# ymxlzgy/echoscene

Hardware: AMD Instinct MI355X
Metric: denoising steps/sec (layout+SDF) for 32-node scene-graph, 64^3 SDF (3x16^3 latent), full step = one DDPM layout step + one DDIM shape step over all objects; `value` = the FUSED step (both loops as one hipGraph per step, the layout step on a parallel branch: what the K timed steps ran); `full_steps_p (higher is better)
Workload: dtype f16 MFMA operands / f32 accumulate (shape UNet); f32 (layout, GCN)

## Files before the change

echoscene_amd/csrc/es_conv_route.h:

```cpp
#pragma once
#include <cstddef>
#include <cstdint>
#include "../../include/echoscene_hip.h"
#include "es_error.h"

constexpr int BN = 224;
constexpr int GN_VT = 64;

struct ConvGeom {
    int O, D, H, W;
    int Hi, Wi;
    int Di;
    int lw, lh, ld;
};

enum class ConvKernel {
    none,
    small_n, small_n_tiled, n16, kw_4_1, kw_2_2, ws_256_8_4_3, ws_64_4_4_3, ws_64_4_4_6, ws_128_4_4_3, ws_128_4_8_3, ws_128_4_8_5, ws3,
    ws_256_up_fold,
    linear_ws, linear_deep, lean_256, lean_128, lean_64
};
extern const char* const kConvKernelName[(int)ConvKernel::lean_64 + 1];
enum class ConvReduce { none, plain, gn_part };

enum class SplitRule {
    direct,
    forced_tile,
    few_plain,
    few_kstreams,
    caller,
    rows256,
    deep,
    tiny,
    fill256,
    auto128,
    none
};

struct ConvRoute {
    ConvGeom g;
    int ncdhw;
    long M;
    long omax;
    ConvKernel kernel;
    unsigned gx = 1, gy = 1, gz = 1;
    size_t lds;
    SplitRule rule;
    int S;
    int ncb;
    bool upm, geglu;
    char unbuilt[96];
    bool epi_stats;
    bool stats;
    bool part_ok;
    ConvReduce reduce;
    int vt;
    bool stats_pass;
    int slabs;
    bool fold_bal;
};

struct RouteOptions {
    int conv_tile = 0;
    int conv_force256 = 0;
    int conv_ws = 1;
    int conv_wssplit = 1;
    int conv_wss_target = 256;
    int conv_deep = 1;
    int conv_tinysplit = 1;
    int gn_rg = 1;
    int conv_few = 1;
    int conv_st_bm = 0;
    int conv_st_np = 4;
    int conv_st_ns = 3;
    int conv_kw_ks = 0;
    int env_a3 = 1;
    int env_linws = 1;
    int env_n16 = 1;
};
const RouteOptions& es_route_options();

int conv_route(const es_conv_args& a, const RouteOptions& o, ConvRoute* r);

es_conv_args conv_chunk_args(const es_conv_args& a, const ConvGeom& g, long o0, long n);

inline int gn_voxel_tile(long Oh, int V) {
    int vt = GN_VT;
    while (vt > 8 && Oh * ((V + vt - 1) / vt) < 512) vt >>= 1;
    return vt;
}
```

echoscene_amd/csrc/es_conv_route.hip:

```cpp
#include "es_conv_route.h"
#include <algorithm>
#include <cstdio>
#include <cstdlib>
#include <cstring>
#include <string>

const char* const kConvKernelName[] = {
    "none",
    "small_n", "small_n_tiled", "n16", "kw_4_1", "kw_2_2", "ws_256_8_4_3", "ws_64_4_4_3", "ws_64_4_4_6", "ws_128_4_4_3", "ws_128_4_8_3", "ws_128_4_8_5", "ws3",
    "ws_256_up_fold", "linear_ws", "linear_deep", "lean_256", "lean_128", "lean_64"
};

#ifndef ES_CONV_A3_DEFAULT
#define ES_CONV_A3_DEFAULT true
#endif
namespace {
const struct { const char* name; int RouteOptions::*field; } kOptions[] = {
    {"conv_tile", &RouteOptions::conv_tile}, {"conv_force256", &RouteOptions::conv_force256}, {"conv_ws", &RouteOptions::conv_ws},
    {"conv_wssplit", &RouteOptions::conv_wssplit}, {"conv_wss_target", &RouteOptions::conv_wss_target}, {"conv_deep", &RouteOptions::conv_deep},
    {"conv_tinysplit", &RouteOptions::conv_tinysplit}, {"gn_rg", &RouteOptions::gn_rg}, {"conv_few", &RouteOptions::conv_few},
    {"conv_st_bm", &RouteOptions::conv_st_bm}, {"conv_st_np", &RouteOptions::conv_st_np}, {"conv_st_ns", &RouteOptions::conv_st_ns},
    {"conv_kw_ks", &RouteOptions::conv_kw_ks},
};

RouteOptions& process_options() {
    static RouteOptions o = [] {
        RouteOptions v;
        const char* a3 = getenv("ES_CONV_A3");
        const char* lin = getenv("ES_CONV_LINWS");
        const char* n16 = getenv("ES_CONV_N16");
        v.env_a3 = a3 ? atoi(a3) != 0 : ES_CONV_A3_DEFAULT;
        v.env_linws = !(lin && atoi(lin) == 0);
        v.env_n16 = !(n16 && atoi(n16) == 0);
        return v;
    }();
    return o;
}
}

const RouteOptions& es_route_options() { return process_options(); }

extern "C" int es_vol_set_option(const char* name, int value) {
    ES_REQUIRE(name != nullptr, "es_vol_set_option: null name");
    for (const auto& k : kOptions) if (!strcmp(k.name, name)) { process_options().*k.field = value; return 0; }
    ES_REQUIRE(false, "es_vol_set_option: unknown option '%s'", name);
}
extern "C" int es_vol_options(char* out, int cap) {
    std::string s;
    for (const auto& k : kOptions) { s += k.name; s += '='; s += std::to_string(process_options().*k.field); s += ';'; }
    if (out && cap > 0) { strncpy(out, s.c_str(), (size_t)cap - 1); out[cap - 1] = 0; }
    return (int)s.size() + 1;
}

namespace {

int ilog2_exact(int v) {
    int l = 0;
    while ((1 << l) < v) ++l;
    return (1 << l) == v ? l : -1;
}

int route_geometry(const es_conv_args& a, ConvRoute* r) {
    ES_REQUIRE(a.Cin % 32 == 0 && a.Cin > 0, "es_conv_mfma_f16: Cin=%d must be a positive multiple of 32", a.Cin);
    ES_REQUIRE(a.taps == 27 || a.taps == 1, "es_conv_mfma_f16: taps=%d", a.taps);
    ES_REQUIRE(!a.a2 || (a.Cin2 % 32 == 0 && a.Cin2 > 0), "es_conv_mfma_f16: Cin2=%d", a.Cin2);
    ES_REQUIRE(a.out_f32 || a.out_f16, "es_conv_mfma_f16: no output");
    ES_REQUIRE(a.epilogue == ES_EPI_NONE || (a.epilogue == ES_EPI_GEGLU && a.N % 224 == 0 && a.out_f16 && !a.out_f32 && !a.res &&
                                             !a.rowvec && !a.a2 && a.bias && a.out_ld >= a.N / 2 && a.out_ld % 8 == 0 && a.splitk <= 1),
               "es_conv_mfma_f16: GEGLU epilogue needs N %% 224 == 0 (N=%d), bias, f16 output only, no split-K", a.N);
    ConvGeom& g = r->g;
    g.O = a.O; g.D = a.D; g.H = a.H; g.W = a.W;
    g.Hi = a.H; g.Wi = a.W;
    g.Di = a.D;
    if (a.mode == ES_CONV_DOWN_HW) { g.Hi = 2 * a.H; g.Wi = 2 * a.W; }
    ES_REQUIRE(a.mode >= ES_CONV_SAME && a.mode <= ES_CONV_DOWN_DHW_P01, "es_conv_mfma_f16: unknown mode %d", a.mode);
    if (a.mode == ES_CONV_DOWN_DHW || a.mode == ES_CONV_DOWN_DHW_P01) { g.Hi = 2 * a.H; g.Wi = 2 * a.W; g.Di = 2 * a.D; }
    if (a.mode == ES_CONV_UP_DHW) g.Di = a.D / 2;
    if (a.mode == ES_CONV_UP_HW || a.mode == ES_CONV_UP_DHW) { g.Hi = a.H / 2; g.Wi = a.W / 2; }
    g.lw = ilog2_exact(a.W); g.lh = ilog2_exact(a.H); g.ld = ilog2_exact(a.D);
    ES_REQUIRE(g.lw >= 0 && g.lh >= 0 && g.ld >= 0, "es_conv_mfma_f16: D,H,W must be powers of two (%d,%d,%d)", a.D, a.H, a.W);
    r->ncdhw = a.out_ld < 0 ? 1 : 0;
    ES_REQUIRE(!r->ncdhw || (a.out_f32 && !a.res && !a.out_f16), "es_conv_mfma_f16: NCDHW output is fp32-only, no residual");
    r->M = (long)a.O * a.D * a.H * a.W;
    return 0;
}

long obj_bytes_in(const es_conv_args& a, const ConvGeom& g) { return (long)g.Di * g.Hi * g.Wi * a.Cin * 2; }
long obj_bytes_in2(const es_conv_args& a) { return a.a2 ? (long)a.D * a.H * a.W * a.Cin2 * 2 : 0; }

int route_chunks(const es_conv_args& a, const RouteOptions& o, ConvRoute* r) {
    const ConvGeom& g = r->g;
    const long per_obj_in = obj_bytes_in(a, g), per_obj_in2 = obj_bytes_in2(a);
    const long halo = 4L * ((g.Hi + 1) * g.Wi + 1) * a.Cin;
    const long lim = (1L << 31) - halo - 1;
    long omax = a.O;
    if (per_obj_in > 0) omax = std::min(omax, lim / per_obj_in);
    if (per_obj_in2 > 0) omax = std::min(omax, lim / per_obj_in2);
    ES_REQUIRE(omax >= 1, "es_conv_mfma_f16: one object exceeds 2 GiB of input (%ld bytes)", per_obj_in);
    if (omax >= a.O) return 0;
    ConvRoute rc;
    if (int err = conv_route(conv_chunk_args(a, g, 0, omax), o, &rc)) return err;
    r->omax = omax;
    r->S = rc.S;
    r->slabs = (int)((rc.slabs * omax + a.O - 1) / a.O);
    r->stats_pass = a.gn_stats_out != nullptr;
    return 0;
}

bool route_direct(const es_conv_args& a, const RouteOptions& o, ConvRoute* r) {
    if (a.N <= 4 && a.taps == 27 && a.Cin <= 64) {
        const size_t lds_t = (size_t)1000 * (a.Cin * 2 + 16) + (size_t)a.N * 27 * a.Cin * 2;
        const bool tiled = a.D % 8 == 0 && a.H % 8 == 0 && a.W % 8 == 0 && a.Cin % 8 == 0 && lds_t <= 160 * 1024;
        r->kernel = tiled ? ConvKernel::small_n_tiled : ConvKernel::small_n;
        r->gx = (unsigned)(tiled ? (long)a.O * (a.D / 8) * (a.H / 8) * (a.W / 8) : (r->M + 255) / 256);
        r->lds = tiled ? lds_t : (size_t)a.N * 27 * a.Cin * 2;
        r->S = 1;
        return true;
    }
    if (a.N <= 16 && a.taps == 27 && a.Cin > 64 && r->ncdhw && a.mode == ES_CONV_SAME && !a.a2 && !a.res && !a.rowvec &&
        !a.out_f16 && a.D % 4 == 0 && a.H % 4 == 0 && a.W % 16 == 0 && o.env_n16 &&
        (long)a.O * a.D * a.H * a.W * a.Cin * 2 < (1L << 31)) {
        r->kernel = ConvKernel::n16;
        r->gx = (unsigned)((long)a.O * (a.D / 4) * (a.H / 4) * (a.W / 16));
        r->S = 1;
        return true;
    }
    return false;
}

struct TileCounts {
    long t256, t128, t64;
    long t64h;
};
TileCounts tile_counts(long rows, int N) {
    const long ntn = (N + BN - 1) / BN;
    return {((rows + 255) / 256) * ntn, ((rows + 127) / 128) * ntn, ((rows + 63) / 64) * ntn, ((rows + 63) / 64) * ((N + 111) / 112)};
}
struct LaunchSize {
    long M;
    int ntn, nks;
    TileCounts wg;
    bool can_split;
    bool ws;
    int forced_ks, forced_bm;
};
struct RefSize {
    long Oh;
    TileCounts hg;
    int slab_cap;
    bool small;
};
long ref_objects(const es_conv_args& a) { return a.O_hint < 0 ? -(long)a.O_hint : (long)(a.O_hint > a.O ? a.O_hint : a.O); }

LaunchSize launch_size(const es_conv_args& a, const RouteOptions& o, const ConvRoute& r) {
    LaunchSize L;
    L.M = r.M;
    L.ntn = (a.N + BN - 1) / BN;
    L.nks = a.taps * (a.Cin / 32) + (a.a2 ? a.Cin2 / 32 : 0);
    L.wg = tile_counts(r.M, a.N);
    const bool vec_out = !r.ncdhw && a.N % 4 == 0 && a.out_ld % 4 == 0 && (!a.rowvec || a.rowvec_ld % 4 == 0);
    L.can_split = a.workspace && vec_out;
    L.ws = o.conv_ws != 0 && vec_out && r.M * (long)a.out_ld < (1L << 30) && r.M * (long)a.N < (1L << 30) &&
           (!a.rowvec || (a.D * a.H * a.W) % 64 == 0);
// ... 5 lines not shown
    RefSize R;
    R.Oh = ref_objects(a);
    const long Mh = R.Oh * a.D * a.H * a.W;
    R.hg = tile_counts(Mh, a.N);
    R.slab_cap = Mh * (long)a.N <= (1L << 22) ? 16 : 8;
    R.small = R.hg.t256 < 256 && o.conv_tile != 128 && o.conv_force256 != 1;
    return R;
}

int keep_units(int s, int nks, int units) {
    while (s > 1 && nks / s < units) --s;
    return s;
}
int caller_split(const es_conv_args& a, const LaunchSize& L) { return a.splitk > 1 && L.can_split && a.epilogue != ES_EPI_GEGLU ? a.splitk : 1; }

int split_forced_tile(const es_conv_args& a, const RouteOptions&, const LaunchSize& L, const RefSize&) { return L.forced_bm ? caller_split(a, L) : 0; }

bool few_eligible(const es_conv_args& a, const RouteOptions& o, const LaunchSize& L, const RefSize& R) {
    if (!o.conv_few || !L.ws || !R.small) return false;
    if (a.epilogue == ES_EPI_GEGLU) return a.mode != ES_CONV_UP_HW && a.mode != ES_CONV_UP_DHW && a.taps == 1 && a.splitk <= 0 && L.wg.t128 < 320;
    return a.splitk < 0 && L.can_split;
}
bool few_kstreams_fit(const es_conv_args& a, const LaunchSize& L, const RefSize& R) {
    return a.epilogue != ES_EPI_GEGLU && a.taps == 1 && L.nks < 112 && R.hg.t64h <= 272 && L.nks >= 12;
}
int split_few_plain(const es_conv_args& a, const RouteOptions& o, const LaunchSize& L, const RefSize& R) {
    if (!few_eligible(a, o, L, R)) return 0;
    if (a.epilogue == ES_EPI_GEGLU || (a.taps == 1 && L.nks < 112)) return few_kstreams_fit(a, L, R) ? 0 : 1;
    const long h128 = R.hg.t128;
    int s2 = (int)((256 + h128 / 2) / h128);
    s2 = s2 < 1 ? 1 : (s2 > 8 ? 8 : s2);
    const bool one_round = h128 * s2 <= 272;
    s2 = keep_units(s2, L.nks, 24);
    return !(L.nks >= 800 && h128 * 8 < 256) && one_round && (s2 >= 2 || h128 >= 224) ? s2 : 0;
}
int split_few_kstreams(const es_conv_args& a, const RouteOptions& o, const LaunchSize& L, const RefSize& R) {
    if (!few_eligible(a, o, L, R) || !few_kstreams_fit(a, L, R)) return 0;
    return L.wg.t256 < 256 && L.wg.t64h <= 768 ? 1 : 4;
}

int split_caller(const es_conv_args& a, const RouteOptions&, const LaunchSize& L, const RefSize&) { return a.splitk > 0 ? caller_split(a, L) : 0; }

int split_rows256(const es_conv_args& a, const RouteOptions& o, const LaunchSize& L, const RefSize& R) {
    if (!(L.ws && a.epilogue != ES_EPI_GEGLU && a.splitk < 0 && L.can_split && R.small && o.conv_wssplit != 0)) return 0;
    const long wst = o.conv_wss_target;
    const int s2 = keep_units((int)std::min(wst / R.hg.t256, (long)R.slab_cap), L.nks, 24);
    return s2 >= 2 && R.hg.t256 * s2 >= 160 ? s2 : 0;
}

int split_deep(const es_conv_args& a, const RouteOptions& o, const LaunchSize& L, const RefSize& R) {
    return a.splitk <= 0 && R.small && R.hg.t64 <= 256 && a.taps == 1 && !a.a2 && a.mode == ES_CONV_SAME && L.nks >= 4 && L.nks <= 28 &&
           a.out_ld >= 0 && L.M * (long)a.Cin * 2 < (1L << 31) && o.conv_deep != 0 ? 1 : 0;
}
int split_tiny(const es_conv_args& a, const RouteOptions& o, const LaunchSize& L, const RefSize& R) {
    if (!(a.splitk < 0 && L.can_split && o.conv_force256 != 1 && R.hg.t256 < 256 && R.hg.t128 < 128 && R.hg.t64 < 256 && L.nks >= 10 &&
          o.conv_tinysplit != 0)) return 0;
    const int s3 = (int)std::min(std::min((256 + R.hg.t64 - 1) / R.hg.t64, (long)R.slab_cap), (long)(L.nks / 5));
    return s3 >= 2 ? s3 : 0;
}

int split_fill256(const es_conv_args& a, const RouteOptions&, const LaunchSize& L, const RefSize& R) {
    const long hg256 = R.hg.t256;
    if (!(a.splitk < 0 && L.can_split && hg256 >= 256)) return 0;
    const long r1 = (hg256 + 255) / 256;
    if ((double)hg256 / (double)(r1 * 256) < 0.8)
        for (int s2 = 2; s2 <= 4; ++s2) {
            const long w = hg256 * s2;
            if ((double)w / (double)(((w + 255) / 256) * 256) >= 0.95 && L.nks / s2 >= 48) return s2;
        }
    return 0;
}

int split_auto128(const es_conv_args& a, const RouteOptions& o, const LaunchSize& L, const RefSize& R) {
    if (!(a.splitk < 0 && L.can_split && o.conv_force256 != 1 && R.hg.t256 < 256 && R.hg.t128 < 512)) return 0;
    const long want = (768 + R.hg.t128 / 2) / R.hg.t128;
    const int S = keep_units((int)std::min(std::max(want, 1L), 8L), L.nks, 24);
    return S > 1 ? S : 0;
}
int split_none(const es_conv_args&, const RouteOptions&, const LaunchSize&, const RefSize&) { return 1; }

const struct { SplitRule rule; int (*split)(const es_conv_args&, const RouteOptions&, const LaunchSize&, const RefSize&); } kSplitRules[] = {
    {SplitRule::forced_tile, split_forced_tile}, {SplitRule::few_plain, split_few_plain}, {SplitRule::few_kstreams, split_few_kstreams},
    {SplitRule::caller, split_caller},           {SplitRule::rows256, split_rows256},     {SplitRule::deep, split_deep},
    {SplitRule::tiny, split_tiny},               {SplitRule::fill256, split_fill256},     {SplitRule::auto128, split_auto128},
    {SplitRule::none, split_none},
};
void choose_split(const es_conv_args& a, const RouteOptions& o, const LaunchSize& L, const RefSize& R, ConvRoute* r) {
    for (const auto& k : kSplitRules)
        if (const int S = k.split(a, o, L, R)) {
            r->rule = k.rule;
            r->S = r->slabs = S;
            return;
        }
}

int few_tile_rows(const es_conv_args& a, const LaunchSize& L, const ConvRoute& r) {
    if (L.wg.t256 >= 256) return 256;
    if (r.rule == SplitRule::few_kstreams) return r.S == 1 ? 0 : 128;
    return a.taps == 1 && r.S == 1 ? (L.wg.t128 >= 320 ? 128 : 64) : 128;
}
int tile_rows(const es_conv_args& a, const RouteOptions& o, const LaunchSize& L, const ConvRoute& r) {
    const bool no256 = o.conv_tile == 128, force256 = o.conv_force256 == 1;
    switch (r.rule) {
    case SplitRule::few_plain:
    case SplitRule::few_kstreams: return few_tile_rows(a, L, r);
    case SplitRule::rows256: return 256;
    case SplitRule::tiny: return 64;
    default: break;
    }
    if (!no256 && (L.wg.t256 >= 256 || (force256 && (r.S == 1 || r.rule == SplitRule::fill256)))) return 256;
    return L.wg.t128 >= 512 || r.S > 1 ? 128 : 64;
}

void forced_tile(const RouteOptions& o, const LaunchSize& L, ConvRoute* r) {
    const unsigned uy = (unsigned)L.ntn;
    if (const int ks = L.forced_ks) {
        r->kernel = ks == 4 ? ConvKernel::kw_4_1 : ks == 2 ? ConvKernel::kw_2_2 : ConvKernel::none;
        snprintf(r->unbuilt, sizeof(r->unbuilt), "conv_kw_ks=%d (2 or 4)", ks);
        r->gx = (unsigned)((L.M + 63) / 64); r->gy = ks == 4 ? 2 * uy : uy;
        return;
    }
    const int bm = L.forced_bm, np = o.conv_st_np, ns = o.conv_st_ns;
    if (bm == 64 && np == 4 && ns == 3) r->kernel = ConvKernel::ws_64_4_4_3;
    else if (bm == 64 && np == 4 && ns == 6) r->kernel = ConvKernel::ws_64_4_4_6;
    else if (bm == 128 && np == 4 && ns == 3) r->kernel = ConvKernel::ws_128_4_4_3;
    else if (bm == 128 && np == 8 && ns == 3) r->kernel = ConvKernel::ws_128_4_8_3;
    else if (bm == 128 && np == 8 && ns == 5) r->kernel = ConvKernel::ws_128_4_8_5;
    else snprintf(r->unbuilt, sizeof(r->unbuilt), "conv_st_bm=%d conv_st_np=%d conv_st_ns=%d is not a built tile", bm, np, ns);
    r->gx = (unsigned)((L.M + bm - 1) / bm); r->gy = uy;
}

void tile_256(const es_conv_args& a, const RouteOptions& o, const LaunchSize& L, ConvRoute* r) {
    r->gx = (unsigned)((L.M + 255) / 256);
    if (L.ws && a.taps == 1 && !a.a2 && a.mode == ES_CONV_SAME && r->S == 1 && L.ntn >= 2 && o.env_linws)
        for (const int ncb : {8, 6, 4, 3, 2})
            if (L.ntn % ncb == 0 && (long)r->gx * (L.ntn / ncb) >= 256) {
                r->kernel = ConvKernel::linear_ws;
                r->ncb = ncb; r->gy = (unsigned)(L.ntn / ncb);
                return;
            }
    if (!(L.ws && (!r->geglu || !r->upm))) { r->kernel = ConvKernel::lean_256; return; }
    const bool a3 = o.env_a3 && a.taps == 27 && a.mode == ES_CONV_SAME && !a.a2 && a.W <= 16 && a.W >= 4;
    r->kernel = a3 ? ConvKernel::ws3 : ConvKernel::ws_256_8_4_3;
    if (a3 || !(a.mode == ES_CONV_UP_HW && a.w2 && !a.a2 && r->S == 1 && a.O_hint == 0 && a.H >= 2 && a.W >= 2 &&
                ((long)a.D * r->g.Hi * r->g.Wi) % 256 == 0)) return;
    r->kernel = ConvKernel::ws_256_up_fold;
    const long rounds = (L.wg.t256 + 255) / 256;
    if (L.ntn == 3 && !a.workspace && L.M % 256 == 0 && (double)L.wg.t256 / (double)(rounds * 256) < 0.8) {
        r->fold_bal = true;
        r->gy = 2;
    }
}

bool choose_tile(const es_conv_args& a, const RouteOptions& o, const LaunchSize& L, ConvRoute* r) {
    r->ncb = 1;
    r->gy = (unsigned)L.ntn; r->gz = (unsigned)r->S;
    if (r->rule == SplitRule::forced_tile) { forced_tile(o, L, r); return L.forced_bm == 128; }
    if (r->rule == SplitRule::deep) {
        r->kernel = ConvKernel::linear_deep;
        r->gx = (unsigned)((L.M + 63) / 64);
        return false;
    }
    const bool few = r->rule == SplitRule::few_plain || r->rule == SplitRule::few_kstreams;
    const int rows = tile_rows(a, o, L, *r);
    switch (rows) {
    case 256: tile_256(a, o, L, r); return L.ws && r->ncb == 1;
    case 128: r->kernel = few ? ConvKernel::ws_128_4_8_5 : ConvKernel::lean_128; break;
    case 64: r->kernel = few ? ConvKernel::ws_64_4_4_3 : ConvKernel::lean_64; break;
    default: r->kernel = ConvKernel::kw_4_1; r->gy = 2 * (unsigned)L.ntn; break;
    }
    r->gx = (unsigned)((L.M + (rows ? rows : 64) - 1) / (rows ? rows : 64));
    return few && rows == 128;
}

void route_flags(const es_conv_args& a, bool stats_tile, ConvRoute* r) {
    const int V = a.D * a.H * a.W;
    r->epi_stats = stats_tile && !r->geglu && r->S == 1 && (a.out_f32 || a.out_f16) && a.N % 4 == 0 && a.out_ld % 4 == 0 && V % 64 == 0;
    r->part_ok = r->S > 1 && r->rule != SplitRule::few_kstreams && a.out_f32 && !r->ncdhw && a.N % 4 == 0 && a.N <= 2048 && a.out_ld == a.N &&
                 a.gn_part_groups > 0 && a.gn_part_groups <= 64 && a.N % a.gn_part_groups == 0;
    const bool want_stats = a.gn_stats_out != nullptr;
    r->stats = want_stats && r->epi_stats;
    r->stats_pass = want_stats && !r->epi_stats;
    if (r->S > 1) {
        r->reduce = a.gn_part_out && r->part_ok ? ConvReduce::gn_part : ConvReduce::plain;
        if (r->reduce == ConvReduce::gn_part) r->vt = gn_voxel_tile(ref_objects(a), V);
    }
}

}

es_conv_args conv_chunk_args(const es_conv_args& a, const ConvGeom& g, long o0, long n) {
    const long V = (long)a.D * a.H * a.W;
    es_conv_args c = a;
    c.O = (int32_t)n;
    c.O_hint = a.O_hint < 0 ? a.O_hint : (a.O_hint > a.O ? a.O_hint : a.O);
    c.a = (const char*)a.a + o0 * obj_bytes_in(a, g);
    if (a.a2) c.a2 = (const char*)a.a2 + o0 * obj_bytes_in2(a);
    if (a.rowvec) c.rowvec = a.rowvec + o0 * a.rowvec_ld;
    if (a.out_ld < 0) {
        c.out_f32 = a.out_f32 + o0 * a.N * V;
    } else {
        if (a.res) c.res = a.res + o0 * V * a.out_ld;
        if (a.out_f32) c.out_f32 = a.out_f32 + o0 * V * a.out_ld;
        if (a.out_f16) c.out_f16 = (char*)a.out_f16 + o0 * V * a.out_ld * 2;
    }
    c.gn_stats_out = c.gn_part_out = nullptr;
    return c;
}

int conv_route(const es_conv_args& a, const RouteOptions& o, ConvRoute* r) {
    *r = ConvRoute{};
    if (int err = route_geometry(a, r)) return err;
    if (int err = route_chunks(a, o, r)) return err;
    if (r->omax || route_direct(a, o, r)) return 0;
    ES_REQUIRE(!a.gn_stats_out || ((a.out_f32 || a.out_f16) && !r->ncdhw && a.N % 4 == 0 && a.out_ld % 4 == 0 && (a.D * a.H * a.W) % 64 == 0 &&
                                   a.epilogue == ES_EPI_NONE),
               "es_conv_mfma_f16: gn_stats_out needs a channels-last output, N %% 4 == 0 and voxels per object %% 64 == 0");
    r->upm = a.mode == ES_CONV_UP_HW || a.mode == ES_CONV_UP_DHW;
    r->geglu = a.epilogue == ES_EPI_GEGLU;
    ES_REQUIRE(!r->upm || (!a.a2 && a.taps == 27), "es_conv_mfma_f16: nearest-up modes take 3x3x3 convs without a fused skip");
    const LaunchSize L = launch_size(a, o, *r);
    choose_split(a, o, L, ref_size(a, o), r);
    route_flags(a, choose_tile(a, o, L, r), r);
    return 0;
}

extern "C" int es_conv_route_of(const es_conv_args* a, es_conv_route_info* out) {
    ConvRoute r;
    if (conv_route(*a, es_route_options(), &r) != 0) return -1;
    *out = es_conv_route_info{(int32_t)r.kernel, r.gx, r.gy, r.gz, (int32_t)r.lds, r.S, r.slabs, r.ncb, (int32_t)r.omax,
                              (int32_t)r.epi_stats, (int32_t)r.stats, (int32_t)r.stats_pass, (int32_t)r.part_ok, (int32_t)r.reduce, r.vt,
                              (int32_t)r.fold_bal};
    return 0;
}
extern "C" int es_conv_emits_gn_stats(const es_conv_args* a) {
    es_conv_route_info i;
    return es_conv_route_of(a, &i) == 0 ? i.epi_stats : -1;
}
extern "C" int es_conv_emits_gn_part(const es_conv_args* a) {
    es_conv_route_info i;
    return es_conv_route_of(a, &i) == 0 ? i.part_ok : -1;
}
extern "C" int es_conv_split_of(const es_conv_args* a) {
    es_conv_route_info i;
    return es_conv_route_of(a, &i) == 0 ? i.slabs : -1;
}
extern "C" int es_conv_kernel_of(const es_conv_args* a, char* name_out, int cap) {
    es_conv_route_info i;
    if (es_conv_route_of(a, &i) != 0) return -1;
    if (name_out && cap > 0) snprintf(name_out, (size_t)cap, "%s", i.omax ? "chunked" : kConvKernelName[i.kernel]);
    return i.S > 1 ? i.S : 1;
}
extern "C" int es_conv_fold_balanced(const es_conv_args* a) {
    es_conv_route_info i;
    return es_conv_route_of(a, &i) == 0 ? i.fold_bal : -1;
}
```

echoscene_amd/csrc/es_vol.hip:

```cpp
#include "es_common.h"
#include "es_conv_route.h"
#include <string>
#include <algorithm>
#include <cstdlib>
#include <initializer_list>
#include <utility>
#include <type_traits>

namespace {

__device__ __forceinline__ int f_swz(int row) { return (0x1320 >> (((row >> 2) & 3) * 4)) & 3; }


__global__ __launch_bounds__(256) void k_gn_partial(const es_gn_args a, float* part, int vt) {
    __shared__ float ssum4[4][2048], ssq4[4][2048];
    float* ssum = ssum4[0];
    float* ssq = ssq4[0];
    const int o = blockIdx.y, tile = blockIdx.x, C = a.C1 + a.C2;
    const int v0 = tile * vt;
    const int nv = min(vt, a.V - v0);
    const int c4n = C >> 2;
    const int CX = 64;
    const int cx = threadIdx.x & (CX - 1), vy = threadIdx.x >> 6;
    for (int c4 = cx; c4 < c4n; c4 += CX) {
// ... 828 lines not shown
        stage_advance();
    };

    f4 acc[MI][7];
#pragma unroll
    for (int i = 0; i < MI; ++i)
#pragma unroll
        for (int j = 0; j < 7; ++j) acc[i][j] = f4{0.f, 0.f, 0.f, 0.f};

    const int i16 = lane & 15, q = lane >> 4;
    const int fragA = (wm * WROWS + i16) * 64 + ((q ^ f_swz(i16)) << 4);
    const int fragB = A_BYTES + (wn * 112 + i16) * 64 + ((q ^ f_swz(i16)) << 4);

    stage_all(0);
    if (nloc > 1) stage_all(1);
    int ks = 0;
    auto body = [&](auto slot_c) __attribute__((always_inline)) {
        constexpr int RS = decltype(slot_c)::value;
        constexpr int WS = (RS + 2) % NS;
        if (ks + 1 < nloc) wait_vmcnt<NLOAD>(); else wait_vmcnt<0>();
        __builtin_amdgcn_s_barrier();
        const bool pf = ks + 2 < nloc;
        if (pf) stage_prep();
        h8 af[MI], bfr[7];
        const char* As = smem + RS * STAGE_BYTES;
#pragma unroll
        for (int j = 0; j < 7; ++j) bfr[j] = *(const h8*)(As + fragB + j * 1024);
#pragma unroll
        for (int i = 0; i < MI; ++i) af[i] = *(const h8*)(As + fragA + i * 1024);
        constexpr int PPR = (NLOAD + MI - 1) / MI;
#pragma unroll
        for (int i = 0; i < MI; ++i) {
#pragma unroll
            for (int j = 0; j < 7; ++j)
                acc[i][j] = __builtin_amdgcn_mfma_f32_16x16x32_f16(af[i], bfr[j], acc[i][j], 0, 0, 0);
            __builtin_amdgcn_sched_barrier(0);
            if (pf) {
#pragma unroll
                for (int pp = 0; pp < PPR; ++pp)
                    if (i * PPR + pp < NLOAD) stage_piece(WS, i * PPR + pp);
            }
            __builtin_amdgcn_sched_barrier(0);
        }
        if (pf) stage_advance();
    };
    while (true) {
        body(std::integral_constant<int, 0>{}); if (++ks >= nloc) break;
        body(std::integral_constant<int, 1>{}); if (++ks >= nloc) break;
        body(std::integral_constant<int, 2>{}); if (++ks >= nloc) break;
    }
    conv_epilogue<BM_, NW_>(a, g, acc, smem, M, m0, n0, wave, lane, S, bz, ncdhw);
}

__global__ __launch_bounds__(256) void k_linear_deep(const es_conv_args a, const ConvGeom g) {
    constexpr int BM_ = 64, NW_ = 4, NS = 7, NT = 256;
    constexpr int WROWS = BM_ / (NW_ / 2), MI = WROWS / 16;
    constexpr int A_BYTES = BM_ * BK * 2, B_BYTES = BNP * BK * 2, STAGE_BYTES = A_BYTES + B_BYTES;
    constexpr int NA = BM_ * 4 / NT, NB = BNP * 4 / NT, NLOAD = NA + NB;
    constexpr unsigned OOB = 0x80000000u;
    typedef __attribute__((address_space(3))) void* lds_ptr;
    extern __shared__ __attribute__((aligned(16))) char smem[];
    const int tid = threadIdx.x, lane = tid & 63;
    const int wave = __builtin_amdgcn_readfirstlane(tid >> 6);
    const int wm = wave >> 1, wn = wave & 1;
    const long M = (long)g.O * g.D * g.H * g.W;
    int bx, by, bz;
    conv_tile_of(a, bx, by, bz);
    const long m0 = (long)bx * BM_;
    const int n0 = by * BN;
    const int nloc = a.Cin >> 5;
    unsigned voffA;
    {
        const int row = tid >> 2;
        const long m = m0 + row;
        voffA = m < M ? (unsigned)(m * a.Cin * 2 + (((tid & 3) ^ f_swz(row)) * 16)) : OOB;
    }
    const __amdgpu_buffer_rsrc_t rA = __builtin_amdgcn_make_buffer_rsrc(uniform_ptr(a.a), (short)0, (int)OOB, 0x00020000);
    const __amdgpu_buffer_rsrc_t rB = __builtin_amdgcn_make_buffer_rsrc(uniform_ptr((const _Float16*)a.w + ((long)by * nloc) * (BNP * BK)), (short)0, (int)OOB, 0x00020000);
    auto stage = [&](int ks, int slot) __attribute__((always_inline)) {
        char* dst = smem + slot * STAGE_BYTES + wave * 1024;
        __builtin_amdgcn_raw_ptr_buffer_load_lds(rA, (lds_ptr)dst, 16, (int)voffA, (int)((unsigned)ks * 64u), 0, 0);
#pragma unroll
        for (int j = 0; j < NB; ++j) {
            const unsigned vB = (unsigned)tid * 16u + (unsigned)j * (NT * 16) >= (unsigned)(BN * BK * 2) ? OOB : (unsigned)tid * 16u;
            __builtin_amdgcn_raw_ptr_buffer_load_lds(rB, (lds_ptr)(dst + A_BYTES + j * (NT * 16)), 16, (int)vB,
                                                     (int)((unsigned)ks * (unsigned)B_BYTES + (unsigned)j * (NT * 16)), 0, 0);
        }
    };
    f4 acc[MI][7];
#pragma unroll
    for (int i = 0; i < MI; ++i)
#pragma unroll
        for (int j = 0; j < 7; ++j) acc[i][j] = f4{0.f, 0.f, 0.f, 0.f};
    const int i16 = lane & 15, q = lane >> 4;
    const int fragA = (wm * WROWS + i16) * 64 + ((q ^ f_swz(i16)) << 4);
    const int fragB = A_BYTES + (wn * 112 + i16) * 64 + ((q ^ f_swz(i16)) << 4);
    int issued = 0;
    for (; issued < NS - 1 && issued < nloc; ++issued) stage(issued, issued);
    int slot = 0;
    for (int ks = 0; ks < nloc; ++ks) {
        const int after = issued - 1 - ks;
        if (after >= 5) wait_vmcnt<5 * NLOAD>(); else if (after == 4) wait_vmcnt<4 * NLOAD>(); else if (after == 3) wait_vmcnt<3 * NLOAD>();
        else if (after == 2) wait_vmcnt<2 * NLOAD>(); else if (after == 1) wait_vmcnt<NLOAD>(); else wait_vmcnt<0>();
        __builtin_amdgcn_s_barrier();
        if (issued < nloc) { const int ws_ = slot == 0 ? NS - 1 : slot - 1; stage(issued, ws_); ++issued; }
        const char* As = smem + slot * STAGE_BYTES;
        h8 af[MI], bfr[7];
#pragma unroll
        for (int j = 0; j < 7; ++j) bfr[j] = *(const h8*)(As + fragB + j * 1024);
#pragma unroll
        for (int i = 0; i < MI; ++i) af[i] = *(const h8*)(As + fragA + i * 1024);
#pragma unroll
        for (int i = 0; i < MI; ++i)
#pragma unroll
            for (int j = 0; j < 7; ++j) acc[i][j] = __builtin_amdgcn_mfma_f32_16x16x32_f16(af[i], bfr[j], acc[i][j], 0, 0, 0);
        slot = slot == NS - 1 ? 0 : slot + 1;
    }
    conv_epilogue<BM_, NW_>(a, g, acc, smem, M, m0, n0, wave, lane, 1, 0, 0);
}

template <int MI>
__device__ __forceinline__ void ws_read_frags(const char* As, int fragA, int fragB, h8 (&af)[MI], h8 (&bfr)[7]) {
#pragma unroll
    for (int j = 0; j < 7; ++j) bfr[j] = *(const h8*)(As + fragB + j * 1024);
#pragma unroll
    for (int i = 0; i < MI; ++i) af[i] = *(const h8*)(As + fragA + i * 1024);
}

template <int MI>
__device__ __forceinline__ void ws_mma(f4 (&acc)[MI][7], const h8 (&af)[MI], const h8 (&bfr)[7]) {
#pragma unroll
    for (int i = 0; i < MI; ++i)
#pragma unroll
        for (int j = 0; j < 7; ++j) acc[i][j] = __builtin_amdgcn_mfma_f32_16x16x32_f16(af[i], bfr[j], acc[i][j], 0, 0, 0);
}

#ifdef ES_STAMP
__device__ unsigned long long* g_stamp_buf = nullptr;
#define ES_STAMP_AT(k) do { if (stamp && lane == 0) stamp[k] = __builtin_amdgcn_s_memrealtime(); } while (0)
#else
#define ES_STAMP_AT(k) do { } while (0)
#endif

template <int NL, int MAXA>
__device__ __forceinline__ void wait_ahead(int ahead) {
    if constexpr (MAXA > 0) {
        if (ahead >= MAXA) { wait_vmcnt<MAXA * NL>(); return; }
        wait_ahead<NL, MAXA - 1>(ahead);
    } else {
        wait_vmcnt<0>();
    }
}

template <int BM_, int NC_, int NP_, bool UP_, int EPI_, bool STATS_, int NS_ = 3, bool FOLD_ = false>
__device__ __forceinline__ void conv_ws_tile(const es_conv_args& a, const ConvGeom& g, int ncdhw, char* smem, const int wave, const int lane,
                                             const long M, const int bx, const int by, const int ks_begin, const int ks_end,
                                             const int S, const int bz, unsigned long long* stamp) {
    constexpr int NS = NS_, UPS_ = 1;
    constexpr int WROWS = BM_ / (NC_ / 2);
    constexpr int MI = WROWS / 16;
    constexpr int A_BYTES = BM_ * BK * 2, B_BYTES = BNP * BK * 2, UNIT_BYTES = A_BYTES + B_BYTES;
    constexpr int STAGE_BYTES = UPS_ * UNIT_BYTES;
    constexpr int APIECES = BM_ / 16, BPIECES = BNP / 16;
    constexpr int NA = APIECES / NP_, NB = BPIECES / NP_, NLOAD = NA + NB;
    static_assert(APIECES % NP_ == 0 && BPIECES % NP_ == 0, "pieces must divide over the producer waves");
    constexpr unsigned OOB = 0x80000000u;
    typedef __attribute__((address_space(3))) void* lds_ptr;
    (void)stamp;
    const long m0 = (long)bx * BM_;
    const int n0 = by * BN;
    const int kch0 = a.Cin >> 5;
    const int ntap0 = FOLD_ ? 12 : a.taps;
    const int nks0 = ntap0 * kch0;
    const int nloc = ks_end - ks_begin;
    const int nstage = (nloc + UPS_ - 1) / UPS_;
    static_assert(!FOLD_ || UP_, "the folded taps are those of a nearest-up conv");
    const int fold_cls = FOLD_ ? (int)((m0 >> (g.lw + g.lh + g.ld - 2)) & 3) : 0;
    const int fold_ph = fold_cls >> 1, fold_pw = fold_cls & 1;
    if (wave >= NC_) {
        const int pw = wave - NC_;
        int a_lc[NA], a_o[NA], a_d[NA], a_h[NA], a_w[NA];
        bool a_ok[NA];
#pragma unroll
        for (int j = 0; j < NA; ++j) {
            const int p = (pw + NP_ * j) * 64 + lane;
            const int row = p >> 2;
            a_lc[j] = (p & 3) ^ f_swz(row);
            const long m = m0 + row;
            a_ok[j] = m < M;
            const long mm = a_ok[j] ? m : 0;
            a_w[j] = (int)(mm & (g.W - 1));
            a_h[j] = (int)((mm >> g.lw) & (g.H - 1));
            a_d[j] = (int)((mm >> (g.lw + g.lh)) & (g.D - 1));
            a_o[j] = (int)(mm >> (g.lw + g.lh + g.ld));
            if constexpr (FOLD_) {
                a_w[j] = 2 * (int)(mm & (g.Wi - 1)) + fold_pw;
                a_h[j] = 2 * (int)((mm >> (g.lw - 1)) & (g.Hi - 1)) + fold_ph;
                a_d[j] = (int)((mm >> (g.lw + g.lh - 2)) & (g.D - 1));
            }
        }
        int st_phase = ks_begin >= nks0 ? 1 : 0;
        int st_tap = st_phase ? 0 : ks_begin % ntap0;
        int st_c = st_phase ? (ks_begin - nks0) : (ks_begin / ntap0);
        int st_ntap = st_phase ? 1 : ntap0, st_kch = st_phase ? (a.Cin2 >> 5) : kch0;
        unsigned st_boff = (unsigned)(st_phase ? (ks_begin - nks0) : ks_begin) * (unsigned)B_BYTES;
        unsigned voff[NA], msk[NA];
        int upm[NA][3], upp[NA][3];
        int dtab = 0;
        __amdgpu_buffer_rsrc_t rA, rB;
        auto set_phase = [&]() __attribute__((always_inline)) {
            const _Float16* Wg = (const _Float16*)(st_phase ? a.w2 : a.w);
            const long nks_ph = st_phase ? (long)(a.Cin2 >> 5) : (long)nks0;
            if constexpr (FOLD_) Wg = (const _Float16*)a.w2 + ((long)fold_cls * ((a.N + BN - 1) / BN) * nks0) * (BNP * BK);
            rB = __builtin_amdgcn_make_buffer_rsrc((void*)(Wg + ((long)by * nks_ph) * (BNP * BK)), (short)0, (int)OOB, 0x00020000);
            const _Float16* Ag = (const _Float16*)(st_phase ? a.a2 : a.a);
            const int Cin = st_phase ? a.Cin2 : a.Cin;
            const int p01 = (!st_phase && a.mode == ES_CONV_DOWN_DHW_P01) ? 1 : 0;
            const bool down = !st_phase && (a.mode == ES_CONV_DOWN_HW || a.mode == ES_CONV_DOWN_DHW || p01);
            const bool downd = !st_phase && (a.mode == ES_CONV_DOWN_DHW || p01);
            const int Dsrc = downd ? 2 * g.D : g.D;
            const int Hi = st_phase ? g.H : g.Hi, Wi = st_phase ? g.W : g.Wi;
            const int ntap = st_phase ? 1 : a.taps;
            const bool updhw = UP_ && a.mode == ES_CONV_UP_DHW;
            const int Di = updhw ? g.D / 2 : g.D;
            const int bias = ntap == 27 ? ((Hi + 1) * Wi + 1) * Cin * 2 : 0;
            rA = __builtin_amdgcn_make_buffer_rsrc((void*)((const char*)Ag - bias), (short)0, (int)OOB, 0x00020000);
            {
                const int t = lane < 27 ? lane : 13;
                const int kd = t / 9 - 1, kh = (t / 3) % 3 - 1, kw = t % 3 - 1;
                dtab = ntap == 27 ? ((kd * Hi + kh) * Wi + kw) * Cin * 2 + bias : 0;
                if (UP_) dtab = ntap == 27 ? (updhw ? 0 : kd * Hi * Wi * Cin * 2) + bias : 0;
            }
#pragma unroll
            for (int j = 0; j < NA; ++j) {
                const int ch = down ? 2 * a_h[j] + p01 : a_h[j];
                const int cw = down ? 2 * a_w[j] + p01 : a_w[j];
                const int cd = downd ? 2 * a_d[j] + p01 : a_d[j];
                voff[j] = (unsigned)(((((long)a_o[j] * Dsrc + cd) * Hi + ch) * Wi + cw) * Cin * 2 + a_lc[j] * 16);
                if (UP_) {
                    const int sd = updhw ? a_d[j] >> 1 : a_d[j];
                    voff[j] = (unsigned)(((((long)a_o[j] * Di + sd) * Hi + (a_h[j] >> 1)) * Wi + (a_w[j] >> 1)) * Cin * 2 + a_lc[j] * 16);
                    const int SD = Hi * Wi * Cin * 2, SH = Wi * Cin * 2, SW = Cin * 2;
                    upm[j][0] = (updhw && !(a_d[j] & 1)) ? -SD : 0; upp[j][0] = (updhw && (a_d[j] & 1)) ? SD : 0;
                    upm[j][1] = !(a_h[j] & 1) ? -SH : 0;            upp[j][1] = (a_h[j] & 1) ? SH : 0;
                    upm[j][2] = !(a_w[j] & 1) ? -SW : 0;            upp[j][2] = (a_w[j] & 1) ? SW : 0;
                }
                unsigned m = 0;
                if (ntap == 1) {
                    m = a_ok[j] ? 1u : 0u;
                } else {
                    m = a_ok[j] ? tap_mask27(cd, Dsrc, ch, UP_ ? g.H : Hi, cw, UP_ ? g.W : Wi) : 0u;
                }
                msk[j] = m;
            }
        };
        set_phase();
        ES_STAMP_AT(1);
        const unsigned voffB = (unsigned)lane * 16u;
        auto issue_unit = [&](char* dst) __attribute__((always_inline)) {
            int tap27 = st_tap;
            if constexpr (FOLD_) tap27 = (st_tap >> 2) * 9 + (((st_tap >> 1) & 1) + fold_ph) * 3 + (st_tap & 1) + fold_pw;
            const unsigned sA = (unsigned)__builtin_amdgcn_readlane(dtab, tap27) + (unsigned)st_c * 64u;
            const unsigned sbit = 1u << tap27;
            int ukd = 0, ukh = 0, ukw = 0;
            if (UP_) { ukd = tap27 / 9 - 1; ukh = (tap27 / 3) % 3 - 1; ukw = tap27 % 3 - 1; }
#pragma unroll
            for (int j = 0; j < NA; ++j) {
                unsigned vs = voff[j];
                if (UP_) {
                    vs += (unsigned)(ukd < 0 ? upm[j][0] : ukd > 0 ? upp[j][0] : 0);
                    vs += (unsigned)(ukh < 0 ? upm[j][1] : ukh > 0 ? upp[j][1] : 0);
                    vs += (unsigned)(ukw < 0 ? upm[j][2] : ukw > 0 ? upp[j][2] : 0);
                }
                const unsigned vo = (msk[j] & sbit) ? vs : OOB;
                __builtin_amdgcn_raw_ptr_buffer_load_lds(rA, (lds_ptr)(dst + (pw + NP_ * j) * 1024), 16, (int)vo, (int)sA, 0, 0);
            }
#pragma unroll
            for (int j = 0; j < NB; ++j) {
                const int q = pw + NP_ * j;
                const unsigned vB = q * 16 >= BN ? OOB : voffB;
                __builtin_amdgcn_raw_ptr_buffer_load_lds(rB, (lds_ptr)(dst + A_BYTES + q * 1024), 16, (int)vB,
                                                         (int)(st_boff + (unsigned)q * 1024u), 0, 0);
            }
            st_boff += (unsigned)B_BYTES;
            if (++st_tap == st_ntap) {
                st_tap = 0;
                if (++st_c == st_kch && !st_phase && a.a2) {
                    st_phase = 1; st_c = 0; st_ntap = 1; st_kch = a.Cin2 >> 5; st_boff = 0;
                    set_phase();
                }
            }
        };
        int issued = 0;
        auto issue_stage = [&](int st) __attribute__((always_inline)) {
            char* base = smem + (st % NS) * STAGE_BYTES;
#pragma unroll
            for (int u = 0; u < UPS_; ++u)
                if (issued < nloc) { issue_unit(base + u * UNIT_BYTES); ++issued; }
        };
        {
            static_assert(NLOAD * (NS - 2) <= 63, "vmcnt is a 6-bit counter");
#pragma unroll
            for (int st = 0; st < NS - 1; ++st)
                if (st < nstage) issue_stage(st);
            for (int st = 0; st < nstage; ++st) {
                wait_ahead<NLOAD, NS - 2>(nstage - 1 - st);
                __builtin_amdgcn_s_barrier();
                if (st == 0) ES_STAMP_AT(2);
                if (st + NS - 1 < nstage) issue_stage(st + NS - 1);
            }
        }
        ES_STAMP_AT(3);
        f4 dummy[MI][7];
        conv_epilogue<BM_, NC_, false, true, EPI_, false, STATS_, FOLD_>(a, g, dummy, smem, M, m0, n0, wave, lane, S, bz, ncdhw);
        ES_STAMP_AT(4);
        return;
    }
    const int wm = wave >> 1, wn = wave & 1;
    f4 acc[MI][7];
#pragma unroll
    for (int i = 0; i < MI; ++i)
#pragma unroll
        for (int j = 0; j < 7; ++j) acc[i][j] = f4{0.f, 0.f, 0.f, 0.f};
    const int i16 = lane & 15, q = lane >> 4;
    const int fragA = (wm * WROWS + i16) * 64 + ((q ^ f_swz(i16)) << 4);
    const int fragB = A_BYTES + (wn * 112 + i16) * 64 + ((q ^ f_swz(i16)) << 4);
    h8 af[MI], bfr[7];
    {
        int slot = 0;
        ES_STAMP_AT(1);
        __builtin_amdgcn_s_barrier();
        ES_STAMP_AT(2);
        ws_read_frags<MI>(smem, fragA, fragB, af, bfr);
        for (int ks = 0; ks + 1 < nloc; ++ks) {
            slot = slot == NS - 1 ? 0 : slot + 1;
            const char* const An = smem + slot * STAGE_BYTES;
#pragma unroll
            for (int j = 0; j < 7; ++j) acc[0][j] = __builtin_amdgcn_mfma_f32_16x16x32_f16(af[0], bfr[j], acc[0][j], 0, 0, 0);
            __builtin_amdgcn_sched_barrier(0);
            asm volatile("s_waitcnt lgkmcnt(0)" ::: "memory");
            __builtin_amdgcn_s_barrier();
            __builtin_amdgcn_sched_barrier(0);
#pragma unroll
            for (int i = 1; i < MI; ++i) {
                af[i - 1] = *(const h8*)(An + fragA + (i - 1) * 1024);
                __builtin_amdgcn_sched_barrier(0);
                if (i < MI - 1) {
#pragma unroll
                    for (int j = 0; j < 7; ++j) acc[i][j] = __builtin_amdgcn_mfma_f32_16x16x32_f16(af[i], bfr[j], acc[i][j], 0, 0, 0);
                    __builtin_amdgcn_sched_barrier(0);
                } else {
#pragma unroll
                    for (int j = 0; j < 7; ++j) {
                        acc[i][j] = __builtin_amdgcn_mfma_f32_16x16x32_f16(af[i], bfr[j], acc[i][j], 0, 0, 0);
                        __builtin_amdgcn_sched_barrier(0);
                        bfr[j] = *(const h8*)(An + fragB + j * 1024);
                        __builtin_amdgcn_sched_barrier(0);
                    }
                }
            }
            af[MI - 1] = *(const h8*)(An + fragA + (MI - 1) * 1024);
            __builtin_amdgcn_sched_barrier(0);
        }
        ws_mma<MI>(acc, af, bfr);
    }
    ES_STAMP_AT(3);
    conv_epilogue<BM_, NC_, true, true, EPI_, false, STATS_, FOLD_>(a, g, acc, smem, M, m0, n0, wave, lane, S, bz, ncdhw);
    ES_STAMP_AT(4);
}

template <int BM_, int NC_, int NP_, bool UP_ = false, int EPI_ = ES_EPI_NONE, bool STATS_ = false, int NS_ = 3>
__global__ __launch_bounds__(64 * (NC_ + NP_), 3) void k_conv_ws(const es_conv_args a, const ConvGeom g, int ncdhw) {
    extern __shared__ __attribute__((aligned(16))) char smem[];
    const int tid = threadIdx.x, lane = tid & 63;
    const int wave = __builtin_amdgcn_readfirstlane(tid >> 6);
    unsigned long long* stamp = nullptr;
#ifdef ES_STAMP
    stamp = g_stamp_buf ? g_stamp_buf + ((size_t)(blockIdx.x + gridDim.x * (blockIdx.y + gridDim.y * blockIdx.z)) * (NC_ + NP_) + wave) * 8 : nullptr;
#endif
    ES_STAMP_AT(0);
    const long M = (long)g.O * g.D * g.H * g.W;
    int bx, by, bz;
    conv_tile_of(a, bx, by, bz);
    const int S = gridDim.z;
    int ks_begin, ks_end;
    split_range(a.taps * (a.Cin >> 5), a.a2 ? (a.Cin2 >> 5) : 0, a.taps, bz, S, ks_begin, ks_end);
    conv_ws_tile<BM_, NC_, NP_, UP_, EPI_, STATS_, NS_>(a, g, ncdhw, smem, wave, lane, M, bx, by, ks_begin, ks_end, S, bz, stamp);
}

template <bool STATS_>
__global__ __launch_bounds__(768, 3) void k_conv_ws_fold(const es_conv_args a, const ConvGeom g) {
    extern __shared__ __attribute__((aligned(16))) char smem[];
    const int tid = threadIdx.x, lane = tid & 63;
    const int wave = __builtin_amdgcn_readfirstlane(tid >> 6);
    unsigned long long* stamp = nullptr;
#ifdef ES_STAMP
    stamp = g_stamp_buf ? g_stamp_buf + ((size_t)(blockIdx.x + gridDim.x * (blockIdx.y + gridDim.y * blockIdx.z)) * 12 + wave) * 8 : nullptr;
#endif
    ES_STAMP_AT(0);
    const long M = (long)g.O * g.D * g.H * g.W;
    int bx, by, bz;
    conv_tile_of(a, bx, by, bz);
    conv_ws_tile<256, 8, 4, true, ES_EPI_NONE, STATS_, 3, true>(a, g, 0, smem, wave, lane, M, bx, by, 0, 12 * (a.Cin >> 5), 1, 0, stamp);
}

template <bool STATS_>
__global__ __launch_bounds__(768, 3) void k_conv_ws_fold_bal(const es_conv_args a, const ConvGeom g) {
    extern __shared__ __attribute__((aligned(16))) char smem[];
    const int tid = threadIdx.x, lane = tid & 63;
    const int wave = __builtin_amdgcn_readfirstlane(tid >> 6);
    const long M = (long)g.O * g.D * g.H * g.W;
    int bx, by, bz;
    conv_tile_of(a, bx, by, bz);
    const int nks = 12 * (a.Cin >> 5);
    conv_ws_tile<256, 8, 4, true, ES_EPI_NONE, STATS_, 3, true>(a, g, 0, smem, wave, lane, M, bx, by, 0, nks, 1, 0, nullptr);
    __syncthreads();
    conv_ws_tile<128, 8, 4, true, ES_EPI_NONE, STATS_, 3, true>(a, g, 0, smem, wave, lane, M, 2 * bx + by, 2, 0, nks, 1, 0, nullptr);
}

typedef int i4v __attribute__((ext_vector_type(4)));
template <int DIR>
__device__ __forceinline__ h8 a3_shift(const h8 v, const bool zero_lane) {
    i4v x = __builtin_bit_cast(i4v, v);
#pragma unroll
    for (int e = 0; e < 4; ++e) {
        const int s = DIR < 0 ? __builtin_amdgcn_update_dpp(0, x[e], 0x111, 0xf, 0xf, true) : __builtin_amdgcn_update_dpp(0, x[e], 0x101, 0xf, 0xf, true);
        x[e] = zero_lane ? 0 : s;
    }
    return __builtin_bit_cast(h8, x);
}

template <bool STATS_>
__global__ __launch_bounds__(768, 3) void k_conv_ws3(const es_conv_args a, const ConvGeom g) {
    constexpr int BM_ = 256, NC_ = 8, NP_ = 4, NSB = 7, MI = 4;
    constexpr int A_BYTES = BM_ * BK * 2, B_BYTES = BNP * BK * 2, A_RING = NSB * B_BYTES;
    constexpr int NA = (BM_ / 16) / NP_, NB = (BNP / 16) / NP_;
    constexpr unsigned OOB = 0x80000000u;
    typedef __attribute__((address_space(3))) void* lds_ptr;
    extern __shared__ __attribute__((aligned(16))) char smem[];
    const int tid = threadIdx.x, lane = tid & 63;
    const int wave = __builtin_amdgcn_readfirstlane(tid >> 6);
    const long M = (long)g.O * g.D * g.H * g.W;
    int bx, by, bz;
    conv_tile_of(a, bx, by, bz);
    const int S = gridDim.z;
    const int kch0 = a.Cin >> 5, nks0 = 27 * kch0;
    int ks_begin, ks_end;
    split_range(nks0, 0, 27, bz, S, ks_begin, ks_end);
    const int nloc = ks_end - ks_begin, ngrp = nloc / 3;
    const long m0 = (long)bx * BM_;
    const int n0 = by * BN;
    if (wave >= NC_) {
        const int pw = wave - NC_;
        unsigned voff[NA], msk[NA];
#pragma unroll
        for (int j = 0; j < NA; ++j) {
            const int p = (pw + NP_ * j) * 64 + lane;
            const int row = p >> 2;
            const int lc = (p & 3) ^ f_swz(row);
            const long m = m0 + row;
            const bool ok = m < M;
            const long mm = ok ? m : 0;
            const int w = (int)(mm & (g.W - 1)), h = (int)((mm >> g.lw) & (g.H - 1)), d = (int)((mm >> (g.lw + g.lh)) & (g.D - 1));
            const int o = (int)(mm >> (g.lw + g.lh + g.ld));
            voff[j] = (unsigned)(((((long)o * g.D + d) * g.H + h) * g.W + w) * a.Cin * 2 + lc * 16);
            msk[j] = ok ? tap_mask27(d, g.D, h, g.H, w, g.W) : 0u;
        }
        const int bias = ((g.H + 1) * g.W + 1) * a.Cin * 2;
        const __amdgpu_buffer_rsrc_t rA = __builtin_amdgcn_make_buffer_rsrc((void*)((const char*)a.a - bias), (short)0, (int)OOB, 0x00020000);
        const __amdgpu_buffer_rsrc_t rB = __builtin_amdgcn_make_buffer_rsrc((void*)((const _Float16*)a.w + ((long)by * nks0) * (BNP * BK)), (short)0, (int)OOB, 0x00020000);
        int dtab;
        {
            const int t = lane < 27 ? lane : 13;
            const int kd = t / 9 - 1, kh = (t / 3) % 3 - 1, kw = t % 3 - 1;
            dtab = ((kd * g.H + kh) * g.W + kw) * a.Cin * 2 + bias;
        }
        int a_tap = ks_begin % 27, a_c = ks_begin / 27;
        unsigned b_off = (unsigned)ks_begin * (unsigned)B_BYTES;
        const unsigned voffB = (unsigned)lane * 16u;
        auto issue_A = [&](int slot) __attribute__((always_inline)) {
            char* dst = smem + A_RING + slot * A_BYTES;
            const unsigned sA = (unsigned)__builtin_amdgcn_readlane(dtab, a_tap + 1) + (unsigned)a_c * 64u;
            const unsigned sbit = 1u << (a_tap + 1);
#pragma unroll
            for (int j = 0; j < NA; ++j)
                __builtin_amdgcn_raw_ptr_buffer_load_lds(rA, (lds_ptr)(dst + (pw + NP_ * j) * 1024), 16, (int)((msk[j] & sbit) ? voff[j] : OOB), (int)sA, 0, 0);
            a_tap += 3;
            if (a_tap == 27) { a_tap = 0; ++a_c; }
        };
        auto issue_B = [&](int slot) __attribute__((always_inline)) {
            char* dst = smem + slot * B_BYTES;
#pragma unroll
            for (int j = 0; j < NB; ++j) {
                const int q = pw + NP_ * j;
                __builtin_amdgcn_raw_ptr_buffer_load_lds(rB, (lds_ptr)(dst + q * 1024), 16, (int)(q * 16 >= BN ? OOB : voffB), (int)(b_off + (unsigned)q * 1024u), 0, 0);
            }
            b_off += (unsigned)B_BYTES;
        };
        int sb = 0;
        auto issue_group = [&](int gi) __attribute__((always_inline)) {
            issue_A(gi & 1);
#pragma unroll
            for (int t = 0; t < 3; ++t) { issue_B(sb); sb = sb == NSB - 1 ? 0 : sb + 1; }
        };
        issue_group(0);
        for (int gi = 0; gi < ngrp; ++gi) {
            wait_vmcnt<0>();
            __builtin_amdgcn_s_barrier();
            if (gi + 1 < ngrp) issue_group(gi + 1);
        }
        __builtin_amdgcn_s_barrier();
        f4 dummy[MI][7];
        conv_epilogue<BM_, NC_, false, true, ES_EPI_NONE, false, STATS_>(a, g, dummy, smem, M, m0, n0, wave, lane, S, bz, 0);
        return;
    }
    const int wm = wave >> 1, wn = wave & 1;
    f4 acc[MI][7];
#pragma unroll
    for (int i = 0; i < MI; ++i)
#pragma unroll
        for (int j = 0; j < 7; ++j) acc[i][j] = f4{0.f, 0.f, 0.f, 0.f};
    const int i16 = lane & 15, q = lane >> 4;
    const int fragA = A_RING + (wm * 64 + i16) * 64 + ((q ^ f_swz(i16)) << 4);
    const int fragB = (wn * 112 + i16) * 64 + ((q ^ f_swz(i16)) << 4);
    const bool zl = (i16 & (g.W - 1)) == 0, zr = (i16 & (g.W - 1)) == ((g.W - 1) & 15);
    h8 afc[MI], bq[3];
    __builtin_amdgcn_s_barrier();
    bq[0] = *(const h8*)(smem + fragB);
    bq[1] = *(const h8*)(smem + fragB + 1024);
#pragma unroll
    for (int i = 0; i < MI; ++i) afc[i] = *(const h8*)(smem + fragA + i * 1024);
    int slotB = 0;
    for (int grp = 0; grp < ngrp; ++grp) {
        const char* const An = smem + ((grp + 1) & 1) * A_BYTES;
        auto unit = [&](auto kwc) __attribute__((always_inline)) {
            constexpr int KW = decltype(kwc)::value;
            const char* const Bc = smem + slotB * B_BYTES;
            slotB = slotB == NSB - 1 ? 0 : slotB + 1;
            const char* const Bn = smem + slotB * B_BYTES;
            h8 ash[MI];
// ... 1041 lines not shown
    const int h0 = jh == 0 ? 0 : (ph == 0 ? 1 : 2), h1 = jh == 0 ? (ph == 0 ? 0 : 1) : 2;
    const int w0 = jw == 0 ? 0 : (pw == 0 ? 1 : 2), w1 = jw == 0 ? (pw == 0 ? 0 : 1) : 2;
    double s = 0.0;
    for (int kh = h0; kh <= h1; ++kh)
        for (int kw = w0; kw <= w1; ++kw) s += (double)w27[kd * 9 + kh * 3 + kw];
    float f = (float)s;
    if ((double)f != s) {
        uint32_t u = __builtin_bit_cast(uint32_t, f);
        const double af = f < 0.f ? -(double)f : (double)f, as = s < 0.0 ? -s : s;
        if (af > as) --u;
        u |= 1u;
        f = __builtin_bit_cast(float, u);
    }
    return f;
}

extern "C" size_t es_pack_conv_up_fold_f16_size(int N, int Cin) { return 4 * es_pack_conv_f16_size(N, Cin, 12); }

extern "C" int es_pack_conv_up_fold_f16(const float* h_w, int N, int CinW, uint16_t* h_out) {
    ES_REQUIRE(h_w && h_out && N > 0 && CinW > 0, "es_pack_conv_up_fold_f16: N=%d Cin=%d", N, CinW);
    const int Cin = (CinW + 31) / 32 * 32;
    const int nt = (N + BN - 1) / BN, kch = Cin / 32;
    es_parallel_for(4L * nt * kch * 12, [=](long bi) {
        const int tap = (int)(bi % 12), kc = (int)((bi / 12) % kch), t = (int)((bi / (12L * kch)) % nt), cls = (int)(bi / (12L * kch * nt));
        uint16_t* blk = h_out + (size_t)bi * (BNP * BK);
        for (int p = 0; p < BNP * 4; ++p) {
            const int row = p >> 2, lc = (p & 3) ^ h_swz(row);
            const int n = t * BN + row;
            for (int e = 0; e < 8; ++e) {
                const int c = kc * 32 + lc * 8 + e;
                blk[p * 8 + e] = (row < BN && n < N && c < CinW) ? f32_to_f16_bits(up_fold_weight(h_w + ((size_t)n * CinW + c) * 27, cls, tap)) : 0;
            }
        }
    });
    return 0;
}

__global__ __launch_bounds__(256) void k_pack_conv_up_fold_f16(const float* __restrict__ w, int N, int CinW, int kch, int nt, h8* __restrict__ out, long nslots) {
    const long s = (long)blockIdx.x * 256 + threadIdx.x;
    if (s >= nslots) return;
    const int p = (int)(s & (BNP * 4 - 1));
    const long bi = s / (BNP * 4);
    const int tap = (int)(bi % 12), kc = (int)((bi / 12) % kch), t = (int)((bi / (12L * kch)) % nt), cls = (int)(bi / (12L * kch * nt));
    const int row = p >> 2, lc = (p & 3) ^ ((0x1320 >> (((row >> 2) & 3) * 4)) & 3);
    const int n = t * BN + row;
    h8 v;
#pragma unroll
    for (int e = 0; e < 8; ++e) {
        const int c = kc * 32 + lc * 8 + e;
        v[e] = (row < BN && n < N && c < CinW) ? (_Float16)up_fold_weight(w + ((size_t)n * CinW + c) * 27, cls, tap) : (_Float16)0.f;
    }
    out[s] = v;
}

extern "C" int es_pack_conv_up_fold_f16_dev(const float* d_w, int N, int CinW, uint16_t* d_out, es_stream stream) {
    ES_REQUIRE(d_w && d_out && N > 0 && CinW > 0, "es_pack_conv_up_fold_f16_dev: N=%d Cin=%d", N, CinW);
    const int Cin = (CinW + 31) / 32 * 32;
    const long nslots = (long)es_pack_conv_up_fold_f16_size(N, Cin) / 8;
    hipLaunchKernelGGL(k_pack_conv_up_fold_f16, dim3((unsigned)((nslots + 255) / 256)), dim3(256), 0, (hipStream_t)stream, d_w, N, CinW, Cin / 32,
                       (N + BN - 1) / BN, (h8*)d_out, nslots);
    ES_CHECK_HIP(hipGetLastError());
    return 0;
}

extern "C" int es_pack_conv_rows_f16(const float* h_w, int N, int CinW, int taps, uint16_t* h_out) {
    const int Cin = (CinW + 31) / 32 * 32;
    for (int n = 0; n < N; ++n)
        for (int t = 0; t < taps; ++t)
            for (int c = 0; c < Cin; ++c)
                h_out[((size_t)n * taps + t) * Cin + c] = c < CinW ? f32_to_f16_bits(h_w[((size_t)n * CinW + c) * taps + t]) : 0;
    return 0;
}

namespace {
struct LdsLimits {
    hipError_t err = hipSuccess;
    LdsLimits(std::initializer_list<std::pair<const void*, int>> kernels) {
        for (const auto& k : kernels)
            if (const hipError_t e = hipFuncSetAttribute(k.first, hipFuncAttributeMaxDynamicSharedMemorySize, k.second); err == hipSuccess) err = e;
    }
};

dim3 grid_of(const ConvRoute& r) { return dim3(r.gx, r.gy, r.gz); }
}

constexpr int LDS256 = 3 * (256 * BK * 2 + BNP * BK * 2), LDS128 = 3 * (128 * BK * 2 + BNP * BK * 2), LDS64 = 3 * (64 * BK * 2 + BNP * BK * 2);
constexpr int LDSLIN = LDS256 + 8 * 16 * 116 * 4;
constexpr int LDSDEEP = 7 * (64 * BK * 2 + BNP * BK * 2);
constexpr int LDSWS3 = 9 * 16384;

template <int BM_, int NC_, int NP_, int NS_>
static int launch_ws(const es_conv_args* a, const ConvRoute& r, hipStream_t st) {
    constexpr int LDS = NS_ * (BM_ * BK * 2 + BNP * BK * 2);
    constexpr bool CAN_STATS = BM_ / (NC_ / 2) == 64;
    static_assert(LDS <= 160 * 1024, "ring exceeds the CU's LDS");
    static const LdsLimits lim{{(const void*)k_conv_ws<BM_, NC_, NP_, false, ES_EPI_NONE, false, NS_>, LDS},
                               {(const void*)k_conv_ws<BM_, NC_, NP_, true, ES_EPI_NONE, false, NS_>, LDS},
                               {(const void*)k_conv_ws<BM_, NC_, NP_, false, ES_EPI_GEGLU, false, NS_>, LDS}};
    ES_REQUIRE(lim.err == hipSuccess, "es_conv_mfma_f16: hipFuncSetAttribute failed: %s", hipGetErrorString(lim.err));
    const dim3 blk(64 * (NC_ + NP_));
    if (r.geglu) hipLaunchKernelGGL((k_conv_ws<BM_, NC_, NP_, false, ES_EPI_GEGLU, false, NS_>), grid_of(r), blk, LDS, st, *a, r.g, r.ncdhw);
    else if (r.stats) {
        if constexpr (CAN_STATS) {
            static const LdsLimits lim_stats{{(const void*)k_conv_ws<BM_, NC_, NP_, false, ES_EPI_NONE, true, NS_>, LDS},
                                             {(const void*)k_conv_ws<BM_, NC_, NP_, true, ES_EPI_NONE, true, NS_>, LDS}};
            ES_REQUIRE(lim_stats.err == hipSuccess, "es_conv_mfma_f16: hipFuncSetAttribute failed: %s", hipGetErrorString(lim_stats.err));
            if (r.upm) hipLaunchKernelGGL((k_conv_ws<BM_, NC_, NP_, true, ES_EPI_NONE, true, NS_>), grid_of(r), blk, LDS, st, *a, r.g, r.ncdhw);
            else hipLaunchKernelGGL((k_conv_ws<BM_, NC_, NP_, false, ES_EPI_NONE, true, NS_>), grid_of(r), blk, LDS, st, *a, r.g, r.ncdhw);
        } else ES_REQUIRE(false, "launch_ws: row-group sums need 64-row waves");
    }
    else if (r.upm) hipLaunchKernelGGL((k_conv_ws<BM_, NC_, NP_, true, ES_EPI_NONE, false, NS_>), grid_of(r), blk, LDS, st, *a, r.g, r.ncdhw);
    else hipLaunchKernelGGL((k_conv_ws<BM_, NC_, NP_, false, ES_EPI_NONE, false, NS_>), grid_of(r), blk, LDS, st, *a, r.g, r.ncdhw);
    return 0;
}

template <int KS_, int NCH_>
static int launch_kw(const es_conv_args* a, const ConvRoute& r, hipStream_t st) {
    constexpr int RING = 3 * KS_ * (64 * BK * 2 + NCH_ * 112 * BK * 2), PART = 4 * 112 * 64 * 4;
    constexpr int LDS = RING > PART ? RING : PART;
    static const LdsLimits lim{{(const void*)k_conv_kw<KS_, NCH_, false, ES_EPI_NONE>, LDS},
                               {(const void*)k_conv_kw<KS_, NCH_, true, ES_EPI_NONE>, LDS},
                               {(const void*)k_conv_kw<KS_, NCH_, false, ES_EPI_GEGLU>, LDS}};
    ES_REQUIRE(lim.err == hipSuccess, "es_conv_mfma_f16: hipFuncSetAttribute failed: %s", hipGetErrorString(lim.err));
    const dim3 blk(768);
    if (r.geglu) hipLaunchKernelGGL((k_conv_kw<KS_, NCH_, false, ES_EPI_GEGLU>), grid_of(r), blk, LDS, st, *a, r.g, r.ncdhw);
    else if (r.upm) hipLaunchKernelGGL((k_conv_kw<KS_, NCH_, true, ES_EPI_NONE>), grid_of(r), blk, LDS, st, *a, r.g, r.ncdhw);
    else hipLaunchKernelGGL((k_conv_kw<KS_, NCH_, false, ES_EPI_NONE>), grid_of(r), blk, LDS, st, *a, r.g, r.ncdhw);
    return 0;
}

template <int BM_, int NW_>
static void launch_lean(const es_conv_args* a, const ConvRoute& r, hipStream_t st) {
    constexpr int LDS = 3 * (BM_ * BK * 2 + BNP * BK * 2);
    if (r.upm) hipLaunchKernelGGL((k_conv_lean<BM_, NW_, true>), grid_of(r), dim3(64 * NW_), LDS, st, *a, r.g, r.ncdhw);
    else hipLaunchKernelGGL((k_conv_lean<BM_, NW_>), grid_of(r), dim3(64 * NW_), LDS, st, *a, r.g, r.ncdhw);
}

static void launch_rowgroup_stats(const es_conv_args* a, long rows, hipStream_t st) {
    const long n4 = ((rows + 63) / 64) * (a->N / 4);
    const int blocks = (int)((n4 + 255) / 256 < 8192 ? (n4 + 255) / 256 : 8192);
    hipLaunchKernelGGL(k_rowgroup_stats, dim3(blocks), dim3(256), 0, st, (const float*)a->out_f32, rows, a->N, a->out_ld, a->gn_stats_out);
}

static int conv_launch(const es_conv_args* a, const ConvRoute& r, hipStream_t st) {
    static const LdsLimits lim{{(const void*)k_conv_small_n_tiled, 160 * 1024},
                               {(const void*)k_conv_n16, N16_A_BYTES + N16_B_BYTES},
                               {(const void*)k_conv_lean<256, 8>, LDS256}, {(const void*)k_conv_lean<256, 8, true>, LDS256},
                               {(const void*)k_conv_lean<128, 4>, LDS128}, {(const void*)k_conv_lean<128, 4, true>, LDS128},
                               {(const void*)k_conv_lean<64, 4>, LDS64}, {(const void*)k_conv_lean<64, 4, true>, LDS64},
                               {(const void*)k_linear_deep, LDSDEEP},
                               {(const void*)k_linear_ws<ES_EPI_NONE>, LDSLIN}, {(const void*)k_linear_ws<ES_EPI_GEGLU>, LDSLIN},
                               {(const void*)k_conv_ws3<false>, LDSWS3}, {(const void*)k_conv_ws3<true>, LDSWS3},
                               {(const void*)k_conv_ws_fold<false>, LDS256}, {(const void*)k_conv_ws_fold<true>, LDS256},
                               {(const void*)k_conv_ws_fold_bal<false>, LDS256}, {(const void*)k_conv_ws_fold_bal<true>, LDS256}};
    ES_REQUIRE(lim.err == hipSuccess, "es_conv_mfma_f16: hipFuncSetAttribute failed: %s", hipGetErrorString(lim.err));
    ES_REQUIRE(r.kernel != ConvKernel::none, "es_conv_mfma_f16: %s", r.omax ? "a chunked route is launched chunk by chunk" : r.unbuilt);
    int rc = 0;
    switch (r.kernel) {
    case ConvKernel::none: break;
    case ConvKernel::small_n:
    case ConvKernel::small_n_tiled:
        ES_REQUIRE(a->mode == ES_CONV_SAME && !a->a2 && !a->res && !a->rowvec && !a->out_f16 && !a->gn_stats_out,
                   "es_conv_mfma_f16: the N<=4, Cin<=64 direct kernel takes SAME mode, fp32 output, no fusions");
        if (r.kernel == ConvKernel::small_n_tiled) hipLaunchKernelGGL(k_conv_small_n_tiled, grid_of(r), dim3(256), r.lds, st, *a, r.g, r.ncdhw);
        else hipLaunchKernelGGL(k_conv_small_n, grid_of(r), dim3(256), r.lds, st, *a, r.g, r.ncdhw);
        break;
    case ConvKernel::n16: hipLaunchKernelGGL(k_conv_n16, grid_of(r), dim3(256), N16_A_BYTES + N16_B_BYTES, st, *a, r.g); break;
    case ConvKernel::kw_4_1: rc = launch_kw<4, 1>(a, r, st); break;
    case ConvKernel::kw_2_2: rc = launch_kw<2, 2>(a, r, st); break;
    case ConvKernel::ws_256_8_4_3: rc = launch_ws<256, 8, 4, 3>(a, r, st); break;
    case ConvKernel::ws_64_4_4_3: rc = launch_ws<64, 4, 4, 3>(a, r, st); break;
    case ConvKernel::ws_64_4_4_6: rc = launch_ws<64, 4, 4, 6>(a, r, st); break;
    case ConvKernel::ws_128_4_4_3: rc = launch_ws<128, 4, 4, 3>(a, r, st); break;
    case ConvKernel::ws_128_4_8_3: rc = launch_ws<128, 4, 8, 3>(a, r, st); break;
    case ConvKernel::ws_128_4_8_5: rc = launch_ws<128, 4, 8, 5>(a, r, st); break;
    case ConvKernel::ws3:
        if (r.stats) hipLaunchKernelGGL((k_conv_ws3<true>), grid_of(r), dim3(768), LDSWS3, st, *a, r.g);
        else hipLaunchKernelGGL((k_conv_ws3<false>), grid_of(r), dim3(768), LDSWS3, st, *a, r.g);
        break;
    case ConvKernel::ws_256_up_fold:
        if (r.fold_bal) {
            if (r.stats) hipLaunchKernelGGL((k_conv_ws_fold_bal<true>), grid_of(r), dim3(768), LDS256, st, *a, r.g);
            else hipLaunchKernelGGL((k_conv_ws_fold_bal<false>), grid_of(r), dim3(768), LDS256, st, *a, r.g);
        } else if (r.stats) hipLaunchKernelGGL((k_conv_ws_fold<true>), grid_of(r), dim3(768), LDS256, st, *a, r.g);
        else hipLaunchKernelGGL((k_conv_ws_fold<false>), grid_of(r), dim3(768), LDS256, st, *a, r.g);
        break;
    case ConvKernel::linear_ws:
        if (r.geglu) hipLaunchKernelGGL((k_linear_ws<ES_EPI_GEGLU>), grid_of(r), dim3(768), LDSLIN, st, *a, r.g, r.ncb);
        else hipLaunchKernelGGL((k_linear_ws<ES_EPI_NONE>), grid_of(r), dim3(768), LDSLIN, st, *a, r.g, r.ncb);
        break;
    case ConvKernel::linear_deep: hipLaunchKernelGGL(k_linear_deep, grid_of(r), dim3(256), LDSDEEP, st, *a, r.g); break;
    case ConvKernel::lean_256: launch_lean<256, 8>(a, r, st); break;
    case ConvKernel::lean_128: launch_lean<128, 4>(a, r, st); break;
    case ConvKernel::lean_64: launch_lean<64, 4>(a, r, st); break;
    }
    if (rc) return rc;
    const int V = a->D * a->H * a->W;
    if (r.reduce == ConvReduce::gn_part)
        hipLaunchKernelGGL(k_conv_splitk_reduce_gn, dim3((V + r.vt - 1) / r.vt, a->O), dim3(256), 0, st, *a, r.M, V, r.S, r.vt);
    else if (r.reduce == ConvReduce::plain) {
        const long n4 = r.M * (a->N / 4);
        const int blocks = (int)((n4 + 255) / 256 < 4096 ? (n4 + 255) / 256 : 4096);
        hipLaunchKernelGGL(k_conv_splitk_reduce, dim3(blocks), dim3(256), 0, st, *a, r.M, V, r.S);
    }
    if (r.stats_pass) {
        ES_REQUIRE(a->out_f32, "es_conv_mfma_f16: this launch's route forms gn_stats_out by a pass over the fp32 output: out_f32 must be given "
                               "(es_conv_emits_gn_stats() == 0)");
        launch_rowgroup_stats(a, r.M, st);
    }
    ES_CHECK_HIP(hipGetLastError());
    return 0;
}

extern "C" int es_conv_mfma_f16(const es_conv_args* a, es_stream stream) {
    ConvRoute r;
    if (int rc = conv_route(*a, es_route_options(), &r)) return rc;
    const hipStream_t st = (hipStream_t)stream;
    if (!r.omax) return conv_launch(a, r, st);
    for (long o0 = 0; o0 < a->O; o0 += r.omax) {
        const es_conv_args c = conv_chunk_args(*a, r.g, o0, std::min(r.omax, (long)a->O - o0));
        ConvRoute rc;
        if (int err = conv_route(c, es_route_options(), &rc)) return err;
        if (int err = conv_launch(&c, rc, st)) return err;
    }
    if (r.stats_pass) {
        ES_REQUIRE(a->out_f32 && !r.ncdhw && a->N % 4 == 0 && a->out_ld % 4 == 0 && ((long)a->D * a->H * a->W) % 64 == 0,
                   "es_conv_mfma_f16: gn_stats_out needs a channels-last fp32 output");
        launch_rowgroup_stats(a, r.M, st);
        ES_CHECK_HIP(hipGetLastError());
    }
    return 0;
}

extern "C" int es_groupnorm_vol(const es_gn_args* a, es_stream stream) {
    const int C = a->C1 + a->C2;
    ES_REQUIRE(C % a->groups == 0 && C <= 2048 && a->groups <= 64, "es_groupnorm_vol: C=%d groups=%d", C, a->groups);
    ES_REQUIRE(a->C1 % 8 == 0 && a->C2 % 8 == 0, "es_groupnorm_vol: channel counts must be multiples of 8 (%d,%d)", a->C1, a->C2);
    ES_REQUIRE(a->stats != nullptr, "es_groupnorm_vol: stats scratch missing");
    const long Oh = a->O_hint < 0 ? -(long)a->O_hint : (long)(a->O_hint > a->O ? a->O_hint : a->O);
    const int vt = gn_voxel_tile(Oh, a->V);
    const int ntiles = (a->V + vt - 1) / vt;
    float* part = a->stats;
    const bool from_rg = a->stats1 && (!a->x2 || a->stats2) && a->V % 64 == 0 && (a->x1_is_f16 || es_route_options().gn_rg != 0);
    ES_REQUIRE(!a->x1_is_f16 || (from_rg && !a->x2 && !a->raw_f16),
               "es_groupnorm_vol: an f16 source needs the producer's row-group sums (stats1), one source, no raw copy");
    ES_REQUIRE(!a->part_in || (!from_rg && !a->x2), "es_groupnorm_vol: part_in needs one source and no row-group sums");
    if (a->part_in) part = (float*)a->part_in;
    else if (!from_rg) hipLaunchKernelGGL(k_gn_partial, dim3(ntiles, a->O), dim3(256), 0, (hipStream_t)stream, *a, part, vt);
    int vpb = 32;
    while (vpb > 8 && (long)a->O * ((a->V + vpb - 1) / vpb) < 512) vpb >>= 1;
    while (vpb < 1024 && (long)a->O * ((a->V + vpb - 1) / vpb) > 16384) vpb <<= 1;
    const float* fin = nullptr;
    if (from_rg) {
        hipLaunchKernelGGL(k_gn_finalize_rg, dim3(a->groups, a->O), dim3(256), 0, (hipStream_t)stream, *a, part);
        fin = part;
    } else if (ntiles > 128) {
        float* f = a->part_in ? a->stats : part + (size_t)a->O * ntiles * a->groups * 2;
        hipLaunchKernelGGL(k_gn_finalize, dim3(a->groups, a->O), dim3(256), 0, (hipStream_t)stream, *a, part, ntiles, f);
        fin = f;
    }
    hipLaunchKernelGGL(k_gn_apply, dim3((a->V + vpb - 1) / vpb, a->O), dim3(256), 0, (hipStream_t)stream, *a, part, ntiles, vpb, fin);
    ES_CHECK_HIP(hipGetLastError());
    return 0;
}

extern "C" int es_layernorm_tokens(const es_ln_args* a, es_stream stream) {
    ES_REQUIRE(a->C <= 1024 && a->C > 0 && a->C % 4 == 0, "es_layernorm_tokens: C=%d (a multiple of 4, max 1024)", a->C);
    long wgs = ((long)a->M + 3) / 4;
    if (wgs > 2048) wgs = 2048;
    hipLaunchKernelGGL(k_layernorm, dim3((unsigned)wgs), dim3(256), 0, (hipStream_t)stream, *a);
    ES_CHECK_HIP(hipGetLastError());
    return 0;
}

extern "C" int es_attention_f16(const es_attn_args* a, es_stream stream) {
    ES_REQUIRE(a->dhead % 4 == 0 && a->dhead <= 256 && a->dhead > 0, "es_attention_f16: dhead=%d (multiple of 4, <= 256)", a->dhead);
    ES_REQUIRE(a->scale > 0.f, "es_attention_f16: scale=%g must be positive (the row maximum is taken over the raw scores)", (double)a->scale);
    const bool big = a->Ntok >= 512 && a->dhead <= 96;
    const int rows = big ? 128 : 64;
    dim3 grid((a->Ntok + rows - 1) / rows, a->B * a->heads);
    hipStream_t st = (hipStream_t)stream;
    if (a->dhead <= 32) { if (big) hipLaunchKernelGGL((k_attention<32, 4, 2>), grid, dim3(256), 0, st, *a); else hipLaunchKernelGGL((k_attention<32, 4, 1>), grid, dim3(256), 0, st, *a); }
    else if (a->dhead <= 64) { if (big) hipLaunchKernelGGL((k_attention<64, 4, 2>), grid, dim3(256), 0, st, *a); else hipLaunchKernelGGL((k_attention<64, 4, 1>), grid, dim3(256), 0, st, *a); }
    else if (a->dhead <= 96) { if (big) hipLaunchKernelGGL((k_attention<96, 4, 2>), grid, dim3(256), 0, st, *a); else hipLaunchKernelGGL((k_attention<96, 4, 1>), grid, dim3(256), 0, st, *a); }
    else hipLaunchKernelGGL((k_attention<256, 4, 1>), grid, dim3(256), 0, st, *a);
    ES_CHECK_HIP(hipGetLastError());
    return 0;
}

extern "C" int es_geglu_f16(const es_geglu_args* a, es_stream stream) {
    ES_REQUIRE(a->C4 % 4 == 0, "es_geglu_f16: C4=%d", a->C4);
    const long n4 = (long)a->M * (a->C4 / 4);
    const int blocks = (int)((n4 + 255) / 256 < 8192 ? (n4 + 255) / 256 : 8192);
    hipLaunchKernelGGL(k_geglu, dim3(blocks), dim3(256), 0, (hipStream_t)stream, *a);
    ES_CHECK_HIP(hipGetLastError());
    return 0;
}

static int latent_to_cl(const float* x, int O, int C, int V, int Cpad, void* out, int is_f32, es_stream stream) {
    const long n = (long)O * V * Cpad;
    const int blocks = (int)((n + 255) / 256 < 4096 ? (n + 255) / 256 : 4096);
    hipLaunchKernelGGL(k_to_cl, dim3(blocks), dim3(256), 0, (hipStream_t)stream, x, O, C, V, Cpad, (_Float16*)out, is_f32);
    ES_CHECK_HIP(hipGetLastError());
    return 0;
}
extern "C" int es_latent_to_cl_f16(const float* x, int O, int C, int V, int Cpad, void* out, es_stream stream) { return latent_to_cl(x, O, C, V, Cpad, out, 0, stream); }
extern "C" int es_latent_to_cl_f32(const float* x, int O, int C, int V, int Cpad, void* out, es_stream stream) { return latent_to_cl(x, O, C, V, Cpad, out, 1, stream); }

extern "C" int es_split_f16x3(const float* x, long M, int C, void* out, es_stream stream) {
    ES_REQUIRE(x && out && M > 0 && C > 0 && C % 4 == 0, "es_split_f16x3: M=%ld C=%d (C a multiple of 4)", M, C);
    const long n = M * (C / 4);
    const int blocks = (int)((n + 255) / 256 < 8192 ? (n + 255) / 256 : 8192);
    hipLaunchKernelGGL(k_split_f16x3, dim3(blocks), dim3(256), 0, (hipStream_t)stream, x, M, C, (_Float16*)out);
    ES_CHECK_HIP(hipGetLastError());
    return 0;
}

extern "C" int es_shape_stem(const es_stem_args* a, es_stream stream) {
    const long n1 = (long)a->O * 32 * 512, n2 = (long)a->O * 512;
    const int Cx = a->Cin ? a->Cin : 3;
    ES_REQUIRE(Cx >= 1 && Cx <= 4, "es_shape_stem: Cin=%d (3 or 4)", Cx);
    (void)n1;
    hipLaunchKernelGGL(k_stem1, dim3(64, a->O), dim3(256), (size_t)(Cx * 288 + 32 * Cx * 27) * 4, (hipStream_t)stream, *a);
    static const LdsLimits lim{{(const void*)k_stem2, 32 * 513 * 4}};
    ES_REQUIRE(lim.err == hipSuccess, "es_shape_stem: hipFuncSetAttribute failed: %s", hipGetErrorString(lim.err));
    hipLaunchKernelGGL(k_stem2, dim3((unsigned)((n2 * 8 + 255) / 256)), dim3(256), 32 * 513 * 4, (hipStream_t)stream, *a);
    ES_CHECK_HIP(hipGetLastError());
    return 0;
}

extern "C" int es_vq_lookup(const es_vq_args* a, es_stream stream) {
    ES_REQUIRE(a->n_embed > 0 && a->n_embed * 16 <= 160 * 1024 - 1024, "es_vq_lookup: n_embed=%d too large for LDS", a->n_embed);
    ES_REQUIRE(a->Cpad >= 3, "es_vq_lookup: Cpad=%d", a->Cpad);
    static const LdsLimits lim{{(const void*)k_vq_lookup, 160 * 1024 - 1024}};
    ES_REQUIRE(lim.err == hipSuccess, "es_vq_lookup: hipFuncSetAttribute failed: %s", hipGetErrorString(lim.err));
    const long M = (long)a->O * a->V;
    hipLaunchKernelGGL(k_vq_lookup, dim3((unsigned)((M + 255) / 256)), dim3(256), (size_t)a->n_embed * 16, (hipStream_t)stream, *a);
    ES_CHECK_HIP(hipGetLastError());
    return 0;
}
```

echoscene_amd/hip.py:

```python
import ctypes as C
import os

HERE = os.path.dirname(os.path.abspath(__file__))
LIB_PATH = os.path.join(HERE, 'libechoscene_hip%s.so' % os.environ.get('ES_LIB_TAG', ''))

c_f32p = C.c_void_p
c_i32p = C.c_void_p

SEG_DIRECT, SEG_GATHER, SEG_CSRMEAN, SEG_CSRSUM, SEG_CSRWAVG = 0, 1, 2, 3, 4
PRO_NONE, PRO_SILU, PRO_GN, PRO_GN_SILU, PRO_LN, PRO_GEGLU, PRO_LN_ATTN = 0, 1, 2, 3, 4, 5, 6
ACT_NONE, ACT_RELU, ACT_SILU, ACT_GEGLU, ACT_SIGMOID = 0, 1, 2, 3, 4
CONV_SAME, CONV_DOWN_HW, CONV_UP_HW, CONV_UP_DHW, CONV_DOWN_DHW = 0, 1, 2, 3, 4
CONV_DOWN_DHW_P01 = 5
EPI_NONE, EPI_GEGLU = 0, 1
(OP_LINEAR, OP_DDPM, OP_DDIM, OP_COPY, OP_CONV, OP_GN, OP_LN, OP_ATTN, OP_GEGLU, OP_TO_CL, OP_STEM) = range(1, 12)
OP_VQ = 12
OP_FORK, OP_JOIN, OP_ROWSEL = 13, 14, 15
OP_CONV_F32, OP_ATTN_F32 = 16, 17
OP_DDIM_BLEND, OP_CONV_C1 = 18, 19
OP_DDPM_KEEP = 21


class Seg(C.Structure):
    _fields_ = [('ptr', C.c_void_p), ('idx', C.c_void_p), ('ent_row', C.c_void_p), ('ent_off', C.c_void_p),
                ('step', C.c_void_p), ('step_stride', C.c_int32), ('ld', C.c_int32), ('width', C.c_int32),
                ('mode', C.c_int32), ('nslab', C.c_int32), ('slab_stride', C.c_int32), ('pre_act', C.c_int32),
                ('pro', C.c_int32), ('gamma', C.c_void_p), ('beta', C.c_void_p), ('eps', C.c_float), ('gs', C.c_int32),
                ('ent_wt', C.c_void_p)]


class LinearArgs(C.Structure):
    _fields_ = [('seg', Seg * 3), ('nseg', C.c_int32), ('M', C.c_int32), ('K', C.c_int32), ('N', C.c_int32),
                ('wpack', C.c_void_p), ('bias', C.c_void_p), ('prologue', C.c_int32), ('gamma', C.c_void_p),
                ('beta', C.c_void_p), ('eps', C.c_float), ('act', C.c_int32), ('res', C.c_void_p),
                ('res_ld', C.c_int32), ('res_nslab', C.c_int32), ('res_slab_stride', C.c_int32),
                ('res2', C.c_void_p), ('res2_ld', C.c_int32), ('res2_nslab', C.c_int32), ('res2_slab_stride', C.c_int32),
                ('out', C.c_void_p),
                ('out_ld', C.c_int32), ('nbatch', C.c_int32), ('a_bstride', C.c_int32), ('out_bstride', C.c_int32),
                ('kb_per_slice', C.c_int32), ('out_slab_stride', C.c_int32), ('fuse_next', C.c_int32),
                ('res_step', C.c_void_p), ('res_step_stride', C.c_int32), ('seg_slices', C.c_int32)]


class UpdateArgs(C.Structure):
    _fields_ = [('x', C.c_void_p), ('eps', C.c_void_p), ('eps_nslab', C.c_int32), ('eps_slab_stride', C.c_int32),
                ('noise', C.c_void_p), ('noise_stride', C.c_int32),
                ('coef', C.c_void_p), ('coef_stride', C.c_int32), ('step', C.c_void_p), ('n', C.c_int32),
                ('inc_step', C.c_int32), ('clip_x0', C.c_int32)]


class ConvArgs(C.Structure):
    _fields_ = [('a', C.c_void_p), ('w', C.c_void_p), ('O', C.c_int32), ('D', C.c_int32), ('H', C.c_int32),
                ('W', C.c_int32), ('Cin', C.c_int32), ('N', C.c_int32), ('taps', C.c_int32), ('mode', C.c_int32),
                ('a2', C.c_void_p), ('w2', C.c_void_p), ('Cin2', C.c_int32), ('bias', C.c_void_p),
                ('rowvec', C.c_void_p), ('rowvec_ld', C.c_int32), ('res', C.c_void_p), ('out_f32', C.c_void_p), ('out_f16', C.c_void_p),
                ('workspace', C.c_void_p), ('splitk', C.c_int32), ('out_ld', C.c_int32), ('O_hint', C.c_int32),
                ('epilogue', C.c_int32), ('gn_stats_out', C.c_void_p), ('gn_part_out', C.c_void_p), ('gn_part_groups', C.c_int32)]


class ConvRouteInfo(C.Structure):
    _fields_ = [('kernel', C.c_int32), ('grid_x', C.c_uint32), ('grid_y', C.c_uint32), ('grid_z', C.c_uint32)] + \
               [(f, C.c_int32) for f in ('lds', 'S', 'slabs', 'ncb', 'omax', 'epi_stats', 'stats', 'stats_pass', 'part_ok', 'reduce', 'vt',
                                         'fold_bal')]


CONV_KERNELS = ('none', 'small_n', 'small_n_tiled', 'n16', 'kw_4_1', 'kw_2_2', 'ws_256_8_4_3', 'ws_64_4_4_3', 'ws_64_4_4_6', 'ws_128_4_4_3',
                'ws_128_4_8_3', 'ws_128_4_8_5', 'ws3', 'ws_256_up_fold', 'linear_ws', 'linear_deep', 'lean_256', 'lean_128', 'lean_64')


class GNArgs(C.Structure):
    _fields_ = [('x1', C.c_void_p), ('C1', C.c_int32), ('x2', C.c_void_p), ('C2', C.c_int32), ('O', C.c_int32),
                ('V', C.c_int32), ('groups', C.c_int32), ('eps', C.c_float), ('gamma', C.c_void_p),
                ('beta', C.c_void_p), ('silu', C.c_int32), ('stats', C.c_void_p), ('y_f16', C.c_void_p),
                ('raw_f16', C.c_void_p), ('O_hint', C.c_int32), ('stats1', C.c_void_p), ('stats2', C.c_void_p), ('x1_is_f16', C.c_int32), ('y_is_f32', C.c_int32), ('part_in', C.c_void_p)]


class LNArgs(C.Structure):
    _fields_ = [('x', C.c_void_p), ('M', C.c_int32), ('C', C.c_int32), ('eps', C.c_float), ('gamma', C.c_void_p),
                ('beta', C.c_void_p), ('y_f16', C.c_void_p), ('y_is_f32', C.c_int32)]


class AttnArgs(C.Structure):
    _fields_ = [('qkv', C.c_void_p), ('B', C.c_int32), ('Ntok', C.c_int32), ('heads', C.c_int32),
                ('dhead', C.c_int32), ('scale', C.c_float), ('out_f16', C.c_void_p)]


class GegluArgs(C.Structure):
    _fields_ = [('h_f32', C.c_void_p), ('M', C.c_int32), ('C4', C.c_int32), ('out_f16', C.c_void_p), ('out_is_f32', C.c_int32)]


class RowSelArgs(C.Structure):
    _fields_ = [('table', C.c_void_p), ('stride', C.c_int32), ('step', C.c_void_p), ('out', C.c_void_p),
                ('out_ld', C.c_int32), ('rows', C.c_int32), ('n', C.c_int32)]


class CopyArgs(C.Structure):
    _fields_ = [('dst', C.c_void_p), ('src', C.c_void_p), ('bytes', C.c_size_t), ('rows', C.c_int32),
                ('dst_pitch', C.c_size_t), ('src_pitch', C.c_size_t)]


class ToClArgs(C.Structure):
    _fields_ = [('x', C.c_void_p), ('O', C.c_int32), ('C', C.c_int32), ('V', C.c_int32), ('Cpad', C.c_int32),
                ('out', C.c_void_p), ('out_is_f32', C.c_int32)]


class StemArgs(C.Structure):
    _fields_ = [('x', C.c_void_p), ('w0', C.c_void_p), ('b0', C.c_void_p), ('w1', C.c_void_p), ('b1', C.c_void_p),
                ('scratch', C.c_void_p), ('out', C.c_void_p), ('O', C.c_int32), ('Cin', C.c_int32), ('x_ostride', C.c_int32)]


class VQArgs(C.Structure):
    _fields_ = [('z', C.c_void_p), ('codebook', C.c_void_p), ('lut', C.c_void_p), ('O', C.c_int32), ('V', C.c_int32),
                ('n_embed', C.c_int32), ('Cpad', C.c_int32), ('idx_out', C.c_void_p), ('out_f16', C.c_void_p)]


class BlendArgs(C.Structure):
    _fields_ = [('x', C.c_void_p), ('x0', C.c_void_p), ('mask', C.c_void_p), ('noise', C.c_void_p), ('noise_stride', C.c_int32),
                ('tab', C.c_void_p), ('step', C.c_void_p), ('O', C.c_int32), ('n', C.c_int32)]

OP_PLMS, OP_PLMS_FIRST_A, OP_PLMS_FIRST_B = 23, 24, 25
OP_DDIM_ROWS = 27


OP_DDIM_BLEND_VOX = 28


class BlendVoxArgs(C.Structure):
    _fields_ = [('x', C.c_void_p), ('x0', C.c_void_p), ('mask', C.c_void_p), ('noise', C.c_void_p), ('noise_stride', C.c_int32),
                ('tab', C.c_void_p), ('step', C.c_void_p), ('O', C.c_int32), ('C', C.c_int32), ('V', C.c_int32)]


class PlmsArgs(C.Structure):
    _fields_ = [('x', C.c_void_p), ('eps', C.c_void_p), ('eps_nslab', C.c_int32), ('eps_slab_stride', C.c_int32),
                ('coef', C.c_void_p), ('coef_stride', C.c_int32), ('n', C.c_int32), ('step', C.c_void_p),
                ('inc_step', C.c_int32), ('ring_stride', C.c_int32), ('ring', C.c_void_p), ('xsave', C.c_void_p)]


class DdpmKeepArgs(C.Structure):
    _fields_ = [('x', C.c_void_p), ('eps', C.c_void_p), ('eps_nslab', C.c_int32), ('eps_slab_stride', C.c_int32),
                ('noise', C.c_void_p), ('noise_stride', C.c_int32),
                ('coef', C.c_void_p), ('coef_stride', C.c_int32), ('step', C.c_void_p), ('n', C.c_int32),
                ('inc_step', C.c_int32), ('clip_x0', C.c_int32),
                ('x0', C.c_void_p), ('mask', C.c_void_p), ('keep_noise', C.c_void_p), ('keep_noise_stride', C.c_int32),
                ('tab', C.c_void_p), ('n_tab', C.c_int32), ('row', C.c_int32)]


class ConvC1Args(C.Structure):
    _fields_ = [('x', C.c_void_p), ('w', C.c_void_p), ('bias', C.c_void_p), ('out_f32', C.c_void_p), ('out_f16', C.c_void_p),
                ('O', C.c_int32), ('D', C.c_int32), ('H', C.c_int32), ('W', C.c_int32), ('N', C.c_int32)]


class _OpU(C.Union):
    _fields_ = [('linear', LinearArgs), ('update', UpdateArgs), ('copy', CopyArgs), ('conv', ConvArgs),
                ('gn', GNArgs), ('ln', LNArgs), ('attn', AttnArgs), ('geglu', GegluArgs), ('tocl', ToClArgs),
                ('stem', StemArgs), ('vq', VQArgs), ('rowsel', RowSelArgs), ('blend', BlendArgs), ('conv_c1', ConvC1Args),
                ('keep', DdpmKeepArgs), ('plms', PlmsArgs), ('blend_vox', BlendVoxArgs)]


class Op(C.Structure):
    _fields_ = [('kind', C.c_int32), ('lane', C.c_int32), ('u', _OpU)]


class BufferDesc(C.Structure):
    _fields_ = [('ptr', C.c_void_p), ('bytes', C.c_size_t)]


class RegionDesc(C.Structure):
    _fields_ = [('name', C.c_char * 32), ('ptr', C.c_void_p), ('bytes', C.c_size_t)]


EXPORTS = {
    'es_abi_version': (C.c_int, []),
    'es_last_error': (C.c_char_p, []),
    'es_device_info': (C.c_int, [C.c_char_p, C.c_int, C.POINTER(C.c_int)]),
    'es_pack_linear_f32_size': (C.c_size_t, [C.c_int, C.c_int]),
    'es_pack_linear_f32': (C.c_int, [C.c_void_p, C.c_int, C.c_int, C.c_void_p]),
    'es_pack_linear_f32_dev': (C.c_int, [C.c_void_p, C.c_int, C.c_int, C.c_void_p, C.c_void_p]),
    'es_matmul_f64': (C.c_int, [C.c_void_p, C.c_void_p, C.c_void_p, C.c_int, C.c_int, C.c_int, C.c_void_p]),
    'es_pack_linear_geglu_f32': (C.c_int, [C.c_void_p, C.c_void_p, C.c_int, C.c_int, C.c_void_p, C.c_void_p]),
    'es_linear_rows_f32': (C.c_int, [C.POINTER(LinearArgs), C.c_void_p]),
    'es_linear_rows_multi_f32': (C.c_int, [C.POINTER(C.POINTER(LinearArgs)), C.c_int, C.c_void_p]),
    'es_rows_set_kernel_family': (C.c_int, [C.c_int]),
    'es_rows_get_kernel_family': (C.c_int, []),
    'es_vol_set_option': (C.c_int, [C.c_char_p, C.c_int]),
    'es_vol_options': (C.c_int, [C.c_char_p, C.c_int]),
    'es_options_string': (C.c_int, [C.c_char_p, C.c_int]),
    'es_model_file_options': (C.c_int, [C.c_char_p, C.c_char_p, C.c_int]),
    'es_linear_rows_slices': (C.c_int, [C.POINTER(LinearArgs), C.POINTER(C.c_int)]),
    'es_linear_rows_takes_ln_attn': (C.c_int, [C.POINTER(LinearArgs)]),
    'es_linear_rows_auto_slices': (C.c_int, [C.c_int, C.c_int, C.c_int]),
    'es_row_select': (C.c_int, [C.POINTER(RowSelArgs), C.c_void_p]),
    'es_ddpm_update': (C.c_int, [C.POINTER(UpdateArgs), C.c_void_p]),
    'es_ddim_update': (C.c_int, [C.POINTER(UpdateArgs), C.c_void_p]),
    'es_ddim_blend': (C.c_int, [C.POINTER(BlendArgs), C.c_void_p]),
    'es_ddim_blend_vox': (C.c_int, [C.POINTER(BlendVoxArgs), C.c_void_p]),
    'es_range_mask': (C.c_int, [C.c_void_p, C.c_int, C.c_int, C.c_int, C.c_int, C.c_void_p, C.c_void_p]),
    'es_partial_shape': (C.c_int, [C.c_void_p, C.c_void_p, C.c_int, C.c_int, C.c_float, C.c_void_p, C.c_void_p, C.c_void_p, C.c_void_p]),
    'es_conv_c1_f32': (C.c_int, [C.POINTER(ConvC1Args), C.c_void_p]),
    'es_ddpm_update_keep': (C.c_int, [C.POINTER(DdpmKeepArgs), C.c_void_p]),
    'es_ddim_rows_update': (C.c_int, [C.POINTER(DdpmKeepArgs), C.c_void_p]),
    'es_plms_update': (C.c_int, [C.POINTER(PlmsArgs), C.c_void_p]),
    'es_plms_first_a': (C.c_int, [C.POINTER(PlmsArgs), C.c_void_p]),
    'es_plms_first_b': (C.c_int, [C.POINTER(PlmsArgs), C.c_void_p]),
    'es_box_prescale': (C.c_int, [C.c_void_p, C.c_int, C.c_int, C.c_void_p, C.c_void_p, C.c_void_p, C.c_int, C.c_void_p, C.c_int,
                                  C.c_void_p]),
    'es_box_postprocess': (C.c_int, [C.c_void_p, C.c_int, C.c_void_p, C.c_void_p, C.c_void_p, C.c_int, C.c_float,
                                     C.c_void_p]),
    'es_box_descale': (C.c_int, [C.c_void_p, C.c_int, C.c_int, C.c_void_p, C.c_int, C.c_void_p]),
    'es_conv_mfma_f16': (C.c_int, [C.POINTER(ConvArgs), C.c_void_p]),
    'es_conv_emits_gn_stats': (C.c_int, [C.POINTER(ConvArgs)]),
    'es_conv_emits_gn_part': (C.c_int, [C.POINTER(ConvArgs)]),
    'es_conv_split_of': (C.c_int, [C.POINTER(ConvArgs)]),
    'es_conv_kernel_of': (C.c_int, [C.POINTER(ConvArgs), C.c_char_p, C.c_int]),
    'es_conv_fold_balanced': (C.c_int, [C.POINTER(ConvArgs)]),
    'es_conv_route_of': (C.c_int, [C.POINTER(ConvArgs), C.POINTER(ConvRouteInfo)]),
    'es_split_f16x3': (C.c_int, [C.c_void_p, C.c_long, C.c_int, C.c_void_p, C.c_void_p]),
    'es_pack_conv_f16_size': (C.c_size_t, [C.c_int, C.c_int, C.c_int]),
    'es_pack_conv_f16': (C.c_int, [C.c_void_p, C.c_int, C.c_int, C.c_int, C.c_void_p]),
    'es_pack_conv_f16_dev': (C.c_int, [C.c_void_p, C.c_int, C.c_int, C.c_int, C.c_void_p, C.c_void_p]),
    'es_pack_conv_rows_f16': (C.c_int, [C.c_void_p, C.c_int, C.c_int, C.c_int, C.c_void_p]),
    'es_pack_conv_up_fold_f16_size': (C.c_size_t, [C.c_int, C.c_int]),
    'es_pack_conv_up_fold_f16': (C.c_int, [C.c_void_p, C.c_int, C.c_int, C.c_void_p]),
    'es_pack_conv_up_fold_f16_dev': (C.c_int, [C.c_void_p, C.c_int, C.c_int, C.c_void_p, C.c_void_p]),
    'es_groupnorm_vol': (C.c_int, [C.POINTER(GNArgs), C.c_void_p]),
    'es_layernorm_tokens': (C.c_int, [C.POINTER(LNArgs), C.c_void_p]),
    'es_attention_f16': (C.c_int, [C.POINTER(AttnArgs), C.c_void_p]),
    'es_geglu_f16': (C.c_int, [C.POINTER(GegluArgs), C.c_void_p]),
    'es_latent_to_cl_f16': (C.c_int, [C.c_void_p, C.c_int, C.c_int, C.c_int, C.c_int, C.c_void_p, C.c_void_p]),
    'es_latent_to_cl_f32': (C.c_int, [C.c_void_p, C.c_int, C.c_int, C.c_int, C.c_int, C.c_void_p, C.c_void_p]),
    'es_pack_conv_f32_size': (C.c_size_t, [C.c_int, C.c_int, C.c_int]),
    'es_pack_conv_f32': (C.c_int, [C.c_void_p, C.c_int, C.c_int, C.c_int, C.c_void_p]),
    'es_conv_f32': (C.c_int, [C.POINTER(ConvArgs), C.c_void_p]),
    'es_attention_f32': (C.c_int, [C.POINTER(AttnArgs), C.c_void_p]),
    'es_shape_stem': (C.c_int, [C.POINTER(StemArgs), C.c_void_p]),
    'es_vq_lookup': (C.c_int, [C.POINTER(VQArgs), C.c_void_p]),
    'es_init': (C.c_int, []),
    'es_chamfer_forward': (C.c_int, [C.c_void_p, C.c_void_p, C.c_int, C.c_int, C.c_int, C.c_void_p, C.c_void_p, C.c_void_p,
                                     C.c_void_p, C.c_void_p]),
    'es_chamfer_backward': (C.c_int, [C.c_void_p, C.c_void_p, C.c_int, C.c_int, C.c_int, C.c_void_p, C.c_void_p, C.c_void_p,
                                      C.c_void_p, C.c_void_p, C.c_void_p, C.c_void_p]),
    'es_marching_cubes_workspace': (C.c_size_t, [C.c_int, C.c_int]),
    'es_marching_cubes_count': (C.c_int, [C.c_void_p, C.c_int, C.c_int, C.c_float, C.c_void_p, C.c_void_p, C.c_void_p,
                                          C.c_void_p]),
    'es_marching_cubes_emit': (C.c_int, [C.c_void_p, C.c_int, C.c_int, C.c_float, C.c_void_p, C.c_void_p, C.c_void_p,
                                         C.c_void_p, C.c_void_p, C.c_void_p, C.c_void_p]),
    'es_mesh_sdf_workspace': (C.c_size_t, [C.c_int, C.c_long]),
    'es_mesh_sdf': (C.c_int, [C.c_void_p, C.c_void_p, C.c_void_p, C.c_void_p, C.c_int, C.c_long, C.c_long, C.c_int, C.c_float, C.c_float,
                              C.c_void_p, C.c_void_p, C.c_void_p, C.c_void_p, C.c_void_p]),
    'es_chamfer_matrix': (C.c_int, [C.c_void_p, C.c_int, C.c_int, C.c_void_p, C.c_int, C.c_int, C.c_int, C.c_void_p, C.c_void_p]),
    'es_cloud_normalize': (C.c_int, [C.c_void_p, C.c_void_p, C.c_void_p, C.c_int, C.c_int, C.c_long, C.c_void_p, C.c_void_p, C.c_void_p]),
    'es_emd_matrix': (C.c_int, [C.c_void_p, C.c_int, C.c_void_p, C.c_int, C.c_int, C.c_int, C.c_void_p, C.c_void_p, C.c_void_p]),
    'es_emd_matrix_rounds': (C.c_int, [C.c_void_p, C.c_int, C.c_void_p, C.c_int, C.c_int, C.c_int, C.c_void_p, C.c_void_p, C.c_void_p,
                                       C.c_void_p]),
    'es_emd_max_points': (C.c_int, []),
    'es_relation_check': (C.c_int, [C.c_void_p, C.c_int, C.c_int, C.c_void_p, C.c_int, C.c_void_p, C.c_int, C.c_void_p, C.c_int, C.c_int,
                                    C.c_int, C.c_double, C.c_void_p, C.c_void_p, C.c_void_p, C.c_void_p, C.c_void_p]),
    'es_box3d_iou': (C.c_int, [C.c_void_p, C.c_int, C.c_void_p, C.c_int, C.c_int, C.c_int, C.c_void_p, C.c_void_p, C.c_void_p]),
    'es_plan_create': (C.c_void_p, [C.POINTER(Op), C.c_int]),
    'es_plan_destroy': (None, [C.c_void_p]),
    'es_plan_num_ops': (C.c_int, [C.c_void_p]),
    'es_plan_run': (C.c_int, [C.c_void_p, C.c_void_p]),
    'es_plan_capture': (C.c_int, [C.c_void_p, C.c_void_p]),
    'es_sampler_run': (C.c_int, [C.c_void_p, C.c_void_p, C.c_int, C.c_int, C.c_int, C.c_void_p]),
    'es_op_pointer_offsets': (C.c_int, [C.c_int, C.POINTER(C.c_size_t), C.c_int]),
    'es_model_save': (C.c_int, [C.c_char_p, C.c_void_p, C.POINTER(BufferDesc), C.c_int, C.POINTER(RegionDesc), C.c_int]),
    'es_model_load': (C.c_void_p, [C.c_char_p]),
    'es_model_free': (None, [C.c_void_p]),
    'es_model_region': (C.c_int, [C.c_void_p, C.c_char_p, C.POINTER(C.c_void_p), C.POINTER(C.c_size_t)]),
    'es_model_num_ops': (C.c_int, [C.c_void_p]),
    'es_model_run': (C.c_int, [C.c_void_p, C.c_int, C.c_int, C.c_void_p]),
    'es_layout_sample': (C.c_int, [C.c_void_p, C.c_void_p, C.c_int, C.c_int, C.c_void_p, C.c_void_p]),
    'es_layout_sample_keep': (C.c_int, [C.c_void_p, C.c_void_p, C.c_int, C.c_int, C.c_void_p, C.c_void_p, C.c_void_p, C.c_void_p,
                                        C.c_void_p]),
    'es_shape_sample': (C.c_int, [C.c_void_p, C.c_void_p, C.c_int, C.c_void_p, C.c_void_p]),
    'es_vq_decode': (C.c_int, [C.c_void_p, C.c_void_p, C.c_void_p, C.c_void_p]),
}

_lib = None


def lib():
    global _lib
    if _lib is None:
        import torch
        if not os.path.exists(LIB_PATH):
            raise RuntimeError(
                'libechoscene_hip.so is missing (%s). Build it with `python -m echoscene_amd.build` '
                '(hipcc --offload-arch=gfx950); there is no CPU/PyTorch fallback.' % LIB_PATH)
        L = C.CDLL(LIB_PATH)
        for name, (res, args) in EXPORTS.items():
            fn = getattr(L, name)
            fn.restype, fn.argtypes = res, args
        if L.es_abi_version() != 10:
            raise RuntimeError('libechoscene_hip.so ABI version mismatch')
        _lib = L
    return _lib


def check(rc, what=''):
    if rc != 0:
        raise RuntimeError('%s failed (status %d): %s' % (what or 'echoscene_hip call', rc,
                                                          lib().es_last_error().decode()))


def current_stream():
    import torch
    return C.c_void_p(torch.cuda.current_stream().cuda_stream)


def ptr(t):
    return None if t is None else C.c_void_p(t.data_ptr())
```

echoscene_amd/plan_vol.py:

```python
import ctypes as C
import os
import torch

from . import hip
from .hip import ConvArgs, GNArgs, LNArgs, AttnArgs, GegluArgs, ToClArgs, StemArgs, BlendArgs, BlendVoxArgs, ConvC1Args, Op
from .plan import (Builder, PackedLinear, GCNWeights, View, seg, emit_gcn, own, mm64)


VOL_FOLD_FFO = True
VOL_GN_F16 = True
VOL_GN_PART_FUSED = True
VOL_GN_RG_ANY = False


def _gn_rg():
    buf = C.create_string_buffer(512)
    hip.lib().es_vol_options(buf, 512)
    opts = dict(kv.split('=') for kv in buf.value.decode().strip(';').split(';'))
    return int(opts.get('gn_rg', '1')) != 0


def up_fold_weights(W):
    W = W.detach().double().cpu()
    assert W.dim() == 5 and tuple(W.shape[2:]) == (3, 3, 3)
# ... 82 lines not shown
            pad = torch.zeros((W.shape[0], cp - cin) + tuple(W.shape[2:]), dtype=W.dtype, device=W.device)
            W = torch.cat([W, pad], 1)
        hi = W.half().float()
        lo = (W - hi).half().float()
        super().__init__(torch.cat([hi, hi, lo], 1), b, device, geglu=False)
        self.cin_part, self.cin_true = cp, cin
        self.weight_bytes = self.N * cin * self.taps * 6


class UNet3DWeights:
    def __init__(self, sd, net, device, precision='fp16'):
        self.precision = precision
        PackedConv = globals()[{'fp32': 'PackedConv32', 'fp32x': 'PackedConvX3'}.get(precision, 'PackedConv')]
        self.device, self.mc, self.topo = device, net.model_channels, net.topo
        self.enable_t_emb, self.mp = net.enable_t_emb, net.messsage_passing
        self.heads = net.num_heads
        self.concat = bool(getattr(net, 'concat', False))
        dv = lambda k: own(sd[k], device)
        PL = lambda w, b: PackedLinear(sd[w], sd[b] if b else None, device)
        PC = lambda w, b: PackedConv(sd[w], sd[b] if b else None, device)
        self.te0 = PL('time_embed.0.weight', 'time_embed.0.bias')
        self.te2 = PL('time_embed.2.weight', 'time_embed.2.bias')
        self.shape_t = None
        if self.mp:
            self.stem = [dv('shape_embeddings.0.weight'), dv('shape_embeddings.0.bias'),
                         dv('shape_embeddings.2.weight'), dv('shape_embeddings.2.bias')]
            self.stem_lin = PL('shape_embeddings.5.weight', 'shape_embeddings.5.bias')
            self.shape_t = PL('shape_time_emb.weight', 'shape_time_emb.bias') if net.enable_t_emb else None
            self.pred_table = sd['pred_embeddings.weight'].detach().float().cpu()
            self.gcn = GCNWeights(sd, 'shape_code_graph_cov', device)
        inp, mid, out = net.topo
        names = [(f'input_blocks.{i}.{j}', it) for i, blk in enumerate(inp) for j, it in enumerate(blk)]
        names += [(f'middle_block.{j}', it) for j, it in enumerate(mid)]
        names += [(f'output_blocks.{i}.{j}', it) for i, blk in enumerate(out) for j, it in enumerate(blk)]
        self.items, self.emb_slices, self.ca = {}, {}, {}
        emb_w, emb_b, ca_v, ca_b, off = [], [], [], [], 0
        for name, it in names:
            kind, d = it[0], {}
            if kind == 'conv_in':
                d['conv'] = PC(name + '.weight', name + '.bias')
            elif kind == 'res':
                d['gn1'] = (dv(name + '.in_layers.0.weight'), dv(name + '.in_layers.0.bias'))
                d['conv1'] = PC(name + '.in_layers.2.weight', name + '.in_layers.2.bias')
                d['gn2'] = (dv(name + '.out_layers.0.weight'), dv(name + '.out_layers.0.bias'))
                d['conv2'] = PC(name + '.out_layers.3.weight', name + '.out_layers.3.bias')
                if (name + '.skip_connection.weight') in sd:
                    d['skip'] = PackedConv(sd[name + '.skip_connection.weight'].flatten(1), None, device)
                    d['bias2'] = (sd[name + '.out_layers.3.bias'].float() +
                                  sd[name + '.skip_connection.bias'].float()).contiguous().to(device)
                emb_w.append(sd[name + '.emb_layers.1.weight'])
                emb_b.append(sd[name + '.emb_layers.1.bias'])
                self.emb_slices[name] = (off, it[2])
                off += it[2]
            elif kind == 'attn' and self.concat:
                Cc = it[1]
                ch = Cc // self.heads
                perm = torch.cat([torch.cat([torch.arange(h * 3 * ch + part * ch, h * 3 * ch + (part + 1) * ch)
                                             for h in range(self.heads)]) for part in range(3)])
                d['gn'] = (dv(name + '.norm.weight'), dv(name + '.norm.bias'))
                d['qkv'] = PackedConv(sd[name + '.qkv.weight'].flatten(1)[perm], sd[name + '.qkv.bias'][perm], device)
                d['proj_out'] = PackedConv(sd[name + '.proj_out.weight'].flatten(1), sd[name + '.proj_out.bias'], device)
            elif kind == 'attn':
                tb = name + '.transformer_blocks.0'
                d['gn'] = (dv(name + '.norm.weight'), dv(name + '.norm.bias'))
                d['proj_in'] = PackedConv(sd[name + '.proj_in.weight'].flatten(1), sd[name + '.proj_in.bias'], device)
                d['ln1'] = (dv(tb + '.norm1.weight'), dv(tb + '.norm1.bias'))
                d['ln3'] = (dv(tb + '.norm3.weight'), dv(tb + '.norm3.bias'))
                d['qkv'] = PackedConv(torch.cat([sd[tb + '.attn1.to_q.weight'], sd[tb + '.attn1.to_k.weight'],
                                                 sd[tb + '.attn1.to_v.weight']], 0), None, device)
                d['o1'] = PC(tb + '.attn1.to_out.0.weight', tb + '.attn1.to_out.0.bias')
                d['o2'] = PL(tb + '.attn2.to_out.0.weight', tb + '.attn2.to_out.0.bias')
                d['ff1'] = PackedConv(sd[tb + '.ff.net.0.proj.weight'], sd[tb + '.ff.net.0.proj.bias'], device, geglu=True)
                d['ff2'] = PC(tb + '.ff.net.2.weight', tb + '.ff.net.2.bias')
                d['proj_out'] = PackedConv(sd[name + '.proj_out.weight'].flatten(1), sd[name + '.proj_out.bias'], device)
                if VOL_FOLD_FFO:
                    W2, b2 = sd[tb + '.ff.net.2.weight'].double(), sd[tb + '.ff.net.2.bias'].double()
                    Wp, bp = sd[name + '.proj_out.weight'].flatten(1).double(), sd[name + '.proj_out.bias'].double()
                    d['ffo'] = PackedConv(mm64(Wp, W2).float(), None, device)
                    d['po'] = PackedConv(Wp.float(), None, device)
                    d['ffo_bias'] = (mm64(Wp, b2) + bp).float().contiguous().to(device)
                self.ca[name] = (len(ca_v), it[1])
                ca_v.append(mm64(sd[tb + '.attn2.to_out.0.weight'], sd[tb + '.attn2.to_v.weight']).float())
                ca_b.append(sd[tb + '.attn2.to_out.0.bias'])
            elif kind == 'down':
                d['conv'] = PC(name + '.op.weight', name + '.op.bias')
            elif kind == 'up':
                if precision == 'fp16' and not self.concat:
                    d['conv'] = PackedConv(sd[name + '.conv.weight'], sd[name + '.conv.bias'], device, up_fold=True)
                else:
                    d['conv'] = PC(name + '.conv.weight', name + '.conv.bias')
            self.items[name] = d
        self.emb_all = PackedLinear(torch.cat(emb_w, 0), torch.cat(emb_b, 0), device)
        self.cav_all = None if self.concat else PackedLinear(torch.cat(ca_v, 0), torch.cat(ca_b, 0), device)
        self.out_gn = (dv('out.0.weight'), dv('out.0.bias'))
        self.out_conv = PC('out.2.weight', 'out.2.bias')
        self.in_ch, self.out_ch = net.in_channels, net.out_channels


class VolBuilderMixin:

    def _push(self, kind, field, a):
        op = Op()
        op.kind, op.lane = kind, 0
        setattr(op.u, field, a)
        self.ops.append(op)
        return len(self.ops) - 1

    def conv(self, a_f16, pc, O, dims, mode=hip.CONV_SAME, bias=None, rowvec=None, res=None, out_f32=None,
             out_f16=None, skip=None, ncdhw=False, splitk=None, epilogue=0, out_ld=None, w_fold=None):
        D, H, W = dims
        assert w_fold is None or (skip is None and mode == hip.CONV_UP_HW)
        if getattr(self, 'fp32x', False) and a_f16.dtype == torch.float32:
            assert isinstance(pc, PackedConvX3) and not epilogue
            a3 = self.split3(a_f16, pc.cin_part)
            if skip is not None:
                skip = (self.split3(skip[0], skip[1].cin_part), skip[1])
            out = out_f32 if out_f32 is not None else out_f16
            assert out is not None and out.dtype == torch.float32 and (out_f32 is None or out_f16 is None)
            return self.conv(a3, pc, O, dims, mode=mode, bias=bias, rowvec=rowvec, res=res, out_f32=out, skip=skip, ncdhw=ncdhw,
                             splitk=splitk, out_ld=out_ld)
        if getattr(self, 'fp32', False) and not getattr(self, 'fp32x', False):
            return self._conv32(a_f16, pc, O, dims, mode, bias, rowvec, res, out_f32, out_f16, skip, ncdhw, out_ld)
        a = ConvArgs()
        a.a, a.w = a_f16.data_ptr(), pc.w.data_ptr()
        a.O, a.D, a.H, a.W = O, D, H, W
        a.Cin, a.N, a.taps, a.mode = pc.Cin, pc.N, pc.taps, mode
        if skip is not None:
            a.a2, a.w2, a.Cin2 = skip[0].data_ptr(), skip[1].w.data_ptr(), skip[1].Cin
            self.weight_bytes += skip[1].weight_bytes
            self.flops += 2 * O * D * H * W * skip[1].Cin * pc.N
        bt = pc.b if bias is None else bias
        a.bias = bt.data_ptr() if bt is not None else None
        if rowvec is not None:
            a.rowvec, a.rowvec_ld = rowvec.ptr, rowvec.ld
        a.res = res.data_ptr() if res is not None else None
        a.out_f32 = out_f32.data_ptr() if out_f32 is not None else None
        a.out_f16 = out_f16.data_ptr() if out_f16 is not None else None
        a.out_ld = -1 if ncdhw else (pc.N if out_ld is None else out_ld)
        a.epilogue = epilogue
        a.O_hint = int(getattr(self, 'o_hint', 0) or 0)
        M = O * D * H * W
        Mh = (-a.O_hint if a.O_hint < 0 else max(a.O_hint, O)) * D * H * W
        folded = False
        if w_fold is not None:
            a.w2 = w_fold.data_ptr()
            self.keep.append(w_fold)
            name = C.create_string_buffer(32)
            if hip.lib().es_conv_kernel_of(C.byref(a), name, 32) < 0:
                raise RuntimeError('es_conv_kernel_of: ' + hip.lib().es_last_error().decode())
            folded = name.value == b'ws_256_up_fold'
        if not folded and not ncdhw and Mh * pc.N <= 8192 * 5376 and pc.N % 4 == 0 and not epilogue:
            a.splitk = -1 if splitk is None else splitk
            a.workspace = 1
            S = hip.lib().es_conv_split_of(C.byref(a))
            if S < 0:
                raise RuntimeError('es_conv_split_of: ' + hip.lib().es_last_error().decode())
            need = max(S, splitk or 0, 1) * M * pc.N
            if getattr(self, '_ws', None) is None or self._ws.numel() < need:
                self._ws = self.buf(need, scratch=True)
                for op in self.ops:
                    if op.kind == hip.OP_CONV and op.u.conv.workspace:
                        op.u.conv.workspace = self._ws.data_ptr()
            a.workspace = self._ws.data_ptr()
        self.keep += [pc, bt, skip]
        self.weight_bytes += pc.weight_bytes
        self.flops += 2 * O * D * H * W * pc.cin_true * pc.taps * pc.N
        idx = self._push(hip.OP_CONV, 'conv', a)
        if out_f32 is not None and not ncdhw and not epilogue and (out_ld is None or out_ld == pc.N):
            if not hasattr(self, '_conv_of'):
                self._conv_of = {}
            self._conv_of[out_f32.data_ptr()] = (idx, M, pc.N)
        return idx

    def split3(self, x32, C):
        rows = x32.numel() // C
        out = self.buf(rows, 3 * C, dtype=torch.float16, scratch=True)
        a = ToClArgs()
        a.x, a.O, a.C, a.V, a.Cpad, a.out, a.out_is_f32 = x32.data_ptr(), rows, C, 1, C, out.data_ptr(), 2
        self._push(hip.OP_TO_CL, 'tocl', a)
        return out

    def _conv32(self, a32, pc, O, dims, mode, bias, rowvec, res, out_f32, out_f16, skip, ncdhw, out_ld):
        D, H, W = dims
        assert isinstance(pc, PackedConv32) and a32.dtype == torch.float32
        a = ConvArgs()
        a.a, a.w = a32.data_ptr(), pc.w.data_ptr()
        a.O, a.D, a.H, a.W = O, D, H, W
        a.Cin, a.N, a.taps, a.mode = pc.Cin, pc.N, pc.taps, mode
        if skip is not None:
            a.a2, a.w2, a.Cin2 = skip[0].data_ptr(), skip[1].w.data_ptr(), skip[1].Cin
            self.flops += 2 * O * D * H * W * skip[1].Cin * pc.N
        bt = pc.b if bias is None else bias
        a.bias = bt.data_ptr() if bt is not None else None
        if rowvec is not None:
            a.rowvec, a.rowvec_ld = rowvec.ptr, rowvec.ld
        a.res = res.data_ptr() if res is not None else None
        out = out_f32 if out_f32 is not None else out_f16
        assert out is not None and out.dtype == torch.float32 and (out_f32 is None or out_f16 is None)
        a.out_f32 = out.data_ptr()
        a.out_ld = -1 if ncdhw else (pc.N if out_ld is None else out_ld)
        self.keep += [pc, bt, skip]
        self.weight_bytes += pc.weight_bytes
        self.flops += 2 * O * D * H * W * pc.cin_true * pc.taps * pc.N
        return self._push(hip.OP_CONV_F32, 'conv', a)

    def _rowgroup_producer(self, x, Cx, M, V):
        if not _gn_rg() or V % 64 or x is None:
            return None
        ent = getattr(self, '_conv_of', {}).get(x.data_ptr())
        if ent is None or ent[1] != M or ent[2] != Cx:
            return None
        op = self.ops[ent[0]]
        if op.kind != hip.OP_CONV or op.u.conv.out_f32 != x.data_ptr():
            return None
        if not VOL_GN_RG_ANY:
            q = ConvArgs.from_buffer_copy(op.u.conv)
            if q.O_hint > q.O or q.O_hint < 0:
                q.O, q.O_hint = abs(q.O_hint), 0
            if hip.lib().es_conv_emits_gn_stats(C.byref(q)) != 1:
                return None
        return op

    def _rowgroup_stats(self, op, x, Cx, M):
        st = getattr(self, '_rg_stats', None)
        if st is None:
            st = self._rg_stats = {}
        ent = st.get(x.data_ptr())
        if ent is None or ent[0] is not op:
            buf = self.buf(2 * (M // 64) * Cx, scratch=True)
            op.u.conv.gn_stats_out = buf.data_ptr()
            st[x.data_ptr()] = ent = (op, buf)
        assert op.u.conv.gn_stats_out == ent[1].data_ptr() and op.u.conv.out_f32 == x.data_ptr()
        return ent[1]

    def conv_gn_intermediate(self, a_f16, pc, O, dims, rowvec=None):
        D, H, W = dims
        M, V = O * D * H * W, D * H * W
        if getattr(self, 'fp32', False):
            h32 = self.buf(M, pc.N, scratch=True)
            self.conv(a_f16, pc, O, dims, rowvec=rowvec, out_f32=h32)
            return h32
        h16 = self.buf(M, pc.N, dtype=torch.float16, scratch=True)
        idx = self.conv(a_f16, pc, O, dims, rowvec=rowvec, out_f16=h16)
        op = self.ops[idx]
        L = hip.lib()
        if V % 64 == 0 and _gn_rg() and VOL_GN_F16:
            whole = ConvArgs.from_buffer_copy(op.u.conv)
            if whole.O_hint > whole.O or whole.O_hint < 0:
                whole.O, whole.O_hint = abs(whole.O_hint), 0
            if L.es_conv_emits_gn_stats(C.byref(whole)) == 1:
                st = self.buf(2 * (M // 64) * pc.N, scratch=True)
                op.u.conv.gn_stats_out = st.data_ptr()
                if L.es_conv_emits_gn_stats(C.byref(op.u.conv)) != 1:
                    h32 = self.buf(M, pc.N, scratch=True)
                    op.u.conv.out_f32 = h32.data_ptr()
                    self.keep.append(h32)
                if not hasattr(self, '_f16_stats'):
                    self._f16_stats = {}
                self._f16_stats[h16.data_ptr()] = st
                return h16
        h32 = self.buf(M, pc.N, scratch=True)
        op.u.conv.out_f32, op.u.conv.out_f16 = h32.data_ptr(), None
        self.scratch.discard(h16.data_ptr())
        self.keep[:] = [t for t in self.keep if t is not h16]
        del h16
        if not hasattr(self, '_conv_of'):
            self._conv_of = {}
        self._conv_of[h32.data_ptr()] = (idx, M, pc.N)
        return h32

    def groupnorm(self, x1, C1, x2, C2, O, V, gamma, beta, eps, silu, y_f16, raw_f16=None, groups=32):
        a = GNArgs()
        a.x1, a.C1 = x1.data_ptr(), C1
        a.x2, a.C2 = (x2.data_ptr(), C2) if x2 is not None else (None, 0)
        a.O, a.V, a.groups, a.eps = O, V, groups, eps
        a.gamma, a.beta, a.silu = gamma.data_ptr(), beta.data_ptr(), int(silu)
        need = O * ((V + 7) // 8) * groups * 2 + O * groups * 2
        st = getattr(self, '_gn_stats', None)
        if st is None or st.numel() < need:
            st = self._gn_stats = self.buf(need, scratch=True)
        a.stats = st.data_ptr()
        a.y_f16 = y_f16.data_ptr()
        a.raw_f16 = raw_f16.data_ptr() if raw_f16 is not None else None
        a.O_hint = int(getattr(self, 'o_hint', 0) or 0)
        if getattr(self, 'fp32', False):
            assert y_f16.dtype == torch.float32 and (raw_f16 is None or raw_f16.dtype == torch.float32)
            a.y_is_f32 = 1
            self.keep += [gamma, beta]
            return self._push(hip.OP_GN, 'gn', a)
        if x1.dtype == torch.float16:
            assert x2 is None and raw_f16 is None
            a.x1_is_f16 = 1
            a.stats1 = self._f16_stats[x1.data_ptr()].data_ptr()
            self.keep += [gamma, beta]
            return self._push(hip.OP_GN, 'gn', a)
        p1 = self._rowgroup_producer(x1, C1, O * V, V)
        p2 = self._rowgroup_producer(x2, C2, O * V, V) if x2 is not None else None
        if p1 is not None and (x2 is None or p2 is not None):
            a.stats1 = self._rowgroup_stats(p1, x1, C1, O * V).data_ptr()
            a.stats2 = self._rowgroup_stats(p2, x2, C2, O * V).data_ptr() if x2 is not None else None
        elif x2 is None and VOL_GN_PART_FUSED:
            ent = getattr(self, '_conv_of', {}).get(x1.data_ptr())
            if ent is not None and ent[1] == O * V and ent[2] == C1:
                op = self.ops[ent[0]]
                cv = op.u.conv
                if op.kind == hip.OP_CONV and cv.out_f32 == x1.data_ptr() and not cv.gn_part_out and not cv.gn_stats_out:
# ... 577 lines not shown
```

echoscene_amd/samplers.py:

```python
import math
import os

import torch

from . import hip
from .plan import (Builder, GraphIndex, View, GCNWeights, UNet1DWeights, emit_gcn, emit_unet1d_step, time_tables, sub_plan)
from .plan_vol import UNet3DWeights, emit_unet3d_step, VQWeights, emit_vq_decode, VQEncWeights, emit_vq_encode
from .schedules import LayoutSchedule, LayoutDdimSchedule, ShapeSchedule, timestep_embedding_table, SHAPE_SAMPLERS, LAYOUT_SAMPLERS


def _cap(n_triples):
    return max(32, (int(n_triples) + 31) // 32 * 32)


def state_dict_for(module, device=None):
    dev = None if device is None else torch.device(device)
    on_dev = lambda v: dev is not None and dev.type == 'cuda' and v.is_cuda and (dev.index is None or v.device.index == dev.index)
    return {k: (v.detach() if on_dev(v) else v.detach().cpu()) for k, v in module.state_dict().items()}


def _cpu_sd(module):
    return state_dict_for(module, None)


# ... 106 lines not shown


def _check_mask(x0, mask, shape, loop, form, unit, per=1):
    mask = torch.as_tensor(mask, dtype=torch.float32)
    mask = mask.reshape(-1) if per == 1 else mask
    x0 = torch.as_tensor(x0)
    if mask.numel() != shape[0] * per or tuple(x0.shape) != tuple(shape):
        raise ValueError('%s: x0 must be %s = %s and mask [O]; got %s and %d entries' % (loop, form, tuple(shape), tuple(x0.shape), mask.numel()))
    if not bool(((mask == 0) | (mask == 1)).all()):
        raise ValueError('%s: the mask is per %s, 0 (generate) or 1 (keep)' % (loop, unit))
    return x0, mask


def _check_shape_mask(x0, mask, O, z_shape):
    z_shape = tuple(int(d) for d in z_shape)
    zd = z_shape[1:]
    m = torch.as_tensor(mask, dtype=torch.float32)
    if tuple(m.shape) in ((O, 1) + zd, (O,) + zd, (O, math.prod(zd))):
        return _check_mask(x0, m.reshape(O, -1), (O,) + z_shape, 'masked DDIM', '[O, C, D, H, W]', 'voxel', per=math.prod(zd)) + (True,)
    if m.numel() != O:
        raise ValueError('masked DDIM: the mask is per object, [O] = [%d], or per latent voxel, [O, 1, D, H, W] / [O, D, H, W] with '
                         '(D, H, W) = %s -- one value for all channels; got %s (a mask per channel is not supported)'
                         % (O, zd, tuple(m.shape)))
    return _check_mask(x0, m, (O,) + z_shape, 'masked DDIM', '[O, C, D, H, W]', 'object') + (False,)


class LayoutDenoiser:

    def __init__(self, net, diffusion_kwargs, device=None, sampler='ddpm', steps=None, eta=0.0, weights=None):
        if sampler not in LAYOUT_SAMPLERS:
            raise ValueError('layout_sampler must be one of %s, got %r' % (LAYOUT_SAMPLERS, sampler))
        if sampler == 'ddpm' and (steps is not None or float(eta or 0.0) != 0.0):
            raise ValueError("layout_steps / layout_eta need layout_sampler='ddim' (the ancestral loop runs every trained timestep)")
        if sampler == 'ddim' and steps is None:
            raise ValueError("layout_sampler='ddim' needs layout_steps")
        self.sampler, self.eta = sampler, float(eta or 0.0)
        self.device = device or torch.device('cuda')
        self.net = net
        dk = dict(diffusion_kwargs)
        if sampler == 'ddim' and dk.get('model_mean_type', 'eps') != 'eps':
            raise ValueError("layout DDIM: model_mean_type=%r has no reference arithmetic under DDIM" % (dk.get('model_mean_type'),))
        self.w = weights if weights is not None else UNet1DWeights(state_dict_for(net, self.device), net, self.device)
        self.sched = LayoutSchedule(dk.get('time_num', 1000), dk.get('beta_start', 1e-4), dk.get('beta_end', 0.02),
                                    dk.get('schedule_type', 'linear'), dk.get('model_mean_type', 'eps'),
                                    dk.get('model_var_type', 'fixedsmall'))
        self.T = self.sched.time_num
        if sampler == 'ddim':
            self.sched = LayoutDdimSchedule(self.sched, steps, self.eta)
        self.n_iter = len(self.sched.timesteps)
        self.temb = timestep_embedding_table(self.sched.timesteps, net.model_channels).to(self.device)
        self.coef = self.sched.coef.to(self.device)
        self.keep_tab = self.sched.keep_tab.to(self.device)
        self.tables = time_tables(self.w, self.temb, self.w.box_t, self.device)
        self._plans, self._last, self.max_plans = {}, None, 4

    def _plan_for(self, obj_embed, triples, clip=False, keep=False):
        O = obj_embed.shape[0]
        cap = _cap(triples.shape[0])
        key = (O, cap) + (('clip',) if clip else ()) + (('keep',) if keep else ())
        sig = hash(triples.detach().cpu().numpy().tobytes())
        st = self._plans.get(key)
        if st is None:
            g = GraphIndex(triples, O, self.device, capacity=cap)
            b = Builder(self.device)
            bufs = emit_layout_step(b, self.w, g, obj_embed, self.temb, self.tables, self.n_iter, self.coef, self.keep_tab, clip, keep,
                                    sampler=self.sampler, step_noise=self.sampler == 'ddpm' or self.eta != 0.0)
            n_eps_ops = bufs.pop('n_eps_ops')
            st = new_state(plan=b.finish(), eps_plan=sub_plan(b, b.ops[:n_eps_ops]), g=g, sig=sig, **bufs)
            if len(self._plans) >= self.max_plans:
                self._plans.pop(next(iter(self._plans)))
            self._plans[key] = st
        elif st['sig'] != sig:
            st['g'].update(triples)
            st['pred'].copy_(self.w.pred_table[torch.from_numpy(st['g'].p_host)])
            st['sig'] = sig
        st['objbuf'][:, :st['oe_w']].copy_(obj_embed.to(self.device))
        self._last = st
        return st

    @property
    def weight_bytes_per_step(self):
        return self._last['plan'].weight_bytes

    def save_model(self, path, obj_embed, triples, keep=False):
        from .plan import save_model
        st = self._plan_for(obj_embed, triples, keep=keep)
        regions = dict(x=st['x'], noise=st['noise'], step=st['step'], coef=self.coef)
        if keep:
            regions.update(x0=st['x0'], mask=st['mask'], knoise=st['knoise'], ktab=self.keep_tab)
        return save_model(st['plan'], path, regions)

    def eps(self, x, obj_embed, triples, iteration):
        st = self._plan_for(obj_embed, triples)
        st['x'].copy_(x.to(self.device))
        st['eps_plan'].sample(st['step'], int(iteration), 1, use_graph=False)
        torch.cuda.synchronize()
        return st['eps'].value()

    def _fill_keep(self, st, x0, mask, keep_noise):
        O, D = st['x'].shape
        x0, mask = _check_mask(x0, mask, (O, D), 'masked layout loop', '[O, %d]' % D, 'node')
        n = self.n_iter
        if keep_noise is not None and (keep_noise.dim() < 2 or keep_noise.shape[0] < n or keep_noise[0].numel() != O * D):
            raise ValueError('masked layout loop: keep_noise must be [T, O, %d] with T = %d' % (D, n))
        st['x0'].copy_(x0.to(self.device).float())
        st['mask'].copy_(mask.to(self.device))
        if keep_noise is None:
            st['knoise'].normal_()
        else:
            st['knoise'].copy_(keep_noise.to(self.device).float()[:n].reshape(n, O * D))

    def _prime_keep(self, st):
        O, D = st['x'].shape
        a = hip.BlendArgs()
        a.x, a.x0, a.mask, a.noise = st['x'].data_ptr(), st['x0'].data_ptr(), st['mask'].data_ptr(), st['knoise'].data_ptr()
        a.noise_stride, a.tab, a.step, a.O, a.n = O * D, self.keep_tab.data_ptr(), st['step'].data_ptr(), O, D
        st['step'].zero_()
        import ctypes
        hip.check(hip.lib().es_ddim_blend(ctypes.byref(a), hip.current_stream()), 'es_ddim_blend')

    def stage(self, obj_embed, triples, noise=None, x0=None, mask=None, keep_noise=None, clip=False, prime=True):
        _check_keep_pair(x0, mask, keep_noise, 'the masked layout loop')
        st = self._plan_for(obj_embed, triples, clip=clip, keep=mask is not None)
        if mask is not None:
            self._fill_keep(st, x0, mask, keep_noise)
        if noise is None:
            st['noise'].normal_()
        else:
            st['noise'][:noise.shape[0]].copy_(noise.to(self.device))
        st['x'].copy_(st['noise'][0])
        if mask is not None and prime:
            self._prime_keep(st)
        return st

    def sample(self, obj_embed, triples, noise=None, n_steps=None, use_graph=True, clip_denoised=False, x0=None, mask=None,
               keep_noise=None):
        if self.sampler == 'ddim' and clip_denoised:
            raise ValueError('layout DDIM: clip_denoised=True has no reference arithmetic under DDIM (p_sample_ddim never clips)')
        n_steps = self.n_iter if n_steps is None else n_steps
        if not 0 <= n_steps <= self.n_iter:
            raise ValueError('n_steps must be in [0, %d] (the iterations of the schedule), got %r' % (self.n_iter, n_steps))
        st = self.stage(obj_embed, triples, noise, x0, mask, keep_noise, clip=bool(clip_denoised), prime=n_steps > 0)
        st['plan'].sample(st['step'], 0, n_steps, use_graph=use_graph)
        return st['x'].clone()


CANON_OBJECTS = 4


class ShapeDenoiser:

    def __init__(self, df, model_params=None, ddim_steps=100, device=None, z_shape=(3, 16, 16, 16), rank=0, world=1,
                 group=None, deterministic=False, force_exchange=False, precision='fp16', ddim_eta=0.0, sampler='ddim', weights=None,
                 up_fold=True):
        if precision not in ('fp16', 'fp32', 'fp32x'):
            raise ValueError("precision must be 'fp16', 'fp32' or 'fp32x'")
        if sampler not in SHAPE_SAMPLERS:
            raise ValueError('sampler must be one of %s, got %r' % (SHAPE_SAMPLERS, sampler))
        self.sampler = sampler
        self.precision = precision
        self.force_exchange = bool(force_exchange)
        self.device = device or torch.device('cuda')
        self.df = df
        net = df.diffusion_net
        self.net = net
        if weights is not None:
            if getattr(weights, 'precision', None) != precision:
                raise ValueError('weights were packed for precision %r, this denoiser asks for %r' % (getattr(weights, 'precision', None), precision))
            self.w = weights
        else:
            sd = {k[len('diffusion_net.'):]: v for k, v in state_dict_for(df, self.device).items()}
            self.w = UNet3DWeights(sd, net, self.device, precision)
        mp = dict(model_params or {})
        self.ddim_eta = float(ddim_eta)
        self.sched = ShapeSchedule(ddim_steps, mp.get('timesteps', 1000), mp.get('linear_start', 0.00085),
                                   mp.get('linear_end', 0.012), eta=self.ddim_eta)
        self.S = len(self.sched.timesteps)
        if sampler == 'plms':
            self._check_plms()
        self.z_shape = tuple(z_shape)
        self.per = math.prod(int(d) for d in self.z_shape)
        self.temb = timestep_embedding_table(self.sched.timesteps, net.model_channels).to(self.device)
        self.coef = self.sched.coef.to(self.device)
        self.keep_tab = self.sched.keep_tab.to(self.device)
        self.rank, self.world, self.group = rank, world, group
        self.deterministic = deterministic
        self.up_fold = bool(up_fold)
        self.tables = time_tables(self.w, self.temb, self.w.shape_t, self.device)
        self._plans, self.max_plans = {}, 2
        self._cur, self._use_graph = None, True
        self._fused, self._fused_key = None, None

    def _check_plms(self):
        if self.ddim_eta != 0.0:
            raise ValueError('ddim_eta must be 0 for PLMS')
        if self.S < 2:
            raise ValueError('PLMS needs at least 2 timesteps (ddim_steps=%d yields %d)' % (self.S, self.S))

    def _sampler_of(self, sampler):
        sampler = self.sampler if sampler is None else sampler
        if sampler not in SHAPE_SAMPLERS:
            raise ValueError('sampler must be one of %s, got %r' % (SHAPE_SAMPLERS, sampler))
        if sampler == 'plms':
            self._check_plms()
        return sampler

    def _insert_plan(self, key, st):
        while len(self._plans) >= self.max_plans:
            old = self._plans.pop(next(iter(self._plans)))
            if self._fused_key is not None and old['plan'] is not None and self._fused_key[1] == id(old['plan']):
                self._fused, self._fused_key = None, None
        self._plans[key] = st

    def fused_plan(self, layout_plan, ss, r):
        from .plan import combine_plans
        key = (id(layout_plan), id(ss['plan']), r)
        if self._fused_key != key:
            self._fused, self._fused_key = combine_plans(self.device, ss['plan'], layout_plan, side_repeat=r), key
        return self._fused

    def _build_state(self, uc, triples, c, O, cap, keep, sampler, sig):
        from .parallel import partition
        lo, hi, block = partition(O, self.world, self.rank)
        if hi == lo:
            z = lambda *sh: torch.zeros(*sh, device=self.device)
            return new_state(empty=True, x=z(0, *self.z_shape), eps=z(0, *self.z_shape), lo=lo, hi=hi, O=O, codes_local=z(block, 64),
                             codes_all=z(block * self.world, 64), sig=sig, sampler=sampler)
        g = GraphIndex(triples, O, self.device, capacity=cap)
        b = Builder(self.device)
        b.shard_block = block
        b.force_exchange = self.force_exchange
        b.up_fold = self.up_fold and not self.deterministic
        if self.deterministic:
            b.o_hint = -CANON_OBJECTS
        plms = sampler == 'plms'
        bufs = emit_shape_step(b, self.w, g, uc, self.temb, self.tables, self.coef, self.keep_tab, self.S, self.z_shape, lo, hi,
                               c_local=None if c is None else c[lo:hi], gather_rows=block * self.world, keep=bool(keep), plms=plms,
                               step_noise=self.ddim_eta != 0.0, keep_vox=keep == 'vox')
        ops = compose_step_plans(b.ops, bufs.pop('n_blend'), bufs.pop('split'), bufs.pop('n_eps_ops'), *bufs.pop('first_ops'), plms=plms,
                                 sharded=(self.world > 1 or self.force_exchange) and self.w.mp)
        st = new_state(lo=lo, hi=hi, O=O, g=g, sig=sig, sampler=sampler, **bufs)
        made = {id(ops['plan']): b.finish()}
        for name in SUB_PLANS:
            if ops[name] is not None:
                if id(ops[name]) not in made:
                    made[id(ops[name])] = sub_plan(b, ops[name])
                st[name] = made[id(ops[name])]
        return st

    def _plan_for(self, uc, triples, c=None, keep=False, sampler=None):
        uc = uc.reshape(uc.shape[0], -1)
        O = uc.shape[0]
        concat = self.w.concat
        if concat or not self.w.mp:
            if c is None:
                raise ValueError("this shape denoiser needs the conditioning c_s (concat: [O, 4096], echo2shape.py:234-235; "
                                 "no message passing: the cross-attention key [O, 1, context_dim])")
            c = c.reshape(O, -1).to(self.device).float()
        else:
            c = None
        cap = _cap(triples.shape[0])
        sampler = self._sampler_of(sampler)
        key = ((O, cap, 'keepvox' if keep == 'vox' else 'keep') if keep else (O, cap)) + (('plms',) if sampler == 'plms' else ())
        sig = hash(triples.detach().cpu().numpy().tobytes())
        st = self._plans.get(key)
        if st is None:
            st = self._build_state(uc, triples, c, O, cap, keep, sampler, sig)
            self._insert_plan(key, st)
        elif st['sig'] != sig and not st['empty']:
            st['g'].update(triples)
            if st['pred'] is not None:
                st['pred'].copy_(self.w.pred_table[torch.from_numpy(st['g'].p_host)])
            st['sig'] = sig
        if st['empty']:
            return st
        if st['objbuf'] is not None:
            st['objbuf'][:, :st['ucw']].copy_(uc.to(self.device))
        if concat:
            st['xc'][:, 3].copy_(c[st['lo']:st['hi']])
        elif st['cdev'] is not None:
            st['cdev'].copy_(c[st['lo']:st['hi']])
        return st

    def passes(self, i):
        return 2 if (self._cur['sampler'] == 'plms' and int(i) == 0) else 1

    def codes_local(self, i, p=0):
        st = self._cur
        if not st['empty']:
            plan, first = (st['stem2_plan'], 1) if p else (st['stem_plan'], int(i))
            plan.sample(st['step'], first, 1, use_graph=self._use_graph)
        return st['codes_local']

    def gather_buffers(self):
        st = self._cur
        return st['codes_local'], st['codes_all']

    def step(self, i, codes_all, p=0):
        st = self._cur
        if st['empty']:
            return
        if codes_all.data_ptr() != st['codes_all'].data_ptr():
            st['codes_all'][:codes_all.shape[0]].copy_(codes_all)
        plan, first = st['main_plan'], int(i)
        if st['sampler'] == 'plms' and int(i) == 0:
            plan, first = (st['main_b_plan'], 1) if p else (st['main_a_plan'], 0)
        plan.sample(st['step'], first, 1, use_graph=self._use_graph)

    def latents_local(self):
        return self._cur['x']

    def save_model(self, path, uc, triples, c=None, keep=False):
        from .plan import save_model
        if self.sampler == 'plms':
            raise NotImplementedError("model files hold the DDIM loop only (es_shape_sample); sampler='plms' has no C host yet")
        assert self.world == 1 and not self.force_exchange
        st = self._plan_for(uc, triples, c, keep=keep)
        regions = dict(x=st['x'], step=st['step'], coef=self.coef)
        if keep:
            regions.update(x0=st['x0'], mask=st['mask'], keep_noise=st['knoise'])
        if st['snoise'] is not None:
            regions['step_noise'] = st['snoise']
        return save_model(st['plan'], path, regions)

    def step_graph(self, group=None):
        st = self._cur
        if st['sampler'] == 'plms':
            return None
        if not self._use_graph or (st['stem_plan'] is None and not st['empty']) or os.environ.get('ES_STEP_GRAPH', '0') != '1':
            return None
        if 'step_graph' in st:
            return st['step_graph']
        st['step_graph'] = None
        import torch.distributed as dist
        if not dist.is_initialized() or dist.get_backend(group) != 'nccl':
            return None
        send, recv = st['codes_local'], st['codes_all']
        g, ok = None, 1
        dist.all_gather_into_tensor(recv, send, group=group)
        torch.cuda.synchronize(self.device)
        if not st['empty']:
            try:
                s = torch.cuda.Stream(device=self.device)
                s.wait_stream(torch.cuda.current_stream(self.device))
                with torch.cuda.stream(s):
                    g = torch.cuda.CUDAGraph()
                    with torch.cuda.graph(g, stream=s):
                        st['stem_plan'].run()
                        dist.all_gather_into_tensor(recv, send, group=group)
                        st['main_plan'].run()
                torch.cuda.current_stream(self.device).wait_stream(s)
            except Exception as e:
                import warnings
                warnings.warn('sharded DDIM step: the RCCL exchange could not be captured on rank %d (%s)' % (self.rank, e))
                g, ok = None, 0
        flag = torch.tensor([ok], dtype=torch.int32, device=self.device)
        dist.all_reduce(flag, op=dist.ReduceOp.MIN, group=group)
        if int(flag.item()) != 1:
            g = None
        st['step_graph'] = g
        return g

    def begin(self, first_step):
        self._cur['step'].fill_(int(first_step))

    def eps(self, x, uc, triples, iteration, c=None):
        assert self.world == 1
        st = self._plan_for(uc, triples, c)
        st['x'].copy_(x.to(self.device))
        st['eps_plan'].sample(st['step'], int(iteration), 1, use_graph=False)
        return st['eps'].clone()

    @staticmethod
    def _run_loop(st, n_steps, use_graph):
        if st['sampler'] == 'plms':
            if n_steps > 0:
                st['first_plan'].sample(st['step'], 0, 1, use_graph=use_graph)
                st['plan'].sample(st['step'], 1, n_steps - 1, use_graph=use_graph)
        else:
            st['plan'].sample(st['step'], 0, n_steps, use_graph=use_graph)

    def _fill_table(self, st, name, given):
        O, lo, hi = st['O'], st['lo'], st['hi']
        if given is None and self.world > 1:
            given = torch.randn(self.S, O, self.per, device=self.device)
# ... 182 lines not shown
```

include/echoscene_hip.h:

```cpp
#ifndef ECHOSCENE_HIP_H
#define ECHOSCENE_HIP_H

#include <stddef.h>
#include <stdint.h>

#ifdef __cplusplus
extern "C" {
#endif

typedef void* es_stream;
typedef struct es_plan es_plan;

#define ES_ABI_VERSION 10
int es_abi_version(void);
const char* es_last_error(void);
int es_device_info(char* name_out, int name_cap, int* cu_count);

enum { ES_SEG_DIRECT = 0, ES_SEG_GATHER = 1, ES_SEG_CSRMEAN = 2, ES_SEG_CSRSUM = 3, ES_SEG_CSRWAVG = 4 };
enum { ES_PRO_NONE = 0, ES_PRO_SILU = 1, ES_PRO_GN = 2, ES_PRO_GN_SILU = 3, ES_PRO_LN = 4, ES_PRO_GEGLU = 5, ES_PRO_LN_ATTN = 6 };
enum { ES_ACT_NONE = 0, ES_ACT_RELU = 1, ES_ACT_SILU = 2, ES_ACT_GEGLU = 3, ES_ACT_SIGMOID = 4 };

typedef struct es_seg {
    const float* ptr;
    const int32_t* idx;
// ... 44 lines not shown
size_t es_pack_linear_f32_size(int N, int K);
int es_pack_linear_f32(const float* h_w, int N, int K, float* h_out);
int es_pack_linear_f32_dev(const float* d_w, int N, int K, float* d_out, es_stream stream);
int es_matmul_f64(const double* d_a, const double* d_b, double* d_c, int N, int K, int M, es_stream stream);
int es_pack_linear_geglu_f32(const float* h_w, const float* h_bias, int Nh, int K, float* h_out, float* h_bias_out);

int es_linear_rows_f32(const es_linear_args* args, es_stream stream);
int es_linear_rows_multi_f32(const es_linear_args* const* args, int n, es_stream stream);
int es_rows_set_kernel_family(int family);
int es_rows_get_kernel_family(void);

int es_vol_set_option(const char* name, int value);
int es_vol_options(char* out, int cap);
int es_options_string(char* out, int cap);
int es_model_file_options(const char* path, char* out, int cap);
int es_linear_rows_slices(const es_linear_args* args, int* kb_per_slice);
int es_linear_rows_takes_ln_attn(const es_linear_args* args);
int es_linear_rows_auto_slices(int K, int N, int kalign_cols);

typedef struct es_update_args {
    float* x;
    const float* eps;
    int32_t eps_nslab, eps_slab_stride;
    const float* noise;
    int32_t noise_stride;
    const float* coef;
    int32_t coef_stride;
    int32_t* step;
    int32_t n;
    int32_t inc_step;
    int32_t clip_x0;
} es_update_args;
int es_ddpm_update(const es_update_args* args, es_stream stream);
int es_box_postprocess(float* boxes, int ld, const float* sincos, float* angle_out, const float* stats,
                       int O, float angle_scale, es_stream stream);
int es_box_descale(float* boxes, int ld, int ncol, const float* stats, int O, es_stream stream);
int es_ddim_update(const es_update_args* args, es_stream stream);
typedef struct es_blend_args {
    float* x;
    const float* x0;
    const float* mask;
    const float* noise;
    int32_t noise_stride;
    const float* tab;
    const int32_t* step;
    int32_t O, n;
} es_blend_args;
int es_ddim_blend(const es_blend_args* args, es_stream stream);
typedef struct es_blend_vox_args {
    float* x;
    const float* x0;
    const float* mask;
    const float* noise;
    int32_t noise_stride;
    const float* tab;
    const int32_t* step;
    int32_t O, C, V;
} es_blend_vox_args;
int es_ddim_blend_vox(const es_blend_vox_args* args, es_stream stream);
int es_range_mask(const int32_t* bounds, int K, int D, int H, int W, float* mask, es_stream stream);
int es_partial_shape(const float* sdf, const int32_t* bounds, int K, int n, float fill, float* shape_part, float* shape_missing,
                     uint8_t* shape_mask, es_stream stream);
typedef struct es_plms_args {
    float* x;
    const float* eps;
    int32_t eps_nslab, eps_slab_stride;
    const float* coef;
    int32_t coef_stride;
    int32_t n;
    int32_t* step;
    int32_t inc_step;
    int32_t ring_stride;
    float* ring;
    float* xsave;
} es_plms_args;
int es_plms_update(const es_plms_args* args, es_stream stream);
int es_plms_first_a(const es_plms_args* args, es_stream stream);
int es_plms_first_b(const es_plms_args* args, es_stream stream);
typedef struct es_ddpm_keep_args {
    float* x;
    const float* eps;
    int32_t eps_nslab, eps_slab_stride;
    const float* noise;
    int32_t noise_stride;
    const float* coef;
    int32_t coef_stride;
    int32_t* step;
    int32_t n;
    int32_t inc_step;
    int32_t clip_x0;
    const float* x0;
    const float* mask;
    const float* keep_noise;
    int32_t keep_noise_stride;
    const float* tab;
    int32_t n_tab;
    int32_t row;
} es_ddpm_keep_args;
int es_ddpm_update_keep(const es_ddpm_keep_args* args, es_stream stream);
int es_ddim_rows_update(const es_ddpm_keep_args* args, es_stream stream);
int es_box_prescale(const float* boxes, int ld, int ncol, const float* angles, const double* stats, float* out, int out_ld,
                    float* sincos_out, int O, es_stream stream);

enum { ES_CONV_SAME = 0, ES_CONV_DOWN_HW = 1, ES_CONV_UP_HW = 2, ES_CONV_UP_DHW = 3, ES_CONV_DOWN_DHW = 4,
       ES_CONV_DOWN_DHW_P01 = 5 };

typedef struct es_conv_args {
    const void* a;
    const void* w;
    int32_t O, D, H, W;
    int32_t Cin, N;
    int32_t taps;
    int32_t mode;
    const void* a2; const void* w2; int32_t Cin2;
    const float* bias;
    const float* rowvec;
    int32_t rowvec_ld;
    const float* res;
    float* out_f32;
    void* out_f16;
    void* workspace;
    int32_t splitk;
    int32_t out_ld;
    int32_t O_hint;
    int32_t epilogue;
    float* gn_stats_out;
    float* gn_part_out;
    int32_t gn_part_groups;
} es_conv_args;
enum { ES_EPI_NONE = 0, ES_EPI_GEGLU = 1 };
int es_conv_mfma_f16(const es_conv_args* args, es_stream stream);
int es_conv_emits_gn_stats(const es_conv_args* args);
int es_conv_emits_gn_part(const es_conv_args* args);
int es_conv_split_of(const es_conv_args* args);
int es_conv_kernel_of(const es_conv_args* args, char* name_out, int cap);
int es_conv_fold_balanced(const es_conv_args* args);
typedef struct es_conv_route_info {
    int32_t kernel;
    uint32_t grid_x, grid_y, grid_z;
    int32_t lds;
    int32_t S;
    int32_t slabs;
    int32_t ncb;
    int32_t omax;
    int32_t epi_stats;
    int32_t stats;
    int32_t stats_pass;
    int32_t part_ok;
    int32_t reduce;
    int32_t vt;
    int32_t fold_bal;
} es_conv_route_info;
int es_conv_route_of(const es_conv_args* args, es_conv_route_info* out);
int es_split_f16x3(const float* x, long M, int C, void* out, es_stream stream);
size_t es_pack_conv_f16_size(int N, int Cin, int taps);
int es_pack_conv_f16(const float* h_w, int N, int Cin, int taps, uint16_t* h_out);
int es_pack_conv_f16_dev(const float* d_w, int N, int Cin, int taps, uint16_t* d_out, es_stream stream);
int es_pack_conv_rows_f16(const float* h_w, int N, int Cin, int taps, uint16_t* h_out);
size_t es_pack_conv_up_fold_f16_size(int N, int Cin);
int es_pack_conv_up_fold_f16(const float* h_w, int N, int Cin, uint16_t* h_out);
int es_pack_conv_up_fold_f16_dev(const float* d_w, int N, int Cin, uint16_t* d_out, es_stream stream);

typedef struct es_gn_args {
    const float* x1; int32_t C1;
    const float* x2; int32_t C2;
    int32_t O, V;
    int32_t groups; float eps;
    const float* gamma; const float* beta;
    int32_t silu;
    float* stats;
    void* y_f16;
    void* raw_f16;
    int32_t O_hint;
    const float* stats1;
    const float* stats2;
    int32_t x1_is_f16;
    int32_t y_is_f32;
    const float* part_in;
} es_gn_args;
int es_groupnorm_vol(const es_gn_args* args, es_stream stream);

typedef struct es_ln_args {
    const float* x; int32_t M, C; float eps; const float* gamma; const float* beta; void* y_f16;
    int32_t y_is_f32;
} es_ln_args;
int es_layernorm_tokens(const es_ln_args* args, es_stream stream);

typedef struct es_attn_args {
    const void* qkv;
    int32_t B, Ntok, heads, dhead;
    float scale;
    void* out_f16;
} es_attn_args;
int es_attention_f16(const es_attn_args* args, es_stream stream);

typedef struct es_geglu_args { const float* h_f32; int32_t M, C4; void* out_f16; int32_t out_is_f32; } es_geglu_args;
int es_geglu_f16(const es_geglu_args* args, es_stream stream);

size_t es_pack_conv_f32_size(int N, int Cin, int taps);
int es_pack_conv_f32(const float* h_w, int N, int Cin, int taps, float* h_out);
int es_conv_f32(const es_conv_args* args, es_stream stream);
int es_attention_f32(const es_attn_args* args, es_stream stream);

typedef struct es_vq_args {
    const float* z;
    const float* codebook;
    const float* lut;
    int32_t O, V, n_embed, Cpad;
    int32_t* idx_out;
    void* out_f16;
} es_vq_args;
int es_vq_lookup(const es_vq_args* args, es_stream stream);

typedef struct es_conv_c1_args {
    const float* x;
    const float* w;
    const float* bias;
    float* out_f32;
    void* out_f16;
    int32_t O, D, H, W, N;
} es_conv_c1_args;
int es_conv_c1_f32(const es_conv_c1_args* args, es_stream stream);

int es_latent_to_cl_f16(const float* x_ncdhw, int O, int C, int V, int Cpad, void* out_f16, es_stream s);
int es_latent_to_cl_f32(const float* x_ncdhw, int O, int C, int V, int Cpad, void* out_f32, es_stream s);
typedef struct es_stem_args {
    const float* x;
    const float* w0; const float* b0;
    const float* w1; const float* b1;
    float* scratch;
    float* out;
    int32_t O;
    int32_t Cin;
    int32_t x_ostride;
} es_stem_args;
int es_shape_stem(const es_stem_args* args, es_stream stream);


enum {
    ES_OP_LINEAR = 1, ES_OP_DDPM = 2, ES_OP_DDIM = 3, ES_OP_COPY = 4, ES_OP_CONV = 5, ES_OP_GN = 6,
    ES_OP_LN = 7, ES_OP_ATTN = 8, ES_OP_GEGLU = 9, ES_OP_TO_CL = 10, ES_OP_STEM = 11, ES_OP_VQ = 12,
    ES_OP_FORK = 13, ES_OP_JOIN = 14, ES_OP_ROWSEL = 15,
    ES_OP_CONV_F32 = 16, ES_OP_ATTN_F32 = 17,
    ES_OP_DDIM_BLEND = 18,
    ES_OP_CONV_C1 = 19,
    ES_OP_DDPM_KEEP = 21,
    ES_OP_PLMS = 23, ES_OP_PLMS_FIRST_A = 24, ES_OP_PLMS_FIRST_B = 25,
    ES_OP_DDIM_ROWS = 27,
    ES_OP_DDIM_BLEND_VOX = 28
};
typedef struct es_rowsel_args {
    const float* table; int32_t stride;
    const int32_t* step;
    float* out; int32_t out_ld, rows, n;
} es_rowsel_args;
int es_row_select(const es_rowsel_args* args, es_stream stream);

typedef struct es_copy_args {
    void* dst; const void* src; size_t bytes;
    int32_t rows; size_t dst_pitch, src_pitch;
} es_copy_args;
typedef struct es_tocl_args { const float* x; int32_t O, C, V, Cpad; void* out; int32_t out_is_f32; } es_tocl_args;
typedef struct es_op {
    int32_t kind;
    int32_t lane;
    union {
        es_linear_args linear; es_update_args update; es_copy_args copy; es_conv_args conv;
        es_gn_args gn; es_ln_args ln; es_attn_args attn; es_geglu_args geglu; es_tocl_args tocl;
        es_stem_args stem; es_vq_args vq; es_rowsel_args rowsel; es_blend_args blend; es_conv_c1_args conv_c1;
        es_ddpm_keep_args keep; es_plms_args plms; es_blend_vox_args blend_vox;
    } u;
} es_op;

es_plan* es_plan_create(const es_op* ops, int n_ops);
void es_plan_destroy(es_plan* plan);
int es_plan_num_ops(const es_plan* plan);
int es_plan_run(es_plan* plan, es_stream stream);
int es_plan_capture(es_plan* plan, es_stream stream);
int es_chamfer_forward(const float* xyz1, const float* xyz2, int batch, int n, int m, float* dist1, int32_t* idx1,
                       float* dist2, int32_t* idx2, es_stream stream);
int es_chamfer_backward(const float* xyz1, const float* xyz2, int batch, int n, int m, const float* graddist1,
                        const float* graddist2, const int32_t* idx1, const int32_t* idx2, float* gradxyz1,
                        float* gradxyz2, es_stream stream);

size_t es_marching_cubes_workspace(int O, int n);
int es_marching_cubes_count(const float* sdf, int O, int n, float level, const int8_t* tri_table, void* workspace,
                            int32_t* counts, es_stream stream);
int es_marching_cubes_emit(const float* sdf, int O, int n, float level, const int8_t* tri_table, void* workspace,
                           const int64_t* vert_offset, const int64_t* tri_offset, float* verts, int32_t* faces,
                           es_stream stream);

size_t es_mesh_sdf_workspace(int K, long total_T);
int es_mesh_sdf(const float* verts, const int32_t* faces, const int64_t* vert_offset, const int64_t* tri_offset, int K,
                long total_V, long total_T, int n, float trunc, float fit, void* workspace, int32_t* bad_flags,
                float* transform, float* sdf, es_stream stream);

int es_chamfer_matrix(const float* a, int Na, int P, const float* b, int Nb, int Q, int symmetric, float* out, es_stream stream);
int es_cloud_normalize(const float* verts, const int64_t* vert_offset, const int32_t* index, int K, int number, long total_V,
                       int32_t* bad_flags, float* out, es_stream stream);

int es_emd_matrix(const float* a, int Na, const float* b, int Nb, int P, int symmetric, float* out, int32_t* status, es_stream stream);
int es_emd_matrix_rounds(const float* a, int Na, const float* b, int Nb, int P, int symmetric, float* out, int32_t* status,
                         int32_t* rounds, es_stream stream);
int es_emd_max_points(void);

int es_relation_check(const float* boxes, int O, int ld, const int64_t* triples, int T, const int8_t* rule_of_pred, int n_pred,
// ... 30 lines not shown
```

Before: 59.15.

## Add boundary-class conv kernel that skips zero-padded taps in small 3D convs

Adds a ws_256_cls conv kernel for 3x3x3 SAME convs on small H*W planes. It groups output voxels by their (h,w) boundary class and issues only the taps that land inside the volume, so MFMA work on zero padding is skipped. Work pieces are ordered longest-first for load balance, with a per-class split-K chosen on the host. Partial sums go to the split workspace through a new slab store. This adds a class-indexed row mapping and a new schedule path, enabled by default through pad_skip for fp16, non-deterministic, single-device runs.

Result: no change. 59.46, median of 6 (+0.5%).

```diff
diff --git a/echoscene_amd/csrc/es_conv_route.h b/echoscene_amd/csrc/es_conv_route.h
--- a/echoscene_amd/csrc/es_conv_route.h
+++ b/echoscene_amd/csrc/es_conv_route.h
@@ -18,9 +18,10 @@
     none,
     small_n, small_n_tiled, n16, kw_4_1, kw_2_2, ws_256_8_4_3, ws_64_4_4_3, ws_64_4_4_6, ws_128_4_4_3, ws_128_4_8_3, ws_128_4_8_5, ws3,
     ws_256_up_fold,
-    linear_ws, linear_deep, lean_256, lean_128, lean_64
+    linear_ws, linear_deep, lean_256, lean_128, lean_64,
+    ws_256_cls
 };
-extern const char* const kConvKernelName[(int)ConvKernel::lean_64 + 1];
+extern const char* const kConvKernelName[(int)ConvKernel::ws_256_cls + 1];
 enum class ConvReduce { none, plain, gn_part };
 
 enum class SplitRule {
@@ -36,6 +37,22 @@
     auto128,
     none
 };
+
+constexpr unsigned cls_tap_mask(int H, int W, int h, int w) {
+    const unsigned vw = (w >= 1 ? 1u : 0u) | 2u | (w + 1 < W ? 4u : 0u);
+    const unsigned vh = (h >= 1 ? 1u : 0u) | 2u | (h + 1 < H ? 4u : 0u);
+    const unsigned m9 = ((vh & 1u) ? vw : 0u) | ((vh & 2u) ? vw << 3 : 0u) | ((vh & 4u) ? vw << 6 : 0u);
+    return m9 | m9 << 9 | m9 << 18;
+}
+constexpr int CLS_MAX_CLASSES = 64, CLS_MAX_SPLIT = 4;
+struct ConvClsSched {
+    int ntm;
+    uint32_t pair[CLS_MAX_CLASSES * CLS_MAX_SPLIT / 4];
+};
+void conv_cls_piece(int nv, int kch0, int kch2, int bz, int S, int* ks_begin, int* ks_end);
+int conv_cls_order(int H, int W, int kch0, int kch2, int S, int ntm, ConvClsSched* s);
+int conv_cls_longest(int H, int W, int kch0, int kch2, int S);
+int conv_cls_choose_split(int H, int W, int kch0, int kch2, int slab_cap);
 
 struct ConvRoute {
     ConvGeom g;
@@ -58,6 +75,7 @@
     bool stats_pass;
     int slabs;
     bool fold_bal;
+    ConvClsSched cls;
 };
 
 struct RouteOptions {
diff --git a/echoscene_amd/csrc/es_conv_route.hip b/echoscene_amd/csrc/es_conv_route.hip
--- a/echoscene_amd/csrc/es_conv_route.hip
+++ b/echoscene_amd/csrc/es_conv_route.hip
@@ -8,7 +8,8 @@
 const char* const kConvKernelName[] = {
     "none",
     "small_n", "small_n_tiled", "n16", "kw_4_1", "kw_2_2", "ws_256_8_4_3", "ws_64_4_4_3", "ws_64_4_4_6", "ws_128_4_4_3", "ws_128_4_8_3", "ws_128_4_8_5", "ws3",
-    "ws_256_up_fold", "linear_ws", "linear_deep", "lean_256", "lean_128", "lean_64"
+    "ws_256_up_fold", "linear_ws", "linear_deep", "lean_256", "lean_128", "lean_64",
+    "ws_256_cls"
 };
 
 #ifndef ES_CONV_A3_DEFAULT
@@ -320,9 +321,31 @@
     }
 }
 
-bool choose_tile(const es_conv_args& a, const RouteOptions& o, const LaunchSize& L, ConvRoute* r) {
+int cls_split(const es_conv_args& a, const LaunchSize& L, const RefSize& R, const ConvRoute& r) {
+    const int forced = a.splitk <= -12 && a.splitk >= -10 - CLS_MAX_SPLIT ? -a.splitk - 10 : 0;
+    if (!(forced || (a.splitk == -2 && r.rule == SplitRule::rows256))) return 0;
+    const long rho = (long)a.O * a.D;
+    if (!(a.taps == 27 && a.mode == ES_CONV_SAME && a.O_hint == 0 && a.epilogue == ES_EPI_NONE && L.ws && L.can_split && !L.forced_bm &&
+          rho % 256 == 0 && a.H * a.W >= 2 && a.H * a.W <= CLS_MAX_CLASSES)) return 0;
+    const int kch0 = a.Cin / 32, kch2 = a.a2 ? a.Cin2 / 32 : 0;
+    if (forced) {
+        const unsigned corner = cls_tap_mask(a.H, a.W, 0, 0);
+        return forced <= R.slab_cap && keep_units(forced, __builtin_popcount(corner) * kch0 + kch2, 3) == forced ? forced : 0;
+    }
+    const int s = conv_cls_choose_split(a.H, a.W, kch0, kch2, R.slab_cap);
+    return s >= 3 ? s : 0;
+}
+
+bool choose_tile(const es_conv_args& a, const RouteOptions& o, const LaunchSize& L, ConvRoute* r, bool cls) {
     r->ncb = 1;
     r->gy = (unsigned)L.ntn; r->gz = (unsigned)r->S;
+    if (cls) {
+        r->kernel = ConvKernel::ws_256_cls;
+        const int ntm = (int)((long)a.O * a.D / 256);
+        r->gx = (unsigned)(a.H * a.W * ntm);
+        conv_cls_order(a.H, a.W, a.Cin / 32, a.a2 ? a.Cin2 / 32 : 0, r->S, ntm, &r->cls);
+        return false;
+    }
     if (r->rule == SplitRule::forced_tile) { forced_tile(o, L, r); return L.forced_bm == 128; }
     if (r->rule == SplitRule::deep) {
         r->kernel = ConvKernel::linear_deep;
@@ -388,9 +411,61 @@
     r->geglu = a.epilogue == ES_EPI_GEGLU;
     ES_REQUIRE(!r->upm || (!a.a2 && a.taps == 27), "es_conv_mfma_f16: nearest-up modes take 3x3x3 convs without a fused skip");
     const LaunchSize L = launch_size(a, o, *r);
-    choose_split(a, o, L, ref_size(a, o), r);
-    route_flags(a, choose_tile(a, o, L, r), r);
+    const RefSize R = ref_size(a, o);
+    choose_split(a, o, L, R, r);
+    const int scls = cls_split(a, L, R, *r);
+    if (scls) r->S = r->slabs = scls;
+    route_flags(a, choose_tile(a, o, L, r, scls != 0), r);
     return 0;
+}
+
+void conv_cls_piece(int nv, int kch0, int kch2, int bz, int S, int* ks_begin, int* ks_end) {
+    const int nks0 = nv * kch0, U0 = nks0 / 3, UT = U0 + kch2;
+    const int ub = (int)((long)UT * bz / S), ue = (int)((long)UT * (bz + 1) / S);
+    *ks_begin = ub <= U0 ? ub * 3 : nks0 + (ub - U0);
+    *ks_end = ue <= U0 ? ue * 3 : nks0 + (ue - U0);
+}
+
+namespace {
+struct ClsPair { int len, cls, bz; };
+int cls_pairs(int H, int W, int kch0, int kch2, int S, ClsPair* p) {
+    int n = 0;
+    for (int c = 0; c < H * W; ++c)
+        for (int bz = 0; bz < S; ++bz) {
+            int b, e;
+            conv_cls_piece(__builtin_popcount(cls_tap_mask(H, W, c / W, c % W)), kch0, kch2, bz, S, &b, &e);
+            p[n++] = {e - b, c, bz};
+        }
+    std::stable_sort(p, p + n, [](const ClsPair& x, const ClsPair& y) { return x.len > y.len; });
+    return n;
+}
+}
+
+int conv_cls_order(int H, int W, int kch0, int kch2, int S, int ntm, ConvClsSched* s) {
+    ClsPair p[CLS_MAX_CLASSES * CLS_MAX_SPLIT];
+    *s = ConvClsSched{};
+    if (H * W > CLS_MAX_CLASSES || S > CLS_MAX_SPLIT || S < 1) return 0;
+    const int n = cls_pairs(H, W, kch0, kch2, S, p);
+    s->ntm = ntm;
+    for (int i = 0; i < n; ++i) s->pair[i >> 2] |= (uint32_t)(p[i].cls << 2 | p[i].bz) << ((i & 3) * 8);
+    return n;
+}
+
+int conv_cls_longest(int H, int W, int kch0, int kch2, int S) {
+    ClsPair p[CLS_MAX_CLASSES * CLS_MAX_SPLIT];
+    return H * W <= CLS_MAX_CLASSES && S >= 1 && S <= CLS_MAX_SPLIT && cls_pairs(H, W, kch0, kch2, S, p) ? p[0].len : 0;
+}
+
+constexpr int CLS_MAX_CHAIN = 200;
+int conv_cls_choose_split(int H, int W, int kch0, int kch2, int slab_cap) {
+    if (H * W > CLS_MAX_CLASSES) return 0;
+    const int corner = __builtin_popcount(cls_tap_mask(H, W, 0, 0)) * kch0 + kch2;
+    int best = 0;
+    for (int S = 2; S <= CLS_MAX_SPLIT && S <= slab_cap && keep_units(S, corner, 24) == S; ++S) {
+        best = S;
+        if (S >= 3 && conv_cls_longest(H, W, kch0, kch2, S) <= CLS_MAX_CHAIN) break;
+    }
+    return best;
 }
 
 extern "C" int es_conv_route_of(const es_conv_args* a, es_conv_route_info* out) {
@@ -419,6 +494,20 @@
     if (name_out && cap > 0) snprintf(name_out, (size_t)cap, "%s", i.omax ? "chunked" : kConvKernelName[i.kernel]);
     return i.S > 1 ? i.S : 1;
 }
+extern "C" int es_conv_cls_order(int H, int W, int kch0, int kch2, int S, unsigned char* pairs_out, int cap) {
+    ConvClsSched s;
+    const int n = conv_cls_order(H, W, kch0, kch2, S, 1, &s);
+    for (int i = 0; i < n && i < cap; ++i) pairs_out[i] = (unsigned char)((s.pair[i >> 2] >> ((i & 3) * 8)) & 255u);
+    return n;
+}
+extern "C" unsigned es_conv_cls_tap_mask(int H, int W, int cls) { return cls_tap_mask(H, W, cls / W, cls % W); }
+extern "C" int es_conv_cls_piece(int H, int W, int cls, int kch0, int kch2, int bz, int S, int* ks_begin, int* ks_end) {
+    conv_cls_piece(__builtin_popcount(cls_tap_mask(H, W, cls / W, cls % W)), kch0, kch2, bz, S, ks_begin, ks_end);
+    return 0;
+}
+extern "C" int es_conv_cls_choose_split(int H, int W, int kch0, int kch2, int slab_cap) {
+    return conv_cls_choose_split(H, W, kch0, kch2, slab_cap);
+}
 extern "C" int es_conv_fold_balanced(const es_conv_args* a) {
     es_conv_route_info i;
     return es_conv_route_of(a, &i) == 0 ? i.fold_bal : -1;
diff --git a/echoscene_amd/csrc/es_vol.hip b/echoscene_amd/csrc/es_vol.hip
--- a/echoscene_amd/csrc/es_vol.hip
+++ b/echoscene_amd/csrc/es_vol.hip
@@ -1004,10 +1004,57 @@
     }
 }
 
-template <int BM_, int NC_, int NP_, bool UP_, int EPI_, bool STATS_, int NS_ = 3, bool FOLD_ = false>
+template <int BM_, int NW_, bool ACTIVE>
+__device__ __forceinline__ void conv_cls_store_slab(const es_conv_args& a, const ConvGeom& g, f4 (&acc)[BM_ / (NW_ / 2) / 16][7], char* smem,
+                                                    long M, long m0, int n0, int wave, int lane, int bz, int cls) {
+    constexpr int WROWS = BM_ / (NW_ / 2), MI = WROWS / 16;
+    if constexpr (!ACTIVE) {
+        __syncthreads();
+        return;
+    }
+    typedef unsigned int u4v __attribute__((ext_vector_type(4)));
+    constexpr unsigned OOBV = 0x80000000u;
+    const int wm = wave >> 1, wn = wave & 1, i16 = lane & 15, q = lane >> 4;
+    __syncthreads();
+    float* slab = (float*)smem + wave * (16 * 116);
+    const int lhw = g.lw + g.lh;
+    const long R = M >> lhw;
+    const int c4 = lane % 28, rsub = lane / 28;
+    const int n = n0 + wn * 112 + c4 * 4;
+    const bool n_ok = lane < 56 && n < a.N;
+    const long mw0 = m0 + wm * WROWS;
+    const int rows_left = (int)((R - mw0) < (long)WROWS ? (R - mw0 > 0 ? R - mw0 : 0) : (long)WROWS);
+    float* const o32 = (float*)a.workspace + (long)bz * M * a.N + ((mw0 << lhw) + cls) * (long)a.N;
+    const __amdgpu_buffer_rsrc_t rO32 = __builtin_amdgcn_make_buffer_rsrc(uniform_ptr(o32), (short)0, (int)OOBV, 0x00020000);
+    const unsigned rstride = ((unsigned)a.N << lhw) * 4u;
+    const int rsub_l = lane < 56 ? rsub : 0;
+    const unsigned vrow32 = n_ok ? (unsigned)rsub * rstride + (unsigned)n * 4u : OOBV;
+    auto write_slab = [&](int i) __attribute__((always_inline)) {
+#pragma unroll
+        for (int j = 0; j < 7; ++j)
+#pragma unroll
+            for (int r = 0; r < 4; ++r) slab[(q * 4 + r) * 116 + j * 16 + i16] = acc[i][j][r];
+    };
+    write_slab(0);
+#pragma unroll
+    for (int i = 0; i < MI; ++i) {
+        __builtin_amdgcn_s_waitcnt(0xc07f);
+        __builtin_amdgcn_wave_barrier();
+#pragma unroll
+        for (int t = 0; t < 8; ++t) {
+            const bool ok = n_ok && i * 16 + rsub + 2 * t < rows_left;
+            const f4 v = *(const f4*)&slab[(rsub_l + 2 * t) * 116 + c4 * 4];
+            __builtin_amdgcn_raw_buffer_store_b128(__builtin_bit_cast(u4v, v), rO32, (int)(ok ? vrow32 + (unsigned)(i * 16 + 2 * t) * rstride : OOBV), 0, 0);
+        }
+        __builtin_amdgcn_wave_barrier();
+        if (i + 1 < MI) write_slab(i + 1);
+    }
+}
+
+template <int BM_, int NC_, int NP_, bool UP_, int EPI_, bool STATS_, int NS_ = 3, bool FOLD_ = false, bool CLS_ = false>
 __device__ __forceinline__ void conv_ws_tile(const es_conv_args& a, const ConvGeom& g, int ncdhw, char* smem, const int wave, const int lane,
                                              const long M, const int bx, const int by, const int ks_begin, const int ks_end,
-                                             const int S, const int bz, unsigned long long* stamp) {
+                                             const int S, const int bz, unsigned long long* stamp, const int cls = 0) {
     constexpr int NS = NS_, UPS_ = 1;
     constexpr int WROWS = BM_ / (NC_ / 2);
     constexpr int MI = WROWS / 16;
@@ -1022,7 +1069,10 @@
     const long m0 = (long)bx * BM_;
     const int n0 = by * BN;
     const int kch0 = a.Cin >> 5;
-    const int ntap0 = FOLD_ ? 12 : a.taps;
+    static_assert(!CLS_ || (!FOLD_ && !UP_ && !STATS_ && EPI_ == ES_EPI_NONE && BM_ == 256), "the class schedule: plain 3x3x3 SAME launches, split");
+    const unsigned cls_mask = CLS_ ? cls_tap_mask(g.H, g.W, cls >> g.lw, cls & (g.W - 1)) : 0u;
+    int ntap0 = FOLD_ ? 12 : a.taps;
+    if constexpr (CLS_) ntap0 = __builtin_popcount(cls_mask);
     const int nks0 = ntap0 * kch0;
     const int nloc = ks_end - ks_begin;
     const int nstage = (nloc + UPS_ - 1) / UPS_;
@@ -1038,7 +1088,8 @@
             const int p = (pw + NP_ * j) * 64 + lane;
             const int row = p >> 2;
             a_lc[j] = (p & 3) ^ f_swz(row);
-            const long m = m0 + row;
+            long m = m0 + row;
+            if constexpr (CLS_) m = ((m0 + row) << (g.lw + g.lh)) + cls;
             a_ok[j] = m < M;
             const long mm = a_ok[j] ? m : 0;
             a_w[j] = (int)(mm & (g.W - 1));
@@ -1056,13 +1107,17 @@
         int st_c = st_phase ? (ks_begin - nks0) : (ks_begin / ntap0);
         int st_ntap = st_phase ? 1 : ntap0, st_kch = st_phase ? (a.Cin2 >> 5) : kch0;
         unsigned st_boff = (unsigned)(st_phase ? (ks_begin - nks0) : ks_begin) * (unsigned)B_BYTES;
+        unsigned st_bits = cls_mask;
+        if constexpr (CLS_)
+            for (int k = 0; !st_phase && k < st_tap; ++k) st_bits &= st_bits - 1u;
         unsigned voff[NA], msk[NA];
         int upm[NA][3], upp[NA][3];
         int dtab = 0;
         __amdgpu_buffer_rsrc_t rA, rB;
         auto set_phase = [&]() __attribute__((always_inline)) {
             const _Float16* Wg = (const _Float16*)(st_phase ? a.w2 : a.w);
-            const long nks_ph = st_phase ? (long)(a.Cin2 >> 5) : (long)nks0;
+            long nks_ph = st_phase ? (long)(a.Cin2 >> 5) : (long)nks0;
+            if constexpr (CLS_) nks_ph = st_phase ? (long)(a.Cin2 >> 5) : (long)a.taps * kch0;
             if constexpr (FOLD_) Wg = (const _Float16*)a.w2 + ((long)fold_cls * ((a.N + BN - 1) / BN) * nks0) * (BNP * BK);
             rB = __builtin_amdgcn_make_buffer_rsrc((void*)(Wg + ((long)by * nks_ph) * (BNP * BK)), (short)0, (int)OOB, 0x00020000);
             const _Float16* Ag = (const _Float16*)(st_phase ? a.a2 : a.a);
@@ -1112,6 +1167,10 @@
         auto issue_unit = [&](char* dst) __attribute__((always_inline)) {
             int tap27 = st_tap;
             if constexpr (FOLD_) tap27 = (st_tap >> 2) * 9 + (((st_tap >> 1) & 1) + fold_ph) * 3 + (st_tap & 1) + fold_pw;
+            if constexpr (CLS_) {
+                tap27 = st_phase ? 0 : __builtin_ctz(st_bits);
+                if (!st_phase) st_boff = (unsigned)(st_c * 27 + tap27) * (unsigned)B_BYTES;
+            }
             const unsigned sA = (unsigned)__builtin_amdgcn_readlane(dtab, tap27) + (unsigned)st_c * 64u;
             const unsigned sbit = 1u << tap27;
             int ukd = 0, ukh = 0, ukw = 0;
@@ -1135,6 +1194,16 @@
                                                          (int)(st_boff + (unsigned)q * 1024u), 0, 0);
             }
             st_boff += (unsigned)B_BYTES;
+            if constexpr (CLS_) {
+                st_bits &= st_bits - 1u;
+                if (st_phase || !st_bits) {
+                    st_bits = cls_mask;
+                    if (++st_c == st_kch && !st_phase && a.a2) {
+                        st_phase = 1; st_c = 0; st_ntap = 1; st_kch = a.Cin2 >> 5; st_boff = 0;
+                        set_phase();
+                    }
+                }
+            } else
             if (++st_tap == st_ntap) {
                 st_tap = 0;
                 if (++st_c == st_kch && !st_phase && a.a2) {
@@ -1164,6 +1233,8 @@
         }
         ES_STAMP_AT(3);
         f4 dummy[MI][7];
+        if constexpr (CLS_) conv_cls_store_slab<BM_, NC_, false>(a, g, dummy, smem, M, m0, n0, wave, lane, bz, cls);
+        else
         conv_epilogue<BM_, NC_, false, true, EPI_, false, STATS_, FOLD_>(a, g, dummy, smem, M, m0, n0, wave, lane, S, bz, ncdhw);
         ES_STAMP_AT(4);
         return;
@@ -1217,6 +1288,8 @@
         ws_mma<MI>(acc, af, bfr);
     }
     ES_STAMP_AT(3);
+    if constexpr (CLS_) conv_cls_store_slab<BM_, NC_, true>(a, g, acc, smem, M, m0, n0, wave, lane, bz, cls);
+    else
     conv_epilogue<BM_, NC_, true, true, EPI_, false, STATS_, FOLD_>(a, g, acc, smem, M, m0, n0, wave, lane, S, bz, ncdhw);
     ES_STAMP_AT(4);
 }
@@ -1238,6 +1311,29 @@
     int ks_begin, ks_end;
     split_range(a.taps * (a.Cin >> 5), a.a2 ? (a.Cin2 >> 5) : 0, a.taps, bz, S, ks_begin, ks_end);
     conv_ws_tile<BM_, NC_, NP_, UP_, EPI_, STATS_, NS_>(a, g, ncdhw, smem, wave, lane, M, bx, by, ks_begin, ks_end, S, bz, stamp);
+}
+
+__global__ __launch_bounds__(768, 3) void k_conv_ws_cls(const es_conv_args a, const ConvGeom g, const ConvClsSched s) {
+    extern __shared__ __attribute__((aligned(16))) char smem[];
+    const int tid = threadIdx.x, lane = tid & 63;
+    const int wave = __builtin_amdgcn_readfirstlane(tid >> 6);
+    unsigned long long* stamp = nullptr;
+    const int wg = blockIdx.x + gridDim.x * (blockIdx.y + gridDim.y * blockIdx.z);
+#ifdef ES_STAMP
+    stamp = g_stamp_buf ? g_stamp_buf + ((size_t)wg * 12 + wave) * 8 : nullptr;
+#endif
+    ES_STAMP_AT(0);
+    const long M = (long)g.O * g.D * g.H * g.W;
+    const int S = gridDim.z;
+    const int per = s.ntm * (int)gridDim.y;
+    const int pi = wg / per, t = wg - pi * per;
+    const int by = t / s.ntm, bx = t - by * s.ntm;
+    const unsigned e = (s.pair[pi >> 2] >> ((pi & 3) * 8)) & 255u;
+    const int cls = (int)(e >> 2), bz = (int)(e & 3u);
+    const int nv = __builtin_popcount(cls_tap_mask(g.H, g.W, cls >> g.lw, cls & (g.W - 1)));
+    int ks_begin, ks_end;
+    split_range(nv * (a.Cin >> 5), a.a2 ? (a.Cin2 >> 5) : 0, 27, bz, S, ks_begin, ks_end);
+    conv_ws_tile<256, 8, 4, false, ES_EPI_NONE, false, 3, false, true>(a, g, 0, smem, wave, lane, M, bx, by, ks_begin, ks_end, S, bz, stamp, cls);
 }
 
 template <bool STATS_>
@@ -2585,7 +2681,8 @@
                                {(const void*)k_linear_ws<ES_EPI_NONE>, LDSLIN}, {(const void*)k_linear_ws<ES_EPI_GEGLU>, LDSLIN},
                                {(const void*)k_conv_ws3<false>, LDSWS3}, {(const void*)k_conv_ws3<true>, LDSWS3},
                                {(const void*)k_conv_ws_fold<false>, LDS256}, {(const void*)k_conv_ws_fold<true>, LDS256},
-                               {(const void*)k_conv_ws_fold_bal<false>, LDS256}, {(const void*)k_conv_ws_fold_bal<true>, LDS256}};
+                               {(const void*)k_conv_ws_fold_bal<false>, LDS256}, {(const void*)k_conv_ws_fold_bal<true>, LDS256},
+                               {(const void*)k_conv_ws_cls, LDS256}};
     ES_REQUIRE(lim.err == hipSuccess, "es_conv_mfma_f16: hipFuncSetAttribute failed: %s", hipGetErrorString(lim.err));
     ES_REQUIRE(r.kernel != ConvKernel::none, "es_conv_mfma_f16: %s", r.omax ? "a chunked route is launched chunk by chunk" : r.unbuilt);
     int rc = 0;
@@ -2626,6 +2723,7 @@
     case ConvKernel::lean_256: launch_lean<256, 8>(a, r, st); break;
     case ConvKernel::lean_128: launch_lean<128, 4>(a, r, st); break;
     case ConvKernel::lean_64: launch_lean<64, 4>(a, r, st); break;
+    case ConvKernel::ws_256_cls: hipLaunchKernelGGL(k_conv_ws_cls, grid_of(r), dim3(768), LDS256, st, *a, r.g, r.cls); break;
     }
     if (rc) return rc;
     const int V = a->D * a->H * a->W;
diff --git a/echoscene_amd/hip.py b/echoscene_amd/hip.py
--- a/echoscene_amd/hip.py
+++ b/echoscene_amd/hip.py
@@ -64,7 +64,8 @@
 
 
 CONV_KERNELS = ('none', 'small_n', 'small_n_tiled', 'n16', 'kw_4_1', 'kw_2_2', 'ws_256_8_4_3', 'ws_64_4_4_3', 'ws_64_4_4_6', 'ws_128_4_4_3',
-                'ws_128_4_8_3', 'ws_128_4_8_5', 'ws3', 'ws_256_up_fold', 'linear_ws', 'linear_deep', 'lean_256', 'lean_128', 'lean_64')
+                'ws_128_4_8_3', 'ws_128_4_8_5', 'ws3', 'ws_256_up_fold', 'linear_ws', 'linear_deep', 'lean_256', 'lean_128', 'lean_64',
+                'ws_256_cls')
 
 
 class GNArgs(C.Structure):
@@ -213,6 +214,10 @@
     'es_conv_kernel_of': (C.c_int, [C.POINTER(ConvArgs), C.c_char_p, C.c_int]),
     'es_conv_fold_balanced': (C.c_int, [C.POINTER(ConvArgs)]),
     'es_conv_route_of': (C.c_int, [C.POINTER(ConvArgs), C.POINTER(ConvRouteInfo)]),
+    'es_conv_cls_tap_mask': (C.c_uint, [C.c_int, C.c_int, C.c_int]),
+    'es_conv_cls_piece': (C.c_int, [C.c_int] * 7 + [C.POINTER(C.c_int), C.POINTER(C.c_int)]),
+    'es_conv_cls_order': (C.c_int, [C.c_int] * 5 + [C.c_char_p, C.c_int]),
+    'es_conv_cls_choose_split': (C.c_int, [C.c_int] * 5),
     'es_split_f16x3': (C.c_int, [C.c_void_p, C.c_long, C.c_int, C.c_void_p, C.c_void_p]),
     'es_pack_conv_f16_size': (C.c_size_t, [C.c_int, C.c_int, C.c_int]),
     'es_pack_conv_f16': (C.c_int, [C.c_void_p, C.c_int, C.c_int, C.c_int, C.c_void_p]),
diff --git a/echoscene_amd/plan_vol.py b/echoscene_amd/plan_vol.py
--- a/echoscene_amd/plan_vol.py
+++ b/echoscene_amd/plan_vol.py
@@ -258,6 +258,13 @@
         if not folded and not ncdhw and Mh * pc.N <= 8192 * 5376 and pc.N % 4 == 0 and not epilogue:
             a.splitk = -1 if splitk is None else splitk
             a.workspace = 1
+            if splitk is None and getattr(self, 'pad_skip', False) and pc.taps == 27 and mode == hip.CONV_SAME:
+                a.splitk = -2
+                name = C.create_string_buffer(32)
+                if hip.lib().es_conv_kernel_of(C.byref(a), name, 32) < 0:
+                    raise RuntimeError('es_conv_kernel_of: ' + hip.lib().es_last_error().decode())
+                if name.value != b'ws_256_cls':
+                    a.splitk = -1
             S = hip.lib().es_conv_split_of(C.byref(a))
             if S < 0:
                 raise RuntimeError('es_conv_split_of: ' + hip.lib().es_last_error().decode())
diff --git a/echoscene_amd/samplers.py b/echoscene_amd/samplers.py
--- a/echoscene_amd/samplers.py
+++ b/echoscene_amd/samplers.py
@@ -282,7 +282,7 @@
 
     def __init__(self, df, model_params=None, ddim_steps=100, device=None, z_shape=(3, 16, 16, 16), rank=0, world=1,
                  group=None, deterministic=False, force_exchange=False, precision='fp16', ddim_eta=0.0, sampler='ddim', weights=None,
-                 up_fold=True):
+                 up_fold=True, pad_skip=True):
         if precision not in ('fp16', 'fp32', 'fp32x'):
             raise ValueError("precision must be 'fp16', 'fp32' or 'fp32x'")
         if sampler not in SHAPE_SAMPLERS:
@@ -316,6 +316,7 @@
         self.rank, self.world, self.group = rank, world, group
         self.deterministic = deterministic
         self.up_fold = bool(up_fold)
+        self.pad_skip = bool(pad_skip)
         self.tables = time_tables(self.w, self.temb, self.w.shape_t, self.device)
         self._plans, self.max_plans = {}, 2
         self._cur, self._use_graph = None, True
@@ -361,6 +362,8 @@
         b.shard_block = block
         b.force_exchange = self.force_exchange
         b.up_fold = self.up_fold and not self.deterministic
+        b.pad_skip = (self.pad_skip and not self.deterministic and self.precision == 'fp16' and self.world == 1
+                      and not self.force_exchange)
         if self.deterministic:
             b.o_hint = -CANON_OBJECTS
         plms = sampler == 'plms'
diff --git a/include/echoscene_hip.h b/include/echoscene_hip.h
--- a/include/echoscene_hip.h
+++ b/include/echoscene_hip.h
@@ -220,6 +220,10 @@
     int32_t fold_bal;
 } es_conv_route_info;
 int es_conv_route_of(const es_conv_args* args, es_conv_route_info* out);
+unsigned es_conv_cls_tap_mask(int H, int W, int cls);
+int es_conv_cls_piece(int H, int W, int cls, int kch0, int kch2, int bz, int S, int* ks_begin, int* ks_end);
+int es_conv_cls_order(int H, int W, int kch0, int kch2, int S, unsigned char* pairs_out, int cap);
+int es_conv_cls_choose_split(int H, int W, int kch0, int kch2, int slab_cap);
 int es_split_f16x3(const float* x, long M, int C, void* out, es_stream stream);
 size_t es_pack_conv_f16_size(int N, int Cin, int taps);
 int es_pack_conv_f16(const float* h_w, int N, int Cin, int taps, uint16_t* h_out);
```
